# DerrickXuNu/CoBEVT

Measured on AMD Instinct MI355X. Metric: bev_frames_per_sec, higher is better.
Workload: dtype bf16

## Files before the change

### cobevt_amd/build.py

```python
import os
import subprocess
import sys

CSRC = os.path.join(os.path.dirname(os.path.abspath(__file__)), "csrc")
LIB = os.path.join(CSRC, "libcobevt_hip.so")
LIB_F32S = os.path.join(CSRC, "libcobevt_hip_f32s.so")
LIB_F32H = os.path.join(CSRC, "libcobevt_hip_f32h.so")
SOURCES = ["igemm.hip", "conv3x3.hip", "basicblock.hip", "bottleneck.hip", "bottleneck_f32.hip", "gemm_rows.hip", "gemm_rows3.hip", "gemm_rows3_f32.hip", "bev_query.hip", "row_chain.hip", "row_chain_f32.hip", "row_chain64.hip", "ln_linear64.hip", "proj_chain128.hip", "proj_chain_k.hip", "swap_stage.hip", "stem7x7.hip", "attention.hip", "attention_resident.hip", "attention_bwd.hip", "train_rows.hip", "train_glue.hip", "train_prep.hip", "wgrad3.hip", "train_nusc.hip", "train_fax.hip", "elementwise.hip", "pairwise_fusion.hip", "postprocess.hip", "depthwise.hip", "peer_gather.hip", "calibrate.hip"]
HEADERS = ["common.hpp", "attn_common.hpp", "warp_common.hpp", "row_chain.hpp", "bev_query.hpp"]
FLAGS = ["--offload-arch=gfx950", "-O3", "-std=c++17", "-fPIC", "-Wno-pass-failed"]
EXTRA_FLAGS = {}


def _hipcc():
    for cand in (os.environ.get("HIPCC"), "/opt/rocm/bin/hipcc", "hipcc"):
        if cand and (os.path.sep not in cand or os.path.exists(cand)):
            return cand
    raise RuntimeError("hipcc not found")


def _stale(target, deps):
    if not os.path.exists(target):
        return True
    t = os.path.getmtime(target)
    return any(os.path.getmtime(d) > t for d in deps)


def _build_one(lib, objdir, extra, force, verbose):
    hipcc = _hipcc()
    hdrs = [os.path.join(CSRC, h) for h in HEADERS]
    os.makedirs(objdir, exist_ok=True)
    objs = []
    procs = []
    for src in SOURCES:
        s = os.path.join(CSRC, src)
        o = os.path.join(objdir, src.replace(".hip", ".o"))
        objs.append(o)
        if force or _stale(o, [s] + hdrs):
            cmd = [hipcc] + FLAGS + extra + EXTRA_FLAGS.get(src, []) + ["-c", s, "-o", o]
            if verbose:
                print(" ".join(cmd), flush=True)
            procs.append((src, subprocess.Popen(cmd, stdout=subprocess.PIPE, stderr=subprocess.STDOUT)))
    for src, p in procs:
        out, _ = p.communicate()
        if p.returncode != 0:
            raise RuntimeError("hipcc failed for %s:\n%s" % (src, out.decode(errors="replace")))
    if force or _stale(lib, objs):
        cmd = [hipcc, "--offload-arch=gfx950", "-shared", "-fPIC", "-o", lib] + objs
        if verbose:
            print(" ".join(cmd), flush=True)
        subprocess.check_call(cmd)
    return lib


def build(force=False, verbose=True):
    _build_one(LIB_F32S, os.path.join(CSRC, "f32s"), ["-DCOBEVT_F32_SPLIT=1"], force, verbose)
    _build_one(LIB_F32H, os.path.join(CSRC, "f32h"), ["-DCOBEVT_F32_SPLIT=2"], force, verbose)
    return _build_one(LIB, CSRC, [], force, verbose)


if __name__ == "__main__":
    build(force="--force" in sys.argv)
    print(LIB)
```

### cobevt_amd/csrc/proj_chain128.hip

```cpp
#include "row_chain.hpp"

namespace cobevt {

namespace {

constexpr int kFp = 0, kFn = 32, kMaxNnt = 8;
constexpr int kTab = (kFn + kMaxNnt * 8) * 1024;
constexpr int kSc = 0, kSh = 128, kBp = 256, kBn = 384;
constexpr int kTabFloats = 640;
constexpr int kLdsBytes = kTab + kTabFloats * 4;

__device__ __forceinline__ float xhalf_sum(float v) {
    const auto r = __builtin_amdgcn_permlane32_swap(__float_as_uint(v), __float_as_uint(v), false, false);
    return __uint_as_float(r[0]) + __uint_as_float(r[1]);
}
__device__ __forceinline__ void half_swap(uint2& a, uint2& b) {
    auto r = __builtin_amdgcn_permlane32_swap(a.x, b.x, false, false);
    a.x = r[0]; b.x = r[1];
    r = __builtin_amdgcn_permlane32_swap(a.y, b.y, false, false);
    a.y = r[0]; b.y = r[1];
}
__device__ __forceinline__ uint4 pack8(const float* v) {
    return make_uint4(pack_bf2(v[0], v[1]), pack_bf2(v[2], v[3]), pack_bf2(v[4], v[5]), pack_bf2(v[6], v[7]));
}
__device__ __forceinline__ float rbf(float x) { return bf2f(f2bf(x)); }

template <int NNT, int NW>
__global__ __launch_bounds__(NW * 64, 1) void proj_chain128_kernel(RowChainParams p, int nblk) {
    extern __shared__ __attribute__((aligned(16))) unsigned char smem[];
    const uint4* wl = (const uint4*)smem;
    float* tab = (float*)(smem + kTab);
    const int tid = threadIdx.x, lane = tid & 63, wave = tid >> 6;
    const int h = lane >> 5, ql = lane & 31;

    {
        uint4* dst = (uint4*)smem;
        constexpr int TOTAL = (kFn + NNT * 8) * 64, PER = (TOTAL + NW * 64 - 1) / (NW * 64);
        uint4 tmp[PER];
#pragma unroll
        for (int u = 0; u < PER; ++u) {
            const int i = tid + u * NW * 64, ic = i < TOTAL ? i : TOTAL - 1;
            const int f = ic >> 6, ln = ic & 63, hh = ln >> 5, q = ln & 31;
            const uint4* base = f < kFn ? p.wp + (size_t)f * 64 : p.wn + (size_t)(f - kFn) * 64;
            const unsigned char* a0 = (const unsigned char*)(base + (f < kFn ? ln : q)) + (f < kFn ? 0 : 8 * hh);
            const unsigned char* a1 = f < kFn ? a0 + 8 : (const unsigned char*)(base + 32 + q) + 8 * hh;
            const uint2 lo = *(const uint2*)a0, hi = *(const uint2*)a1;
            tmp[u] = make_uint4(lo.x, lo.y, hi.x, hi.y);
        }
#pragma unroll
        for (int u = 0; u < PER; ++u) {
            const int i = tid + u * NW * 64;
            if (i < TOTAL) dst[i] = tmp[u];
        }
        for (int i = tid; i < kTabFloats; i += NW * 64) {
            float v;
            if (i < kSh) v = p.pre_scale ? p.pre_scale[i] : 1.f;
            else if (i < kBp) v = p.pre_shift ? p.pre_shift[i - kSh] : 0.f;
            else if (i < kBn) v = p.bp ? p.bp[i - kBp] : 0.f;
            else v = (p.bn && i - kBn < p.Nn) ? p.bn[i - kBn] : 0.f;
            tab[i] = v;
        }
    }
    __syncthreads();

    int opq = 0;
    const float relu_floor = (p.pre_scale && p.pre_relu) ? 0.f : -INFINITY;
    auto load_tile = [&](uint4 (&fr)[8], int first) {
#pragma unroll
        for (int g = 0; g < 8; ++g) fr[g] = wl[(first + g) * 64 + lane + opq];
    };
    const int nwaves = gridDim.x * NW;
    for (int blk = blockIdx.x * NW + wave; blk < nblk; blk += nwaves) {
        asm volatile("" : "+v"(opq));
        const int m0 = blk * 32;
        const bool live = m0 + ql < p.M;
        const size_t grow = live ? m0 + ql : p.M - 1;
        const bf16_t* arow = p.a + grow * 128;
        uint4 af[8], sk[8];
#pragma unroll
        for (int g = 0; g < 8; ++g) af[g] = *(const uint4*)(arow + 16 * g + 8 * h);
        if (p.skip) {
            const bf16_t* srow = p.skip + (size_t)(grow % p.skip_rows) * 128;
#pragma unroll
            for (int g = 0; g < 8; ++g) sk[g] = *(const uint4*)(srow + 16 * g + 8 * h);
        } else {
#pragma unroll
            for (int g = 0; g < 8; ++g) sk[g] = make_uint4(0, 0, 0, 0);
        }
#pragma unroll
        for (int g = 0; g < 8; ++g) {
            float v[8];
            chunk_to_f32<bf16_t>(af[g], v);
            const float* sc = tab + kSc + 16 * g + 8 * h + opq;
            const float4 s0 = *(const float4*)sc, s1 = *(const float4*)(sc + 4);
            const float4 t0 = *(const float4*)(sc + (kSh - kSc)), t1 = *(const float4*)(sc + (kSh - kSc) + 4);
            v[0] = fmaxf(fmaf(v[0], s0.x, t0.x), relu_floor); v[1] = fmaxf(fmaf(v[1], s0.y, t0.y), relu_floor);
            v[2] = fmaxf(fmaf(v[2], s0.z, t0.z), relu_floor); v[3] = fmaxf(fmaf(v[3], s0.w, t0.w), relu_floor);
            v[4] = fmaxf(fmaf(v[4], s1.x, t1.x), relu_floor); v[5] = fmaxf(fmaf(v[5], s1.y, t1.y), relu_floor);
            v[6] = fmaxf(fmaf(v[6], s1.z, t1.z), relu_floor); v[7] = fmaxf(fmaf(v[7], s1.w, t1.w), relu_floor);
            af[g] = f32_to_chunk<bf16_t>(v);
        }

        float y[4][16];
        uint4 fr[2][8];
        load_tile(fr[0], kFp);
#pragma unroll
        for (int t = 0; t < 4; ++t) {
            f32x16 acc;
#pragma unroll
            for (int r = 0; r < 16; ++r) acc[r] = 0.f;
            load_tile(fr[(t + 1) & 1], t < 3 ? kFp + (t + 1) * 8 : kFn);
            __builtin_amdgcn_sched_barrier(0);
#pragma unroll
            for (int g = 0; g < 8; ++g) mfma_kgroup<bf16_t>(fr[t & 1][g], af[g], acc);
#pragma unroll
            for (int m = 0; m < 2; ++m) {
                uint2 s0 = make_uint2(sk[2 * t + m].x, sk[2 * t + m].y), s1 = make_uint2(sk[2 * t + m].z, sk[2 * t + m].w);
                half_swap(s0, s1);
                const float4 b0 = *(const float4*)(tab + kBp + 32 * t + 16 * m + 4 * h + opq);
                const float4 b1 = *(const float4*)(tab + kBp + 32 * t + 16 * m + 8 + 4 * h + opq);
                float* d = &y[t][8 * m];
                d[0] = rbf(acc[8 * m + 0] + b0.x + bf2f(s0.x & 0xffff)); d[1] = rbf(acc[8 * m + 1] + b0.y + bf2f(s0.x >> 16));
                d[2] = rbf(acc[8 * m + 2] + b0.z + bf2f(s0.y & 0xffff)); d[3] = rbf(acc[8 * m + 3] + b0.w + bf2f(s0.y >> 16));
                d[4] = rbf(acc[8 * m + 4] + b1.x + bf2f(s1.x & 0xffff)); d[5] = rbf(acc[8 * m + 5] + b1.y + bf2f(s1.x >> 16));
                d[6] = rbf(acc[8 * m + 6] + b1.z + bf2f(s1.y & 0xffff)); d[7] = rbf(acc[8 * m + 7] + b1.w + bf2f(s1.y >> 16));
            }
        }
        if (p.out) {
            bf16_t* orow = p.out + grow * 128;
#pragma unroll
            for (int i = 0; i < 8; ++i) {
                const uint4 pk = pack8(&y[i >> 1][8 * (i & 1)]);
                uint2 r0 = make_uint2(pk.x, pk.y), r1 = make_uint2(pk.z, pk.w);
                half_swap(r0, r1);
                if (live) *(uint4*)(orow + 16 * i + 8 * h) = make_uint4(r0.x, r0.y, r1.x, r1.y);
            }
        }
        if (p.next_ln) {
            float s = 0.f;
#pragma unroll
            for (int t = 0; t < 4; ++t)
#pragma unroll
                for (int r = 0; r < 16; ++r) s += y[t][r];
            const float mean = xhalf_sum(s) * (1.0f / 128.0f);
            float q = 0.f;
#pragma unroll
            for (int t = 0; t < 4; ++t)
#pragma unroll
                for (int r = 0; r < 16; ++r) { const float d = y[t][r] - mean; q += d * d; }
            const float rstd = rsqrtf(xhalf_sum(q) * (1.0f / 128.0f) + p.eps_next);
#pragma unroll
            for (int t = 0; t < 4; ++t)
#pragma unroll
                for (int r = 0; r < 16; ++r) y[t][r] = (y[t][r] - mean) * rstd;
        }
        uint4 yh[8];
#pragma unroll
        for (int t = 0; t < 4; ++t)
#pragma unroll
            for (int u = 0; u < 2; ++u) yh[2 * t + u] = pack8(&y[t][8 * u]);

        bf16_t* nrow = p.out_next + grow * p.Nn;
#pragma unroll
        for (int n = 0; n < NNT; ++n) {
            f32x16 acc;
#pragma unroll
            for (int r = 0; r < 16; ++r) acc[r] = 0.f;
            if (n + 1 < NNT) load_tile(fr[(n + 1) & 1], kFn + (n + 1) * 8);
            __builtin_amdgcn_sched_barrier(0);
#pragma unroll
            for (int g = 0; g < 8; ++g) mfma_kgroup<bf16_t>(fr[n & 1][g], yh[g], acc);
            float nv[16];
#pragma unroll
            for (int k = 0; k < 4; ++k) {
                const float4 b = *(const float4*)(tab + kBn + 32 * n + 8 * k + 4 * h + opq);
                nv[4 * k] = acc[4 * k] + b.x; nv[4 * k + 1] = acc[4 * k + 1] + b.y;
                nv[4 * k + 2] = acc[4 * k + 2] + b.z; nv[4 * k + 3] = acc[4 * k + 3] + b.w;
            }
#pragma unroll
            for (int m = 0; m < 2; ++m) {
                const uint4 pk = pack8(&nv[8 * m]);
                uint2 r0 = make_uint2(pk.x, pk.y), r1 = make_uint2(pk.z, pk.w);
                half_swap(r0, r1);
                if (live) *(uint4*)(nrow + 32 * n + 16 * m + 8 * h) = make_uint4(r0.x, r0.y, r1.x, r1.y);
            }
        }
    }
}

template <int NNT> int launch128(const RowChainParams& p, hipStream_t stream) {
    constexpr int NW = 8;
    static cobevt::PerDeviceOnce attr_once;
    if (attr_once.first()) {
        (void)hipFuncSetAttribute((const void*)proj_chain128_kernel<NNT, NW>, hipFuncAttributeMaxDynamicSharedMemorySize, kLdsBytes);
    }
    const int nblk = (p.M + 31) / 32;
    int blocks = (nblk + NW - 1) / NW;
    if (blocks > 256) blocks = 256;
    hipLaunchKernelGGL((proj_chain128_kernel<NNT, NW>), dim3((unsigned)blocks), dim3(NW * 64), kLdsBytes, stream, p, nblk);
    return hipGetLastError() == hipSuccess ? COBEVT_OK : COBEVT_ERR_LAUNCH;
}

}

int launch_proj_chain128(const RowChainParams& p, hipStream_t stream) {
    if (p.C != 128 || !p.wn || !p.out_next || p.Nn % 32 != 0 || p.Nn > 32 * kMaxNnt || p.next_act != 0) return -1;
    if (p.M < 32768) return -1;
    switch (p.Nn / 32) {
        case 4: return launch128<4>(p, stream);
        case 8: return launch128<8>(p, stream);
        default: return -1;
    }
}

}
```

### cobevt_amd/csrc/proj_chain_k.hip

```cpp
#include "row_chain.hpp"

namespace cobevt {

namespace {

constexpr int kRow = 256 + 16;
constexpr int kNnMax = 768;

struct ProjChainKSide {
    const float* pre_scale;
    const float* pre_shift;
    const uint4* wp;
    const float* bp;
    const bf16_t* skip;
    const uint4* wn;
    const float* bn;
    bf16_t* out;
    bf16_t* out_next;
    int pre_relu, skip_rows;
};

struct ProjChainKParams {
    const bf16_t* a;
    ProjChainKSide side[2];
    int M, K, Nn, next_ln;
    float eps_next;
};

struct Lds {
    static constexpr int A = 0;
    static constexpr int Y = A + 32 * kRow;
    static constexpr int BIAS = Y + 32 * kRow;
    static constexpr int BYTES = BIAS + 4 * (128 + kNnMax);
};

__device__ __forceinline__ void normalise128(float (&v)[16], float eps) {
    float s = 0.f;
#pragma unroll
    for (int e = 0; e < 16; ++e) s += v[e];
    s += __shfl_xor(s, 1, 64); s += __shfl_xor(s, 2, 64); s += __shfl_xor(s, 4, 64);
    const float mean = s * (1.0f / 128.0f);
    float q = 0.f;
#pragma unroll
    for (int e = 0; e < 16; ++e) { const float d = v[e] - mean; q += d * d; }
    q += __shfl_xor(q, 1, 64); q += __shfl_xor(q, 2, 64); q += __shfl_xor(q, 4, 64);
    const float rstd = rsqrtf(q * (1.0f / 128.0f) + eps);
#pragma unroll
    for (int e = 0; e < 16; ++e) v[e] = (v[e] - mean) * rstd;
}

template <int NCH>
__global__ __launch_bounds__(256, 4) void proj_chain_k_kernel(ProjChainKParams p) {
    extern __shared__ __attribute__((aligned(16))) unsigned char smem[];
    unsigned char* As = smem + Lds::A;
    unsigned char* Ys = smem + Lds::Y;
    float* sb = (float*)(smem + Lds::BIAS);

    ProjChainKSide sd;
    {
        const bool s1 = blockIdx.y != 0;
        const ProjChainKSide &u = p.side[0], &w = p.side[1];
        sd.pre_scale = s1 ? w.pre_scale : u.pre_scale; sd.pre_shift = s1 ? w.pre_shift : u.pre_shift;
        sd.wp = s1 ? w.wp : u.wp; sd.bp = s1 ? w.bp : u.bp; sd.skip = s1 ? w.skip : u.skip;
        sd.wn = s1 ? w.wn : u.wn; sd.bn = s1 ? w.bn : u.bn; sd.out = s1 ? w.out : u.out; sd.out_next = s1 ? w.out_next : u.out_next;
        sd.pre_relu = s1 ? w.pre_relu : u.pre_relu; sd.skip_rows = s1 ? w.skip_rows : u.skip_rows;
    }
    const int tid = threadIdx.x, lane = tid & 63, wn = tid >> 6;
    const int h = lane >> 5, ql = lane & 31;
    const int m0 = blockIdx.x * 32;
    const int row = ql;
    const bool row_ok = m0 + row < p.M;
    const int sr = tid >> 3, sub = tid & 7;
    const bool srow_ok = m0 + sr < p.M;
    constexpr int NKG = NCH * 8;

    {
        constexpr int NIT = (128 + kNnMax + 255) / 256;
        float val[NIT];
#pragma unroll
        for (int it = 0; it < NIT; ++it) {
            const int i = tid + it * 256;
            const bool isp = i < 128;
            const float* src = isp ? sd.bp : sd.bn;
            const int j = isp ? i : i - 128;
            const bool keep = (src != nullptr) & (i < 128 + kNnMax) & (isp | (j < p.Nn));
            val[it] = keep ? src[j] : 0.f;
        }
#pragma unroll
        for (int it = 0; it < NIT; ++it) {
            const int i = tid + it * 256;
            if (i < 128 + kNnMax) sb[i] = val[it];
        }
    }

    auto load_frags = [&](uint4 (&b)[8], const uint4* w, int tile, int nkg, int kg0) {
        const uint4* src = w + ((size_t)tile * nkg + kg0) * 64 + lane;
#pragma unroll
        for (int g = 0; g < 8; ++g) b[g] = src[g * 64];
        __builtin_amdgcn_sched_barrier(0);
    };
    f32x16 acc;
    auto mma = [&](const uint4 (&b)[8], bool zero) {
        if (zero) {
#pragma unroll
            for (int r = 0; r < 16; ++r) acc[r] = 0.f;
        }
        const int abase = row * kRow + h * 16;
#pragma unroll
        for (int g = 0; g < 8; ++g) {
            const uint4 af = *(const uint4*)(As + abase + g * 32);
            mfma_kgroup<bf16_t>(b[g], af, acc);
        }
    };
    auto load_rows = [&](uint4 (&v)[2], int c) {
        const bf16_t* src = p.a + (size_t)(srow_ok ? m0 + sr : 0) * p.K + c * 128 + sub * 16;
        v[0] = *(const uint4*)src;
        v[1] = *(const uint4*)(src + 8);
    };
    auto stage_rows = [&](const uint4 (&v)[2], int c) {
#pragma unroll
        for (int j = 0; j < 2; ++j) {
            uint4 o = v[j];
            if (sd.pre_scale) {
                const int k = c * 128 + sub * 16 + j * 8;
                float f[8];
                chunk_to_f32<bf16_t>(v[j], f);
                const float4 s0 = *(const float4*)(sd.pre_scale + k), s1 = *(const float4*)(sd.pre_scale + k + 4);
                const float4 t0 = *(const float4*)(sd.pre_shift + k), t1 = *(const float4*)(sd.pre_shift + k + 4);
                const float sc[8] = {s0.x, s0.y, s0.z, s0.w, s1.x, s1.y, s1.z, s1.w}, sh[8] = {t0.x, t0.y, t0.z, t0.w, t1.x, t1.y, t1.z, t1.w};
#pragma unroll
                for (int e = 0; e < 8; ++e) {
                    f[e] = fmaf(f[e], sc[e], sh[e]);
                    if (sd.pre_relu) f[e] = fmaxf(f[e], 0.f);
                }
                o = f32_to_chunk<bf16_t>(f);
            }
            if (!srow_ok) o = make_uint4(0, 0, 0, 0);
            *(uint4*)(As + sr * kRow + sub * 32 + j * 16) = o;
        }
    };

    uint4 fa[8], fb[8];
    uint4 ra[2], rb[2];
    load_rows(ra, 0);
    load_frags(fa, sd.wp, wn, NKG, 0);
    const int cbase = wn * 32 + 4 * h;
    uint2 skp[4];
#pragma unroll
    for (int k = 0; k < 4; ++k) {
        skp[k] = make_uint2(0, 0);
        if (sd.skip && row_ok) skp[k] = *(const uint2*)(sd.skip + (size_t)((m0 + row) % sd.skip_rows) * 128 + cbase + 8 * k);
    }

#pragma unroll
    for (int c = 0; c < NCH; ++c) {
        if (c & 1) stage_rows(rb, c); else stage_rows(ra, c);
        if (c + 1 < NCH) {
            if (c & 1) { load_rows(ra, c + 1); load_frags(fa, sd.wp, wn, NKG, 8 * (c + 1)); }
            else { load_rows(rb, c + 1); load_frags(fb, sd.wp, wn, NKG, 8 * (c + 1)); }
        } else {
            if (c & 1) load_frags(fa, sd.wn, wn, 8, 0); else load_frags(fb, sd.wn, wn, 8, 0);
        }
        __syncthreads();
        if (c & 1) mma(fb, false); else mma(fa, c == 0);
        __syncthreads();
    }

    auto pack4 = [&](float x, float y, float z, float w) { return make_uint2(pack_bf2(x, y), pack_bf2(z, w)); };
#pragma unroll
    for (int k = 0; k < 4; ++k) {
        const int col0 = cbase + 8 * k;
        const float4 b = *(const float4*)(sb + col0);
        *(uint2*)(Ys + row * kRow + col0 * 2) = pack4(acc[4 * k] + b.x + bf2f(skp[k].x & 0xffff), acc[4 * k + 1] + b.y + bf2f(skp[k].x >> 16),
                                                      acc[4 * k + 2] + b.z + bf2f(skp[k].y & 0xffff), acc[4 * k + 3] + b.w + bf2f(skp[k].y >> 16));
    }
    __syncthreads();

    {
        const uint4 y0 = *(const uint4*)(Ys + sr * kRow + sub * 32), y1 = *(const uint4*)(Ys + sr * kRow + sub * 32 + 16);
        if (sd.out && srow_ok) {
            *(uint4*)(sd.out + (size_t)(m0 + sr) * 128 + sub * 16) = y0;
            *(uint4*)(sd.out + (size_t)(m0 + sr) * 128 + sub * 16 + 8) = y1;
        }
        uint4 o0 = y0, o1 = y1;
        if (p.next_ln) {
            float v[16];
            chunk_to_f32<bf16_t>(y0, v);
            chunk_to_f32<bf16_t>(y1, v + 8);
            normalise128(v, p.eps_next);
            o0 = f32_to_chunk<bf16_t>(v);
            o1 = f32_to_chunk<bf16_t>(v + 8);
        }
        *(uint4*)(As + sr * kRow + sub * 32) = o0;
        *(uint4*)(As + sr * kRow + sub * 32 + 16) = o1;
    }
    __syncthreads();

    const int npn = (p.Nn + 127) / 128;
    auto next_pass = [&](int pass, const uint4 (&cur)[8], uint4 (&nxt)[8]) {
        if (pass + 1 < npn) load_frags(nxt, sd.wn, (pass + 1) * 4 + wn, 8, 0);
        mma(cur, true);
#pragma unroll
        for (int k = 0; k < 4; ++k) {
            const int col0 = pass * 128 + cbase + 8 * k;
            const float4 b = *(const float4*)(sb + 128 + col0);
            *(uint2*)(Ys + row * kRow + (cbase + 8 * k) * 2) = pack4(acc[4 * k] + b.x, acc[4 * k + 1] + b.y, acc[4 * k + 2] + b.z, acc[4 * k + 3] + b.w);
        }
        __syncthreads();
        if (srow_ok) {
#pragma unroll
            for (int j = 0; j < 2; ++j) {
                const int c0 = pass * 128 + sub * 16 + j * 8;
                if (c0 < p.Nn) *(uint4*)(sd.out_next + (size_t)(m0 + sr) * p.Nn + c0) = *(const uint4*)(Ys + sr * kRow + sub * 32 + j * 16);
            }
        }
        if (pass + 1 < npn) __syncthreads();
    };
    for (int pass = 0; pass < npn; pass += 2) {
        if (NCH & 1) {
            next_pass(pass, fb, fa);
            if (pass + 1 < npn) next_pass(pass + 1, fa, fb);
        } else {
            next_pass(pass, fa, fb);
            if (pass + 1 < npn) next_pass(pass + 1, fb, fa);
        }
    }
}

template <int NCH>
void launch(const ProjChainKParams& p, int nsides, hipStream_t stream) {
    static cobevt::PerDeviceOnce attr_once;
    if (attr_once.first())
        (void)hipFuncSetAttribute((const void*)proj_chain_k_kernel<NCH>, hipFuncAttributeMaxDynamicSharedMemorySize, Lds::BYTES);
    hipLaunchKernelGGL((proj_chain_k_kernel<NCH>), dim3((unsigned)((p.M + 31) / 32), (unsigned)nsides), dim3(256), Lds::BYTES, stream, p);
}

}

}

using namespace cobevt;

extern "C" int cobevt_proj_chain_kv(const void* a, const void* const* ptrs, const int* dims, float eps_next, hipStream_t stream) {
    if (!a || !ptrs || !dims) return COBEVT_ERR_ARG;
    if (dims[0] != 0) return COBEVT_ERR_UNSUPPORTED;
    ProjChainKParams p;
    p.a = (const bf16_t*)a;
    p.M = dims[1]; p.K = dims[2]; p.Nn = dims[3]; p.next_ln = dims[4];
    const int nsides = dims[5];
    p.eps_next = eps_next;
    if (nsides < 1 || nsides > 2) return COBEVT_ERR_ARG;
    if (p.M < 1 || p.K < 256 || p.K > 512 || p.K % 128) return COBEVT_ERR_SHAPE;
    if (p.Nn < 8 || p.Nn % 8 || p.Nn > kNnMax) return COBEVT_ERR_SHAPE;
    for (int s = 0; s < 2; ++s) {
        const void* const* q = ptrs + 9 * (s < nsides ? s : 0);
        ProjChainKSide& sd = p.side[s];
        sd.pre_scale = (const float*)q[0]; sd.pre_shift = (const float*)q[1];
        sd.wp = (const uint4*)q[2]; sd.bp = (const float*)q[3]; sd.skip = (const bf16_t*)q[4];
        sd.wn = (const uint4*)q[5]; sd.bn = (const float*)q[6];
        sd.out = (bf16_t*)q[7]; sd.out_next = (bf16_t*)q[8];
        sd.pre_relu = dims[6 + 2 * (s < nsides ? s : 0)];
        sd.skip_rows = dims[7 + 2 * (s < nsides ? s : 0)] > 0 ? dims[7 + 2 * (s < nsides ? s : 0)] : p.M;
        if (!sd.wp || !sd.wn || !sd.out_next) return COBEVT_ERR_ARG;
        if ((sd.pre_scale == nullptr) != (sd.pre_shift == nullptr)) return COBEVT_ERR_ARG;
        if (sd.skip_rows > p.M || p.M % sd.skip_rows) return COBEVT_ERR_SHAPE;
    }
    switch (p.K / 128) {
        case 2: launch<2>(p, nsides, stream); break;
        case 3: launch<3>(p, nsides, stream); break;
        default: launch<4>(p, nsides, stream); break;
    }
    return hipGetLastError() == hipSuccess ? COBEVT_OK : COBEVT_ERR_LAUNCH;
}
```

### cobevt_amd/csrc/row_chain.hip

```cpp
#include "row_chain.hpp"

namespace cobevt {

constexpr int kRcRow = 256 + 16;
constexpr int kRcHRow = 512 + 16;
template <int ROWS> struct RcLds {
    static constexpr int A = 0;
    static constexpr int Y = A + ROWS * kRcRow;
    static constexpr int H = Y + ROWS * kRcRow;
    static constexpr int TOTAL = H + ROWS * kRcHRow;
    static constexpr int BIAS = TOTAL;
    static constexpr int BYTES = TOTAL + 4 * 1536;
};
constexpr int kRcBp = 0, kRcB1 = 128, kRcB2 = 384, kRcPg = 512, kRcPb = 640, kRcBn = 768, kRcBnMax = 768, kRcBiasFloats = 1536;

__device__ __forceinline__ void rc_normalise(float (&v)[16], int sub, int C, float eps) {
    float s = 0.f;
#pragma unroll
    for (int e = 0; e < 16; ++e) s += v[e];
    s += __shfl_xor(s, 1, 64); s += __shfl_xor(s, 2, 64); s += __shfl_xor(s, 4, 64);
    const float mean = s / (float)C;
    float q = 0.f;
#pragma unroll
    for (int e = 0; e < 16; ++e) { const float d = (sub * 16 + e) < C ? v[e] - mean : 0.f; q += d * d; }
    q += __shfl_xor(q, 1, 64); q += __shfl_xor(q, 2, 64); q += __shfl_xor(q, 4, 64);
    const float rstd = rsqrtf(q / (float)C + eps);
#pragma unroll
    for (int e = 0; e < 16; ++e) v[e] = (sub * 16 + e) < C ? (v[e] - mean) * rstd : 0.f;
}

template <int NPASS, int ROWS, bool FULL, bool MLP = true>
__global__ __launch_bounds__(ROWS * 8, 4) void row_chain_kernel(RowChainParams p) {
    extern __shared__ __attribute__((aligned(16))) unsigned char smem[];
    unsigned char* As = smem + RcLds<ROWS>::A;
    unsigned char* Ys = smem + RcLds<ROWS>::Y;
    unsigned char* Hs = smem + RcLds<ROWS>::H;

    const int tid = threadIdx.x, lane = tid & 63, wave = tid >> 6;
    const int h = lane >> 5, ql = lane & 31;
    const int wm = wave >> 2, wn = wave & 3;
    const int m0 = blockIdx.x * ROWS;
    const int ngc = FULL ? 8 : (p.C * 2 + 31) / 32;
    const int row = wm * 32 + ql;
    const bool row_ok = m0 + row < p.M;

    auto load_frags = [&](uint4 (&b)[8], const uint4* w, int tile, int nkg, int kg0, int n) {
        const uint4* src = w + ((size_t)tile * nkg + kg0) * 64 + lane;
#pragma unroll
        for (int g = 0; g < 8; ++g)
            if (g < n) b[g] = src[g * 64];
        __builtin_amdgcn_sched_barrier(0);
    };
    f32x16 acc;
    auto mma = [&](const unsigned char* A, int a_off, const uint4 (&b)[8], int n, bool zero) {
        if (zero) {
#pragma unroll
            for (int r = 0; r < 16; ++r) acc[r] = 0.f;
        }
#pragma unroll
        for (int g = 0; g < 8; ++g)
            if (g < n) {
                const uint4 af = *(const uint4*)(A + a_off + g * 32);
                mfma_kgroup<bf16_t>(b[g], af, acc);
            }
    };
    const int cbase = wn * 32 + 4 * h;
    const float* sb = (const float*)(smem + RcLds<ROWS>::BIAS);
    {
        float* w = (float*)(smem + RcLds<ROWS>::BIAS);
        constexpr int NT = ROWS * 8, NIT = kRcBiasFloats / NT;
        static_assert(kRcBiasFloats % NT == 0, "bias table fill");
        float val[NIT];
        bool keep[NIT];
#pragma unroll
        for (int it = 0; it < NIT; ++it) {
            const int i = tid + it * NT;
            const float* src = i < kRcB1 ? p.bp : i < kRcB2 ? p.b1 : i < kRcPg ? p.b2 : i < kRcPb ? p.post_g : i < kRcBn ? p.post_b : p.bn;
            const int j = i < kRcB1 ? i : i < kRcB2 ? i - kRcB1 : i < kRcPg ? i - kRcB2 : i < kRcPb ? i - kRcPg : i < kRcBn ? i - kRcPb : i - kRcBn;
            const int n = i < kRcB1 ? p.C : i < kRcB2 ? p.Hd : i < kRcBn ? p.C : p.Nn;
            keep[it] = (src != nullptr) & (j < n);
            val[it] = (src ? src : p.b1)[keep[it] ? j : 0];
        }
#pragma unroll
        for (int it = 0; it < NIT; ++it) w[tid + it * NT] = keep[it] ? val[it] : 0.f;
    }
    auto bias4 = [&](int table, int col0) { return *(const float4*)(sb + table + col0); };
    auto pack4 = [&](float x, float y, float z, float w) { return make_uint2(pack_bf2(x, y), pack_bf2(z, w)); };

    uint4 fa[8], fb[8];
    const int abase = row * kRcRow + h * 16;

    load_frags(fa, p.wp, wn, 8, 0, ngc);
    {
        const int r = tid >> 3, sub = tid & 7;
        const bool ok = m0 + r < p.M;
#pragma unroll
        for (int j = 0; j < 2; ++j) {
            const int k = (sub * 2 + j) * 8;
            uint4 v = make_uint4(0, 0, 0, 0);
            if (ok && k < p.C) v = *(const uint4*)(p.a + (size_t)(m0 + r) * p.C + k);
            if (!MLP && p.pre_scale) {
                float f[8];
                chunk_to_f32<bf16_t>(v, f);
                const float4 s0 = *(const float4*)(p.pre_scale + k), s1 = *(const float4*)(p.pre_scale + k + 4);
                const float4 t0 = *(const float4*)(p.pre_shift + k), t1 = *(const float4*)(p.pre_shift + k + 4);
                const float sc[8] = {s0.x, s0.y, s0.z, s0.w, s1.x, s1.y, s1.z, s1.w}, sh[8] = {t0.x, t0.y, t0.z, t0.w, t1.x, t1.y, t1.z, t1.w};
#pragma unroll
                for (int e = 0; e < 8; ++e) {
                    f[e] = fmaf(f[e], sc[e], sh[e]);
                    if (p.pre_relu) f[e] = fmaxf(f[e], 0.f);
                }
                v = ok ? f32_to_chunk<bf16_t>(f) : make_uint4(0, 0, 0, 0);
            }
            *(uint4*)(As + r * kRcRow + (sub * 2 + j) * 16) = v;
        }
    }
    uint2 skp[4];
#pragma unroll
    for (int k = 0; k < 4; ++k) {
        const int col0 = cbase + 8 * k;
        skp[k] = make_uint2(0, 0);
        if (p.skip && row_ok && col0 < p.C) skp[k] = *(const uint2*)(p.skip + (size_t)((m0 + row) % p.skip_rows) * p.C + col0);
    }
    __syncthreads();

    mma(As, abase, fa, ngc, true);
    if (MLP) load_frags(fb, p.w1, wn, 8, 0, ngc);
    else load_frags(fb, p.wn, wn, 8, 0, ngc);
#pragma unroll
    for (int k = 0; k < 4; ++k) {
        const int col0 = cbase + 8 * k;
        const float4 b = bias4(kRcBp, col0);
        float v0 = acc[4 * k] + b.x + bf2f(skp[k].x & 0xffff), v1 = acc[4 * k + 1] + b.y + bf2f(skp[k].x >> 16);
        float v2 = acc[4 * k + 2] + b.z + bf2f(skp[k].y & 0xffff), v3 = acc[4 * k + 3] + b.w + bf2f(skp[k].y >> 16);
        if (col0 >= p.C) v0 = v1 = v2 = v3 = 0.f;
        *(uint2*)(Ys + row * kRcRow + col0 * 2) = pack4(v0, v1, v2, v3);
    }
    __syncthreads();
    float* stage = (float*)Hs;
    constexpr int SROW = kRcHRow / 4;
    if constexpr (MLP) {

    if (NPASS == 2) load_frags(fa, p.w1, 4 + wn, 8, 0, ngc);
    else load_frags(fa, p.w2, wn, p.Hdp / 16, 0, 8);
    {
        const int r = tid >> 3, sub = tid & 7;
        float v[16];
        chunk_to_f32<bf16_t>(*(const uint4*)(Ys + r * kRcRow + sub * 32), v);
        chunk_to_f32<bf16_t>(*(const uint4*)(Ys + r * kRcRow + sub * 32 + 16), v + 8);
        rc_normalise(v, sub, p.C, p.eps1);
        *(uint4*)(As + r * kRcRow + sub * 32) = f32_to_chunk<bf16_t>(v);
        *(uint4*)(As + r * kRcRow + sub * 32 + 16) = f32_to_chunk<bf16_t>(v + 8);
    }
    __syncthreads();

    auto hidden_epilogue = [&](int pass) {
#pragma unroll
        for (int k = 0; k < 4; ++k) {
            const int col0 = pass * 128 + cbase + 8 * k;
            const float4 b = bias4(kRcB1, col0);
            uint2 o = make_uint2(0, 0);
            if (col0 < p.Hd) o = pack4(gelu_bf16(acc[4 * k] + b.x), gelu_bf16(acc[4 * k + 1] + b.y),
                                       gelu_bf16(acc[4 * k + 2] + b.z), gelu_bf16(acc[4 * k + 3] + b.w));
            *(uint2*)(Hs + row * kRcHRow + col0 * 2) = o;
        }
    };
    const int hbase = row * kRcHRow + h * 16;
    if (NPASS == 2) {
        mma(As, abase, fb, ngc, true);
        load_frags(fb, p.w2, wn, p.Hdp / 16, 0, 8);
        hidden_epilogue(0);
        mma(As, abase, fa, ngc, true);
        load_frags(fa, p.w2, wn, p.Hdp / 16, 8, 8);
        hidden_epilogue(1);
        __syncthreads();
        mma(Hs, hbase, fb, 8, true);
        load_frags(fb, p.wn ? p.wn : p.w1, wn, 8, 0, ngc);
        mma(Hs, hbase + 256, fa, 8, false);
    } else {
        mma(As, abase, fb, ngc, true);
        load_frags(fb, p.wn ? p.wn : p.w1, wn, 8, 0, ngc);
        hidden_epilogue(0);
        __syncthreads();
        mma(Hs, hbase, fa, (p.Hd * 2 + 31) / 32, true);
    }
    __syncthreads();
#pragma unroll
    for (int k = 0; k < 4; ++k) {
        const int col0 = cbase + 8 * k;
        const float4 b = bias4(kRcB2, col0);
        const uint2 y = *(const uint2*)(Ys + row * kRcRow + col0 * 2);
        float4 z = make_float4(0.f, 0.f, 0.f, 0.f);
        if (col0 < p.C)
            z = make_float4(acc[4 * k] + b.x + bf2f(y.x & 0xffff), acc[4 * k + 1] + b.y + bf2f(y.x >> 16),
                            acc[4 * k + 2] + b.z + bf2f(y.y & 0xffff), acc[4 * k + 3] + b.w + bf2f(y.y >> 16));
        *(float4*)(stage + row * SROW + col0) = z;
    }
    } else {
#pragma unroll
        for (int k = 0; k < 4; ++k) {
            const int col0 = cbase + 8 * k;
            const uint2 y = *(const uint2*)(Ys + row * kRcRow + col0 * 2);
            *(float4*)(stage + row * SROW + col0) = make_float4(bf2f(y.x & 0xffff), bf2f(y.x >> 16), bf2f(y.y & 0xffff), bf2f(y.y >> 16));
        }
    }
    const int npn = p.wn ? (p.Nn + 127) / 128 : 0;
    __syncthreads();

    {
        const int r = tid >> 3, sub = tid & 7;
        const bool live = m0 + r < p.M;
        float v[16];
#pragma unroll
        for (int e = 0; e < 16; e += 4) {
            const float4 t = *(const float4*)(stage + r * SROW + sub * 16 + e);
            v[e] = t.x; v[e + 1] = t.y; v[e + 2] = t.z; v[e + 3] = t.w;
        }
        if (p.post_g) {
            rc_normalise(v, sub, p.C, p.eps_post);
#pragma unroll
            for (int e = 0; e < 16; e += 4) {
                const float4 g = *(const float4*)(sb + kRcPg + sub * 16 + e), b = *(const float4*)(sb + kRcPb + sub * 16 + e);
                v[e] = v[e] * g.x + b.x; v[e + 1] = v[e + 1] * g.y + b.y;
                v[e + 2] = v[e + 2] * g.z + b.z; v[e + 3] = v[e + 3] * g.w + b.w;
            }
        }
        uint4 o[2];
        o[0] = f32_to_chunk<bf16_t>(v);
        o[1] = f32_to_chunk<bf16_t>(v + 8);
        if (live && (MLP || p.out)) {
#pragma unroll
            for (int j = 0; j < 2; ++j) {
                const int c0 = sub * 16 + j * 8;
                if (c0 < p.C) *(uint4*)(p.out + (size_t)(m0 + r) * p.C + c0) = o[j];
            }
        }
        if (!npn) return;

        if (p.next_ln) {
            chunk_to_f32<bf16_t>(o[0], v);
            chunk_to_f32<bf16_t>(o[1], v + 8);
            rc_normalise(v, sub, p.C, p.eps_next);
            o[0] = f32_to_chunk<bf16_t>(v);
            o[1] = f32_to_chunk<bf16_t>(v + 8);
        }
        *(uint4*)(As + r * kRcRow + sub * 32) = o[0];
        *(uint4*)(As + r * kRcRow + sub * 32 + 16) = o[1];
    }
    __syncthreads();
    auto next_pass = [&](int pass, const uint4 (&cur)[8], uint4 (&nxt)[8]) {
        if (pass + 1 < npn) load_frags(nxt, p.wn, (pass + 1) * 4 + wn, 8, 0, ngc);
        mma(As, abase, cur, ngc, true);
#pragma unroll
        for (int k = 0; k < 4; ++k) {
            const int col0 = pass * 128 + cbase + 8 * k;
            const float4 b = bias4(kRcBn, col0);
            float v0 = acc[4 * k] + b.x, v1 = acc[4 * k + 1] + b.y, v2 = acc[4 * k + 2] + b.z, v3 = acc[4 * k + 3] + b.w;
            if (p.next_act == 1) { v0 = fmaxf(v0, 0.f); v1 = fmaxf(v1, 0.f); v2 = fmaxf(v2, 0.f); v3 = fmaxf(v3, 0.f); }
            else if (p.next_act == 2) { v0 = gelu_bf16(v0); v1 = gelu_bf16(v1); v2 = gelu_bf16(v2); v3 = gelu_bf16(v3); }
            *(uint2*)(Ys + row * kRcRow + (cbase + 8 * k) * 2) = pack4(v0, v1, v2, v3);
        }
        __syncthreads();
        {
            const int r = tid >> 3, sub = tid & 7;
            if (m0 + r < p.M) {
#pragma unroll
                for (int j = 0; j < 2; ++j) {
                    const int c0 = pass * 128 + sub * 16 + j * 8;
                    if (c0 < p.Nn) *(uint4*)(p.out_next + (size_t)(m0 + r) * p.Nn + c0) = *(const uint4*)(Ys + r * kRcRow + sub * 32 + j * 16);
                }
            }
        }
        if (pass + 1 < npn) __syncthreads();
    };
    for (int pass = 0; pass < npn; pass += 2) {
        next_pass(pass, fb, fa);
        if (pass + 1 < npn) next_pass(pass + 1, fa, fb);
    }
}

template <int NPASS, int ROWS, bool FULL, bool MLP = true>
static void launch_chain(const RowChainParams& p, hipStream_t stream) {
    static cobevt::PerDeviceOnce attr_once;
    if (attr_once.first()) {
        (void)hipFuncSetAttribute((const void*)row_chain_kernel<NPASS, ROWS, FULL, MLP>, hipFuncAttributeMaxDynamicSharedMemorySize, RcLds<ROWS>::BYTES);
    }
    const unsigned blocks = (unsigned)((p.M + ROWS - 1) / ROWS);
    hipLaunchKernelGGL((row_chain_kernel<NPASS, ROWS, FULL, MLP>), dim3(blocks), dim3(ROWS * 8), RcLds<ROWS>::BYTES, stream, p);
}

}

using namespace cobevt;

extern "C" int cobevt_attn_mlp_chain(const void* a, const void* skip, void* out, const void* wp, const float* bp,
                                     const void* w1, const float* b1, const void* w2, const float* b2,
                                     const float* post_gamma, const float* post_beta, const void* wnext, const float* bnext,
                                     void* out_next, const int* dims, float eps1, float eps_post, float eps_next,
                                     hipStream_t stream) {
    if (!a || !out || !wp || !w1 || !b1 || !w2 || !b2 || !dims) return COBEVT_ERR_ARG;
    if (dims[0] != 0 && dims[0] != 1) return COBEVT_ERR_ARG;
    if (dims[0] == 1) {
        if ((post_gamma == nullptr) != (post_beta == nullptr) || (wnext == nullptr) != (out_next == nullptr)) return COBEVT_ERR_ARG;
        const int M = dims[1], sr = dims[9] > 0 ? dims[9] : dims[1];
        if (M < 1 || sr > M || M % sr || (wnext && (dims[7] < 0 || dims[7] > 2))) return COBEVT_ERR_SHAPE;
        const int rc = launch_row_chain_f32(a, skip, out, wp, bp, w1, b1, w2, b2, post_gamma, post_beta, wnext, bnext, out_next, M, dims[2], dims[3],
                                            dims[4], dims[5], dims[6], dims[7], sr, eps1, eps_post, eps_next, stream);
        return rc < 0 ? COBEVT_ERR_UNSUPPORTED : rc;
    }
    RowChainParams p;
    p.a = (const bf16_t*)a; p.skip = (const bf16_t*)skip; p.out = (bf16_t*)out;
    p.wp = (const uint4*)wp; p.bp = bp; p.w1 = (const uint4*)w1; p.b1 = b1; p.w2 = (const uint4*)w2; p.b2 = b2;
    p.post_g = post_gamma; p.post_b = post_beta;
    p.wn = (const uint4*)wnext; p.bn = bnext; p.out_next = (bf16_t*)out_next;
    p.M = dims[1]; p.C = dims[2]; p.Hd = dims[3]; p.Hdp = dims[4];
    p.Nn = dims[5]; p.next_ln = dims[6]; p.next_act = dims[7];
    p.skip_rows = dims[9] > 0 ? dims[9] : p.M;
    p.eps1 = eps1; p.eps_post = eps_post; p.eps_next = eps_next;
    p.pre_scale = p.pre_shift = nullptr; p.pre_relu = 0;
    if (p.M < 1 || p.C < 8 || p.C > 128 || p.C % 8 || p.Hd < 8 || p.Hd > 256 || p.Hd % 8) return COBEVT_ERR_SHAPE;
    if (p.Hdp % 128 || p.Hdp < p.Hd || p.Hdp > 256) return COBEVT_ERR_SHAPE;
    if (p.skip_rows > p.M || p.M % p.skip_rows) return COBEVT_ERR_SHAPE;
    if ((post_gamma == nullptr) != (post_beta == nullptr)) return COBEVT_ERR_ARG;
    if ((wnext == nullptr) != (out_next == nullptr)) return COBEVT_ERR_ARG;
    if (wnext && (p.Nn < 8 || p.Nn % 8 || p.Nn > kRcBnMax || p.next_act < 0 || p.next_act > 2)) return COBEVT_ERR_SHAPE;
    if (dims[8] == 0) {
        const int rc = launch_row_chain64(p, stream);
        if (rc >= 0) return rc;
    }
    const int rows = dims[8] == 64 ? 64 : 32;
    const bool two = p.Hd > 128, full = p.C == 128;
    if (rows == 64) {
        if (two) { if (full) launch_chain<2, 64, true>(p, stream); else launch_chain<2, 64, false>(p, stream); }
        else { if (full) launch_chain<1, 64, true>(p, stream); else launch_chain<1, 64, false>(p, stream); }
    } else {
        if (two) { if (full) launch_chain<2, 32, true>(p, stream); else launch_chain<2, 32, false>(p, stream); }
        else { if (full) launch_chain<1, 32, true>(p, stream); else launch_chain<1, 32, false>(p, stream); }
    }
    return hipGetLastError() == hipSuccess ? COBEVT_OK : COBEVT_ERR_LAUNCH;
}

extern "C" int cobevt_proj_chain(const void* a, const float* pre_scale, const float* pre_shift, const void* skip, const void* wp,
                                 const float* bp, void* out, const void* wnext, const float* bnext, void* out_next, const int* dims,
                                 float eps_next, hipStream_t stream) {
    if (!a || !wp || !wnext || !bnext || !out_next || !dims) return COBEVT_ERR_ARG;
    if ((pre_scale == nullptr) != (pre_shift == nullptr)) return COBEVT_ERR_ARG;
    if (dims[0] != 0) return COBEVT_ERR_UNSUPPORTED;
    RowChainParams p;
    p.a = (const bf16_t*)a; p.skip = (const bf16_t*)skip; p.out = (bf16_t*)out;
    p.wp = (const uint4*)wp; p.bp = bp;
    p.w1 = (const uint4*)wnext; p.b1 = bnext; p.w2 = (const uint4*)wnext; p.b2 = bnext;
    p.post_g = p.post_b = nullptr;
    p.wn = (const uint4*)wnext; p.bn = bnext; p.out_next = (bf16_t*)out_next;
    p.M = dims[1]; p.C = dims[2]; p.Hd = 8; p.Hdp = 128;
    p.Nn = dims[3]; p.next_ln = dims[4]; p.next_act = dims[5];
    p.skip_rows = dims[6] > 0 ? dims[6] : p.M;
    p.pre_scale = pre_scale; p.pre_shift = pre_shift; p.pre_relu = dims[7];
    p.eps1 = 0.f; p.eps_post = 0.f; p.eps_next = eps_next;
    if (p.M < 1 || p.C != 128) return COBEVT_ERR_SHAPE;
    if (p.Nn < 8 || p.Nn % 8 || p.Nn > kRcBnMax || p.next_act < 0 || p.next_act > 2) return COBEVT_ERR_SHAPE;
    if (p.skip_rows > p.M || p.M % p.skip_rows) return COBEVT_ERR_SHAPE;
    if (dims[8] == 0) {
        const int rc = launch_proj_chain128(p, stream);
        if (rc >= 0) return rc;
    }
    launch_chain<1, 32, true, false>(p, stream);
    return hipGetLastError() == hipSuccess ? COBEVT_OK : COBEVT_ERR_LAUNCH;
}
```

### cobevt_amd/csrc/row_chain.hpp

```cpp
#pragma once
#include "common.hpp"

namespace cobevt {

struct RowChainParams {
    const bf16_t* a;
    const bf16_t* skip;
    bf16_t* out;
    const uint4* wp;
    const float* bp;
    const uint4* w1;
    const float* b1;
    const uint4* w2;
    const float* b2;
    const float* post_g;
    const float* post_b;
    const uint4* wn;
    const float* bn;
    bf16_t* out_next;
    int M, C, Hd, Hdp;
    int Nn, next_ln, next_act, skip_rows;
    float eps1, eps_post, eps_next;
    const float* pre_scale;
    const float* pre_shift;
    int pre_relu;
};

int launch_row_chain64(const RowChainParams& p, hipStream_t stream);
int launch_proj_chain128(const RowChainParams& p, hipStream_t stream);

int launch_row_chain_f32(const void* a, const void* skip, void* out, const void* wp, const float* bp, const void* w1, const float* b1,
                         const void* w2, const float* b2, const float* post_g, const float* post_b, const void* wnext, const float* bnext,
                         void* out_next, int M, int C, int Hd, int Hdp, int Nn, int next_ln, int next_act, int skip_rows, float eps1,
                         float eps_post, float eps_next, hipStream_t stream);

}
```

### cobevt_amd/host/fax_modules.py

```python
import torch
import torch.nn as nn

from .. import ops
from ..lib import CobevtHipError
from . import runtime as rt
from . import training
from .runtime import HipModule


def generate_grid(height, width):
    xs = torch.linspace(0, 1, width)
    ys = torch.linspace(0, 1, height)
    gx = xs[None, :].expand(height, width)
    gy = ys[:, None].expand(height, width)
    return torch.stack([gx, gy, torch.ones(height, width)], 0)[None].contiguous()


def get_view_matrix(h=200, w=200, h_meters=100.0, w_meters=100.0, offset=0.0):
    sh = h / h_meters
    sw = w / w_meters
    return [[0., -sw, w / 2.], [-sh, 0., h * offset + h / 2.], [0., 0., 1.]]


class Bottleneck(HipModule):
    expansion = 4

    def __init__(self, inplanes, planes):
        super().__init__()
        width = planes
        self.conv1 = nn.Conv2d(inplanes, width, 1, bias=False)
        self.bn1 = nn.BatchNorm2d(width)
        self.conv2 = nn.Conv2d(width, width, 3, 1, 1, bias=False)
        self.bn2 = nn.BatchNorm2d(width)
        self.conv3 = nn.Conv2d(width, planes * self.expansion, 1, bias=False)
        self.bn3 = nn.BatchNorm2d(planes * self.expansion)
        self.relu = nn.ReLU(inplace=True)
        self.downsample = None

    def entry_plan(self):
        return rt.conv_plan(self, "c1", self.conv1, self.bn1, act=1)

    def fused_plan(self):
        if self.conv1.weight.shape[:2] != (32, 128) or self.downsample is not None:
            return None
        return self._plan("fused", rt.module_tensors(self.conv1, self.bn1, self.conv2, self.bn2, self.conv3, self.bn3),
                          lambda dt, dev: ops.BottleneckPlan(self.conv1, self.bn1, self.conv2, self.bn2, self.conv3, self.bn3, dev))

    def fusable(self, x):
        return ops.bottleneck_fusable(x) and self.conv1.weight.shape[:2] == (32, 128)

    def forward_nhwc(self, x, y1=None):
        if y1 is None and self.fusable(x):
            return ops.bottleneck(x, self.fused_plan())
        p1, p2, p3 = self.entry_plan(), rt.conv_plan(self, "c2", self.conv2, self.bn2, act=1), rt.conv_plan(self, "c3", self.conv3, self.bn3, act=1)
        if ops.bottleneck_f32_fusable(x, p1, p2, p3, y1):
            return ops.bottleneck_f32(x, p1, p2, p3, y1)
        y = ops.conv2d(x, p1) if y1 is None else y1
        y = ops.conv2d(y, p2)
        return ops.conv2d(y, p3, residual=x)

    def forward(self, x):
        if self.training:
            return training.bottleneck(self, x)
        self._require_inference(x)
        return rt.like_input(rt.nchw_view(self.forward_nhwc(rt.to_nhwc(x))), x)


ResNetBottleNeck = lambda c: Bottleneck(c, c // 4)


class BEVEmbedding(nn.Module):

    def __init__(self, dim, sigma, bev_height, bev_width, h_meters, w_meters, offset, upsample_scales):
        super().__init__()
        V_inv = torch.FloatTensor(get_view_matrix(bev_height, bev_width, h_meters, w_meters, offset)).inverse()
        for i, scale in enumerate(upsample_scales):
            h, w = bev_height // scale, bev_width // scale
            grid = generate_grid(h, w).squeeze(0)
            grid[0] = bev_width * grid[0]
            grid[1] = bev_height * grid[1]
            grid = (V_inv @ grid.reshape(3, h * w)).reshape(3, h, w)
            self.register_buffer("grid%d" % i, grid, persistent=False)
        self.learned_features = nn.Parameter(
            sigma * torch.randn(dim, bev_height // upsample_scales[0], bev_width // upsample_scales[0]))

    def get_prior(self):
        return self.learned_features


class Attention(HipModule):

    def __init__(self, dim, dim_head=32, dropout=0., window_size=25):
        super().__init__()
        assert (dim % dim_head) == 0, "dimension should be divisible by dimension per head"
        if dim_head != 32:
            raise CobevtHipError("the HIP attention kernel is built for dim_head = 32")
        self.heads = dim // dim_head
        self.scale = dim_head ** -0.5
        self.window_size = window_size
        self.to_qkv = nn.Linear(dim, dim * 3, bias=False)
        self.attend = nn.Sequential(nn.Softmax(dim=-1), nn.Dropout(dropout))
        self.to_out = nn.Sequential(nn.Linear(dim, dim, bias=False), nn.Dropout(dropout))
        self.rel_pos_bias = nn.Embedding((2 * window_size - 1) ** 2, self.heads)
        pos = torch.arange(window_size)
        gi, gj = torch.meshgrid(pos, pos, indexing="ij")
        grid = torch.stack([gi.reshape(-1), gj.reshape(-1)], -1)
        rel_pos = grid[:, None, :] - grid[None, :, :] + window_size - 1
        rel_pos_indices = (rel_pos * torch.tensor([2 * window_size - 1, 1])).sum(dim=-1)
        self.register_buffer("rel_pos_indices", rel_pos_indices, persistent=False)

    def forward_nhwc(self, x, out=None):
        b, h, w, d = x.shape
        if h != self.window_size or w != self.window_size:
            raise CobevtHipError("FAX global attention expects a %dx%d map" % (self.window_size, self.window_size))
        qkv = ops.linear(x, rt.linear_plan(self, "qkv", self.to_qkv))
        a = torch.empty((b, h, w, d), device=x.device, dtype=x.dtype)
        m = ops.tokmap(0, 1, h, w, h, w)
        table = rt.f32_param(self, "bias", self.rel_pos_bias.weight)
        ops.window_attention(qkv, qkv, qkv, a, m, m, m, b, self.heads, self.scale, 3 * d, 3 * d, 3 * d, d, koff=d,
                             voff=2 * d, bias_table=table, bias_L=1)
        return ops.linear(a, rt.linear_plan(self, "out", self.to_out[0]), out=out)

    def forward(self, x):
        if self.training:
            return training.global_attention(self, x)
        self._require_inference(x)
        return rt.like_input(rt.nchw_view(self.forward_nhwc(rt.to_nhwc(x))), x)


class CrossWinAttention(HipModule):

    def __init__(self, dim, heads, dim_head, qkv_bias, rel_pos_emb=False, norm=nn.LayerNorm):
        super().__init__()
        if dim_head != 32:
            raise CobevtHipError("the HIP attention kernel is built for dim_head = 32")
        self.scale = dim_head ** -0.5
        self.heads = heads
        self.dim_head = dim_head
        self.rel_pos_emb = rel_pos_emb
        self.to_q = nn.Sequential(norm(dim), nn.Linear(dim, heads * dim_head, bias=qkv_bias))
        self.to_k = nn.Sequential(norm(dim), nn.Linear(dim, heads * dim_head, bias=qkv_bias))
        self.to_v = nn.Sequential(norm(dim), nn.Linear(dim, heads * dim_head, bias=qkv_bias))
        self.proj = nn.Linear(heads * dim_head, dim)

    def add_rel_pos_emb(self, x):
        return x

    def _project(self, name, seq, x, out=None):
        return ops.linear(x, rt.linear_plan(self, name, seq[1], ln=seq[0]), out=out)

    def project_kv(self, k_src, v_src, out_k=None, out_v=None):
        return self._project("k", self.to_k, k_src, out_k), self._project("v", self.to_v, v_src, out_v)

    def q_plan(self):
        return rt.linear_plan(self, "q", self.to_q[1], ln=self.to_q[0])

    def attend_projected(self, q_src, kt, vt, qmap, kmap, omap, batch, out_shape, qt=None, ldkv=None, kvoff=0):
        inner = self.heads * self.dim_head
        if qt is None:
            qt = self._project("q", self.to_q, q_src)
        ld = inner if ldkv is None else ldkv
        a = torch.empty(tuple(out_shape) + (inner,), device=qt.device, dtype=qt.dtype)
        ops.window_attention(qt, kt, vt, a, qmap, kmap, omap, batch, self.heads, self.scale, inner, ld, ld, inner,
                             koff=kvoff, voff=kvoff, mean_q=qmap[1] > 1)
        return a

    def attend_core(self, q_src, k_src, v_src, qmap, kmap, omap, batch, out_shape):
        kt, vt = self.project_kv(k_src, v_src)
        return self.attend_projected(q_src, kt, vt, qmap, kmap, omap, batch, out_shape)

    def attend(self, q_src, k_src, v_src, qmap, kmap, omap, batch, skip, out_shape):
        a = self.attend_core(q_src, k_src, v_src, qmap, kmap, omap, batch, out_shape)
        return ops.linear(a, rt.linear_plan(self, "proj", self.proj), residual=skip)

    def forward(self, q, k, v, skip=None):
        if self.training:
            return training.cross_win_attention(self, q, k, v, skip)
        self._require_inference(q, k, v, skip)
        assert k.shape == v.shape
        b, n, X, Y, W1, W2, _ = q.shape
        _, nk, kx, ky, w1, w2, _ = k.shape
        assert X * Y == kx * ky
        qmap = (2, n, X * W1, Y * W2, W1, W2, X, Y)
        kmap = (2, nk, kx * w1, ky * w2, w1, w2, kx, ky)
        omap = (2, 1, X * W1, Y * W2, W1, W2, X, Y)
        sk = rt.as_compute(skip) if skip is not None else None
        z = self.attend(rt.as_compute(q), rt.as_compute(k), rt.as_compute(v), qmap, kmap, omap, b, sk,
                        (b, X, Y, W1, W2))
        return rt.like_input(z, q)


class CrossViewSwapAttention(HipModule):

    def __init__(self, feat_height, feat_width, feat_dim, dim, index, image_height, image_width, qkv_bias, q_win_size,
                 feat_win_size, heads, dim_head, bev_embedding_flag, rel_pos_emb=False, no_image_features=False,
                 skip=True, norm=nn.LayerNorm):
        super().__init__()
        image_plane = generate_grid(feat_height, feat_width)[None]
        image_plane[:, :, 0] *= image_width
        image_plane[:, :, 1] *= image_height
        self.register_buffer("image_plane", image_plane, persistent=False)
        self.feature_linear = nn.Sequential(nn.BatchNorm2d(feat_dim), nn.ReLU(), nn.Conv2d(feat_dim, dim, 1, bias=False))
        if no_image_features:
            self.feature_proj = None
        else:
            self.feature_proj = nn.Sequential(nn.BatchNorm2d(feat_dim), nn.ReLU(), nn.Conv2d(feat_dim, dim, 1, bias=False))
        self.bev_embed_flag = bev_embedding_flag[index]
        if self.bev_embed_flag:
            self.bev_embed = nn.Conv2d(2, dim, 1)
        self.img_embed = nn.Conv2d(4, dim, 1, bias=False)
        self.cam_embed = nn.Conv2d(4, dim, 1, bias=False)
        self.q_win_size = q_win_size[index]
        self.feat_win_size = feat_win_size[index]
        self.rel_pos_emb = rel_pos_emb
        self.cross_win_attend_1 = CrossWinAttention(dim, heads[index], dim_head[index], qkv_bias)
        self.cross_win_attend_2 = CrossWinAttention(dim, heads[index], dim_head[index], qkv_bias)
        self.skip = skip
        self.prenorm_1 = norm(dim)
        self.prenorm_2 = norm(dim)
        self.mlp_1 = nn.Sequential(nn.Linear(dim, 2 * dim), nn.GELU(), nn.Linear(2 * dim, dim))
        self.mlp_2 = nn.Sequential(nn.Linear(dim, 2 * dim), nn.GELU(), nn.Linear(2 * dim, dim))
        self.postnorm = norm(dim)
        self.dim = dim

    def _padded_hw(self, h, w):
        wh, ww = self.feat_win_size
        hp = ((h + wh) // wh) * wh if h % wh != 0 else h
        wp = ((w + ww) // ww) * ww if w % ww != 0 else w
        return hp, wp

    def _proj_mlp(self, name, attn, a, skip, prenorm, mlp, postnorm=None, next_plan=None):
        post = None
        if postnorm is not None:
            post = (rt.f32_param(self, name + ".post.w", postnorm.weight), rt.f32_param(self, name + ".post.b", postnorm.bias),
                    postnorm.eps)
        return ops.attn_mlp_chain(a, skip, rt.linear_plan(attn, "proj", attn.proj),
                                  rt.linear_plan(self, name + ".0", mlp[0], act=2, ln=prenorm),
                                  rt.linear_plan(self, name + ".2", mlp[2]), post, next_plan=next_plan)

    def prepare_kv(self, feature, I_inv, E_inv, batch, out=None):
        bn, h, w, _ = feature.shape
        d, dt = self.dim, feature.dtype
        n = bn // batch
        w1, w2 = self.feat_win_size
        hp, wp = self._padded_hw(h, w)
        padded = (hp, wp) != (h, w)
        plane = rt.f32_param(self, "plane", self.image_plane, (3, h * w))
        w_img = rt.f32_param(self, "w_img", self.img_embed.weight, (d, 4))
        w_cam = rt.f32_param(self, "w_cam", self.cam_embed.weight, (d, 4))
        img = ops.ray_embed(I_inv, E_inv, plane, w_img, w_cam, h * w, d, dt).reshape(bn, h, w, d)

        def kv_buffer(tag):
            if not padded:
                return None
            return self._plan("kvpad.%s.%dx%dx%d" % (tag, bn, hp, wp), [self.img_embed.weight],
                              lambda dt_, dev: torch.zeros((bn, hp, wp, d), device=feature.device, dtype=dt))

        o = out if out is not None else {}
        pk, pv = self._pair_plan("k"), self._pair_plan("v")
        plan_key = rt.conv_plan(self, "fproj", self.feature_proj[2], pre_bn=self.feature_proj[0]) if self.feature_proj is not None else None
        plan_val = rt.conv_plan(self, "flin", self.feature_linear[2], pre_bn=self.feature_linear[0])
        if (not padded and plan_key is not None and ops.proj_chain_fusable(feature, plan_key, pk, img)
                and ops.proj_chain_fusable(feature, plan_val, pv, None)):
            kk = ops.proj_chain(feature, plan_key, pk, residual=img, out_next=o.get("kk"))
            vv = ops.proj_chain(feature, plan_val, pv, out_next=o.get("vv"))
            return {"n": n, "hp": hp, "wp": wp, "kk": kk, "vv": vv}
        if not padded and plan_key is not None and ops.proj_chain_kv_fusable(feature, plan_key, plan_val, pk, pv, img):
            kk, vv = ops.proj_chain_kv(feature, plan_key, plan_val, pk, pv, residual=img, out_k=o.get("kk"), out_v=o.get("vv"))
            return {"n": n, "hp": hp, "wp": wp, "kk": kk, "vv": vv}
        if self.feature_proj is not None:
            key = ops.conv2d(feature, plan_key, residual=img, out=kv_buffer("key"))
        elif padded:
            key = ops.copy_into_interior(img, kv_buffer("key"))
        else:
            key = img
        val = ops.conv2d(feature, plan_val, out=kv_buffer("val"))
        kk = ops.linear(key, pk, out=o.get("kk"))
        vv = ops.linear(val, pv, out=o.get("vv"))
        return {"n": n, "hp": hp, "wp": wp, "kk": kk, "vv": vv}

    def _pair_plan(self, which):
        a1, a2 = getattr(self.cross_win_attend_1, "to_" + which), getattr(self.cross_win_attend_2, "to_" + which)
        if a1[0].eps != a2[0].eps:
            raise CobevtHipError("the two cross attentions normalise their keys / values with different eps")

        def build(dt, dev):
            ws, bs = [], []
            for ln, lin in ((a1[0], a1[1]), (a2[0], a2[1])):
                w = lin.weight.detach().double().cpu()
                b = lin.bias.detach().double().cpu() if lin.bias is not None else torch.zeros(w.shape[0], dtype=torch.float64)
                g, be = ln.weight.detach().double().cpu(), ln.bias.detach().double().cpu()
                bs.append(b + w @ be)
                ws.append(w * g[None, :])
            return ops.ConvPlan(torch.cat(ws), torch.cat(bs), dtype=dt, device=dev, ln_folded_eps=a1[0].eps)
        return self._plan("pair_" + which, rt.module_tensors(a1[0], a1[1], a2[0], a2[1]), build)

    def forward_query(self, index, x, bev, E_inv, kv, next_plan=None):
        b, H, W, d = x.shape
        n, hp, wp = kv["n"], kv["hp"], kv["wp"]
        W1, W2 = self.q_win_size
        w1, w2 = self.feat_win_size
        if self.bev_embed_flag:
            grid = getattr(bev, "grid%d" % index)
            world = rt.f32_param(self, "world%d" % index, grid[:2], (2, H * W))
            w_bev = rt.f32_param(self, "w_bev", self.bev_embed.weight, (d, 2))
            b_bev = rt.f32_param(self, "b_bev", self.bev_embed.bias)
            w_cam = rt.f32_param(self, "w_cam", self.cam_embed.weight, (d, 4))
            q1 = ops.bev_embed_linear(E_inv, world, w_bev, b_bev, w_cam, x.reshape(b, H * W, d), n,
                                      self.cross_win_attend_1.q_plan())
            query, nq = None, n
        else:
            x = x.contiguous()
            query, nq, q1 = x, 1, None
        qmap_n = ops.tokmap(0, nq, H, W, W1, W2)
        qmap_1 = ops.tokmap(0, 1, H, W, W1, W2)
        kwin = ops.tokmap(0, n, hp, wp, w1, w2)
        kgrid = ops.tokmap(1, n, hp, wp, w1, w2)
        if qmap_1[6] * qmap_1[7] != kwin[6] * kwin[7]:
            raise CobevtHipError("query windows %dx%d != key windows %dx%d" % (qmap_1[6], qmap_1[7], kwin[6], kwin[7]))
        inner = self.cross_win_attend_1.heads * self.cross_win_attend_1.dim_head
        a = self.cross_win_attend_1.attend_projected(query, kv["kk"], kv["vv"], qmap_n, kwin, qmap_1, b, (b, H, W), qt=q1,
                                                     ldkv=2 * inner, kvoff=0)
        y, q2 = self._proj_mlp("mlp1", self.cross_win_attend_1, a, x if self.skip else None, self.prenorm_1, self.mlp_1,
                               next_plan=self.cross_win_attend_2.q_plan())
        a = self.cross_win_attend_2.attend_projected(y, kv["kk"], kv["vv"], qmap_1, kgrid, qmap_1, b, (b, H, W), qt=q2,
                                                     ldkv=2 * inner, kvoff=inner)
        return self._proj_mlp("mlp2", self.cross_win_attend_2, a, y if self.skip else None, self.prenorm_2, self.mlp_2,
                              self.postnorm, next_plan=next_plan)

    def forward_nhwc(self, index, x, bev, feature, I_inv, E_inv):
        return self.forward_query(index, x, bev, E_inv, self.prepare_kv(feature, I_inv, E_inv, x.shape[0]))

    def forward(self, index, x, bev, feature, I_inv, E_inv):
        if self.training:
            return training.cross_view_swap_attention(self, index, x, bev, feature, I_inv, E_inv)
        self._require_inference(x, feature, I_inv, E_inv)
        b, n = feature.shape[:2]
        f = rt.to_nhwc(feature.reshape(b * n, *feature.shape[2:]))
        Ii = I_inv.reshape(b * n, 3, 3).to(torch.float32).contiguous()
        Ei = E_inv.reshape(b * n, 4, 4).to(torch.float32).contiguous()
        y = self.forward_nhwc(index, rt.to_nhwc(x), bev, f, Ii, Ei)
        return rt.like_input(rt.nchw_view(y), x)


class _Downsample(HipModule):

    def __init__(self, dim_in, dim_mid, dim_out):
        super().__init__()
        mods = [nn.Conv2d(dim_in, dim_mid, kernel_size=3, stride=1, padding=1, bias=False), nn.PixelUnshuffle(2),
                nn.Conv2d(dim_out, dim_out, 3, padding=1, bias=False), nn.BatchNorm2d(dim_out), nn.ReLU(inplace=True),
                nn.Conv2d(dim_out, dim_out, 1, padding=0, bias=False), nn.BatchNorm2d(dim_out)]
        for i, m in enumerate(mods):
            self.add_module(str(i), m)

    def __getitem__(self, i):
        return getattr(self, str(i))

    def forward_nhwc(self, x, out=None):
        y = ops.conv2d(x, rt.conv_plan(self, "c0", self[0], store_mode=1))
        y = ops.conv2d(y, rt.conv_plan(self, "c2", self[2], self[3], act=1))
        return ops.conv2d(y, rt.conv_plan(self, "c5", self[5], self[6]), out=out)


class FAXModule(HipModule):

    _downsample_div = 4

    def __init__(self, config):
        super().__init__()
        middle = config["middle"]
        dim = config["dim"]
        self.backbone_output_shape = config["backbone_output_shape"]
        assert len(middle) == len(self.backbone_output_shape)
        cross_view = config["cross_view"]
        cross_view_swap = config["cross_view_swap"]
        cross_views, layers, downsample_layers = [], [], []
        for i, (feat_shape, num_layers) in enumerate(zip(self.backbone_output_shape, middle)):
            _, _, _, feat_dim, feat_height, feat_width = tuple(feat_shape)
            cross_views.append(CrossViewSwapAttention(feat_height, feat_width, feat_dim, dim[i], i, **cross_view,
                                                      **cross_view_swap))
            layers.append(nn.Sequential(*[ResNetBottleNeck(dim[i]) for _ in range(num_layers)]))
            if i < len(middle) - 1:
                downsample_layers.append(nn.Sequential(_Downsample(dim[i], dim[i] // self._downsample_div, dim[i + 1])))
        self.bev_embedding = BEVEmbedding(dim[0], **config["bev_embedding"])
        self.cross_views = nn.ModuleList(cross_views)
        self.layers = nn.ModuleList(layers)
        self.downsample_layers = nn.ModuleList(downsample_layers)
        self.self_attn = Attention(dim[-1], **config["self_attn"])

    taps = None

    def forward_features(self, features, I_inv, E_inv, batch, kv=None, levels=None, x=None, out=None):
        nlev = len(self.cross_views)
        first, last = (0, nlev) if levels is None else levels
        if first == 0:
            dt = rt.get_compute_dtype()
            prior = self._plan("prior", [self.bev_embedding.learned_features],
                               lambda d_, dev: self.bev_embedding.learned_features.detach().permute(1, 2, 0).to(dt).contiguous())
            x = prior[None].expand(batch, *prior.shape)
        for i, (cross_view, feature, layer) in enumerate(zip(self.cross_views, features, self.layers)):
            if i < first or i >= last:
                continue
            kvi = kv[i]() if kv is not None else cross_view.prepare_kv(feature, I_inv, E_inv, batch)
            blocks = list(layer)
            y1 = None
            if blocks and not (x.dtype == torch.bfloat16 and ops.USE_BOTTLENECK and x.shape[-1] == 128
                               and blocks[0].conv1.weight.shape[:2] == (32, 128)):
                x, y1 = cross_view.forward_query(i, x, self.bev_embedding, E_inv, kvi, next_plan=blocks[0].entry_plan())
            else:
                x = cross_view.forward_query(i, x, self.bev_embedding, E_inv, kvi)
            for j, blk in enumerate(blocks):
                x = blk.forward_nhwc(x, y1=y1 if j == 0 else None)
            if self.taps is not None:
                self.taps["level%d" % i] = x
            if i < len(self.cross_views) - 1:
                final = out is not None and i == last - 1 and not (self.self_attn is not None and last == nlev)
                x = self.downsample_layers[i][0].forward_nhwc(x, out=out if final else None)
        if self.self_attn is not None and last == nlev:
            x = self.self_attn.forward_nhwc(x, out=out)
        if out is not None and x.data_ptr() != out.data_ptr():
            out.copy_(x)
            x = out
        return x

    def forward(self, batch):
        if self.training:
            return training.fax_module(self, batch)
        b, l, n = batch["inputs"].shape[:3]
        intrinsic, extrinsic = batch["intrinsic"], batch["extrinsic"]
        self._require_inference(intrinsic, extrinsic, *batch["features"])
        I_inv = ops.invert_small(intrinsic.reshape(b * l * n, 3, 3))
        E_inv = self._extrinsic(extrinsic.reshape(b * l * n, 4, 4).to(torch.float32)).contiguous()
        feats = [rt.to_nhwc(f.reshape(b * l * n, *f.shape[3:])) for f in batch["features"]]
        x = self.forward_features(feats, I_inv, E_inv, b * l)
        x = rt.nchw_view(x)
        return x.reshape(b, l, *x.shape[1:])

    @staticmethod
    def _extrinsic(e):
        return e
```

### cobevt_amd/lib.py

```python
import ctypes
import os

import torch

_HERE = os.path.dirname(os.path.abspath(__file__))
LIB_PATH = os.path.join(_HERE, "csrc", "libcobevt_hip.so")
LIB_PATH = os.environ.get("COBEVT_HIP_LIB") or LIB_PATH

_c_int_p = ctypes.POINTER(ctypes.c_int)
_c_long_p = ctypes.POINTER(ctypes.c_long)
_vp = ctypes.c_void_p

SIGNATURES = {
    "cobevt_abi_version": (ctypes.c_int, []),
    "cobevt_strerror": (ctypes.c_char_p, [ctypes.c_int]),
    "cobevt_conv2d_nhwc": (ctypes.c_int, [_vp, _vp, _vp, _vp, _vp, _vp, _vp, _vp, _c_int_p, _vp]),
    "cobevt_conv3x3_nhwc": (ctypes.c_int, [_vp, _vp, _vp, _vp, _vp, _c_int_p, _vp]),
    "cobevt_basicblock_nhwc": (ctypes.c_int, [_vp, _vp, _vp, _vp, _vp, _vp, _c_int_p, _vp]),
    "cobevt_dsblock_nhwc": (ctypes.c_int, [_vp, _vp, _vp, _vp, _vp, _vp, _vp, _vp, _c_int_p, _vp]),
    "cobevt_conv3x3_wfrag_nhwc": (ctypes.c_int, [_vp, _vp, _vp, _vp, _vp, _c_int_p, _vp]),
    "cobevt_conv3x3_ds_wfrag_nhwc": (ctypes.c_int, [_vp, _vp, _vp, _vp, _vp, _vp, _c_int_p, _vp]),
    "cobevt_stem_conv7x7s2_pool": (ctypes.c_int, [_vp, _vp, _vp, _vp, _c_int_p, _vp]),
    "cobevt_stem_conv7x7s2": (ctypes.c_int, [_vp, _vp, _vp, _vp, _c_int_p, _vp]),
    "cobevt_stem_conv7x7s2_pool_u8": (ctypes.c_int, [_vp, _vp, _vp, _vp, _vp, _c_int_p, _vp]),
    "cobevt_bev_embed_linear_rows": (ctypes.c_int, [_vp] * 9 + [_c_long_p, ctypes.c_float, _vp]),
    "cobevt_linear_rows_wfrag": (ctypes.c_int, [_vp, _vp, _vp, _vp, _vp, _vp, _vp, _c_long_p, ctypes.c_float, _vp]),
    "cobevt_linear_rows": (ctypes.c_int, [_vp, _vp, _vp, _vp, _vp, _vp, _vp, _vp, _vp, _c_long_p, ctypes.c_float, _vp]),
    "cobevt_attn_mlp_chain": (ctypes.c_int, [_vp] * 14 + [_c_int_p, ctypes.c_float, ctypes.c_float, ctypes.c_float, _vp]),
    "cobevt_pairwise_warp": (ctypes.c_int, [_vp] * 5 + [ctypes.c_int] * 6 + [ctypes.c_float, ctypes.c_float, _vp]),
    "cobevt_pairwise_warp_bwd": (ctypes.c_int, [_vp] * 4 + [ctypes.c_int] * 6 + [ctypes.c_float, ctypes.c_float, _vp]),
    "cobevt_agent_message_reduce": (ctypes.c_int, [_vp] * 5 + [ctypes.c_int] * 6 + [_vp]),
    "cobevt_gru_zero_state": (ctypes.c_int, [_vp, _vp, ctypes.c_int, ctypes.c_long, ctypes.c_int, _vp]),
    "cobevt_agent_softmax_sum": (ctypes.c_int, [_vp, ctypes.c_int, _vp, _vp, _vp, _vp] + [ctypes.c_int] * 6 + [_vp]),
    "cobevt_window_attention": (ctypes.c_int, [_vp, _vp, _vp, _vp, _vp, _vp, _c_int_p, ctypes.c_float, _vp]),
    "cobevt_window_attention_ksplit": (ctypes.c_int, [_vp] * 8 + [_c_int_p, ctypes.c_float, ctypes.c_int, ctypes.c_long, _vp]),
    "cobevt_window_attention_lse": (ctypes.c_int, [_vp, _vp, _vp, _vp, _vp, _vp, _vp, _c_int_p, ctypes.c_float, ctypes.c_float,
                                                   ctypes.c_uint, _vp, _vp]),
    "cobevt_conv3x3_head_nchw": (ctypes.c_int, [_vp, _vp, _vp, _vp] + [ctypes.c_int] * 6 + [_vp]),
    "cobevt_weighted_cross_entropy_bwd": (ctypes.c_int, [_vp] * 6 + [ctypes.c_int] * 3 + [_vp]),
    "cobevt_attention_dropout_mask": (ctypes.c_int, [ctypes.c_int] * 5 + [ctypes.c_float, ctypes.c_uint, _vp, _vp]),
    "cobevt_layernorm_bwd": (ctypes.c_int, [_vp] * 6 + [ctypes.c_int, ctypes.c_int, ctypes.c_float, _vp]),
    "cobevt_conv_wgrad": (ctypes.c_int, [_vp, _vp, _vp, _c_int_p, _vp]),
    "cobevt_conv_wgrad_blocked": (ctypes.c_int, [_vp, _vp, _vp, _c_int_p, _vp]),
    "cobevt_gelu": (ctypes.c_int, [_vp, _vp, _vp, ctypes.c_long, _vp]),
    "cobevt_layernorm_fwd_t": (ctypes.c_int, [_vp, _vp, _vp, _vp, ctypes.c_int, ctypes.c_int, ctypes.c_float, _c_int_p, _vp]),
    "cobevt_layernorm_bwd_t": (ctypes.c_int, [_vp] * 6 + [ctypes.c_int, ctypes.c_int, ctypes.c_float, _c_int_p, _vp]),
    "cobevt_gelu_bf16": (ctypes.c_int, [_vp, _vp, _vp, ctypes.c_long, _vp]),
    "cobevt_window_attention_bwd": (ctypes.c_int, [_vp] * 13 + [_c_int_p, ctypes.c_float, ctypes.c_float, ctypes.c_uint, _vp, _vp]),
    "cobevt_layernorm": (ctypes.c_int, [_vp, _vp, _vp, _vp, ctypes.c_int, ctypes.c_int, ctypes.c_int, ctypes.c_float,
                                        ctypes.c_int, ctypes.c_long, ctypes.c_long, ctypes.c_int, _vp]),
    "cobevt_fax_ray_embed": (ctypes.c_int, [_vp, _vp, _vp, _vp, _vp, _vp, ctypes.c_int, ctypes.c_int, ctypes.c_int,
                                            ctypes.c_int, _vp]),
    "cobevt_fax_bev_embed": (ctypes.c_int, [_vp, _vp, _vp, _vp, _vp, _vp, _vp, ctypes.c_int, ctypes.c_int, ctypes.c_int,
                                            ctypes.c_int, ctypes.c_int, ctypes.c_int, _vp]),
    "cobevt_maxpool3x3s2": (ctypes.c_int, [_vp, _vp, ctypes.c_int, ctypes.c_int, ctypes.c_int, ctypes.c_int, ctypes.c_int,
                                           _vp]),
    "cobevt_to_nhwc": (ctypes.c_int, [_vp, ctypes.c_int, _vp, ctypes.c_int, ctypes.c_int, ctypes.c_int, ctypes.c_int,
                                      ctypes.c_int, _c_long_p, _vp]),
    "cobevt_from_nhwc": (ctypes.c_int, [_vp, ctypes.c_int, _vp, ctypes.c_int, ctypes.c_int, ctypes.c_int, ctypes.c_int,
                                        ctypes.c_int, _c_long_p, _vp]),
    "cobevt_regroup": (ctypes.c_int, [_vp, _vp, _vp, _vp, ctypes.c_int, ctypes.c_int, ctypes.c_int, ctypes.c_long, _vp]),
    "cobevt_invert_small": (ctypes.c_int, [_vp, _vp, ctypes.c_int, ctypes.c_int, _vp]),
    "cobevt_resize_nhwc": (ctypes.c_int, [_vp, _vp] + [ctypes.c_int] * 8 + [_vp]),
    "cobevt_channel_affine": (ctypes.c_int, [_vp, _vp, _vp, _vp, ctypes.c_long, ctypes.c_int, ctypes.c_long, _vp]),
    "cobevt_sttf_warp": (ctypes.c_int, [_vp, _vp, _vp, _vp, _vp, _vp, _vp, ctypes.c_int, ctypes.c_int, ctypes.c_int, ctypes.c_int,
                                        ctypes.c_int, ctypes.c_int, ctypes.c_float, ctypes.c_float, _vp]),
    "cobevt_softmax_argmax": (ctypes.c_int, [_vp, _vp, _vp, ctypes.c_int, ctypes.c_int, ctypes.c_int, ctypes.c_int, _vp]),
    "cobevt_seg_class_counts": (ctypes.c_int, [_vp, _vp, _vp, ctypes.c_int, ctypes.c_int, ctypes.c_int, _vp]),
    "cobevt_weighted_cross_entropy": (ctypes.c_int, [_vp, _vp, _vp, _vp, _vp, ctypes.c_int, ctypes.c_int, ctypes.c_int, ctypes.c_int, _vp]),
    "cobevt_linear_rows_small_k": (ctypes.c_int, [_vp, _vp, _vp, _vp, _vp, _vp, _vp, _c_long_p, ctypes.c_float, _vp]),
    "cobevt_bev_embed_linear_rows_small_k": (ctypes.c_int, [_vp] * 9 + [_c_long_p, ctypes.c_float, _vp]),
    "cobevt_sigmoid_focal_loss": (ctypes.c_int, [_vp, _vp, _vp, _vp, _vp, _vp, ctypes.c_int, ctypes.c_int, ctypes.c_int, ctypes.c_int,
                                                 ctypes.c_int, ctypes.c_float, ctypes.c_float, ctypes.c_int, _vp]),
    "cobevt_iou_counts": (ctypes.c_int, [_vp, _vp, _vp, _vp, _vp, _vp, ctypes.c_int, ctypes.c_int, ctypes.c_int, ctypes.c_int,
                                         ctypes.c_int, ctypes.c_int, _vp]),
    "cobevt_agent_max": (ctypes.c_int, [_vp, _vp, ctypes.c_int, ctypes.c_int, ctypes.c_int, ctypes.c_long, _vp]),
    "cobevt_bottleneck_nhwc": (ctypes.c_int, [_vp] * 8 + [_c_int_p, _vp]),
    "cobevt_bottleneck_f32_nhwc": (ctypes.c_int, [_vp] * 9 + [_c_int_p, _vp]),
    "cobevt_attention_index_map": (ctypes.c_int, [_c_int_p, ctypes.c_int, _vp, _vp]),
    "cobevt_attention_bias_index": (ctypes.c_int, [_c_int_p, _c_int_p, ctypes.c_int, _vp, _vp]),
    "cobevt_depthwise_conv_nhwc": (ctypes.c_int, [_vp, _vp, _vp, _vp, _c_int_p, _vp]),
    "cobevt_spatial_mean_nhwc": (ctypes.c_int, [_vp, _vp, ctypes.c_int, ctypes.c_int, ctypes.c_int, ctypes.c_int, _vp]),
    "cobevt_se_gate": (ctypes.c_int, [_vp, _vp, _vp, _vp, _vp, _vp, ctypes.c_int, ctypes.c_int, ctypes.c_int, _vp]),
    "cobevt_mean_linear_rows_small_k": (ctypes.c_int, [_vp, _vp, _vp, _vp, _c_long_p, ctypes.c_float, _vp]),
    "cobevt_proj_chain": (ctypes.c_int, [_vp] * 10 + [_c_int_p, ctypes.c_float, _vp]),
    "cobevt_proj_chain_kv": (ctypes.c_int, [_vp, ctypes.POINTER(ctypes.c_void_p), _c_int_p, ctypes.c_float, _vp]),
    "cobevt_swap_fusion_stage": (ctypes.c_int, [_vp, _vp, _vp, _vp, _c_int_p, _vp, _vp, _vp, _vp, _vp, _vp, _vp, _vp, _vp, _vp, _c_int_p,
                                                ctypes.c_float, ctypes.c_float, ctypes.c_float, _vp]),
    "cobevt_channel_sums": (ctypes.c_int, [_vp, _vp, _vp, _vp, _vp, _vp, ctypes.c_int, ctypes.c_int, ctypes.c_long, ctypes.c_int, _vp]),
    "cobevt_f64_to_f32": (ctypes.c_int, [_vp, _vp, ctypes.c_int, _vp]),
    "cobevt_bn_batch_stats": (ctypes.c_int, [_vp] * 10 + [ctypes.c_int, ctypes.c_int, ctypes.c_long, ctypes.c_int, ctypes.c_float, ctypes.c_float, _vp, _vp]),
    "cobevt_bn_finalize": (ctypes.c_int, [_vp] * 10 + [ctypes.c_int, ctypes.c_long, ctypes.c_float, ctypes.c_float, ctypes.c_int, ctypes.c_int, _vp, _vp]),
    "cobevt_bn_apply": (ctypes.c_int, [_vp, _vp, _vp, _vp, _vp, ctypes.c_int, ctypes.c_long, ctypes.c_int, ctypes.c_int, _vp]),
    "cobevt_bn_backward": (ctypes.c_int, [_vp] * 9 + [ctypes.c_int, _vp, _vp, ctypes.c_int, ctypes.c_long, ctypes.c_int, ctypes.c_int,
                                          ctypes.c_int, _vp]),
    "cobevt_maxpool3x3s2_bwd": (ctypes.c_int, [_vp, _vp, _vp] + [ctypes.c_int] * 5 + [_vp]),
    "cobevt_maxpool3x3s2_bwd_t": (ctypes.c_int, [_vp, _vp, _vp] + [ctypes.c_int] * 5 + [_vp]),
    "cobevt_fax_bev_query_train": (ctypes.c_int, [_vp] * 6 + [_c_int_p, _vp]),
    "cobevt_fax_bev_query_train_bwd": (ctypes.c_int, [_vp] * 9 + [_c_int_p, _vp]),
    "cobevt_group_mean": (ctypes.c_int, [_vp, _vp, ctypes.c_int, ctypes.c_long, ctypes.c_int, ctypes.c_long, ctypes.c_int, _vp]),
    "cobevt_pixel_unshuffle2_nhwc": (ctypes.c_int, [_vp, _vp] + [ctypes.c_int] * 6 + [_vp]),
    "cobevt_upsample_nearest2_nhwc": (ctypes.c_int, [_vp, _vp] + [ctypes.c_int] * 6 + [_vp]),
    "cobevt_sttf_warp_bwd": (ctypes.c_int, [_vp, _vp, _vp, _vp] + [ctypes.c_int] * 5 + [ctypes.c_float, ctypes.c_float, _vp]),
    "cobevt_conv_weight_rows": (ctypes.c_int, [_vp, _vp, _vp, _c_int_p, _vp]),
    "cobevt_conv3_weight_operands": (ctypes.c_int, [_vp, _vp, _vp, _c_int_p, _vp]),
    "cobevt_conv3_weight_operands2": (ctypes.c_int, [_vp, ctypes.POINTER(ctypes.c_void_p), _c_int_p, _vp]),
    "cobevt_linear_weight_frags": (ctypes.c_int, [_vp, _vp, _vp, _c_int_p, _vp]),
    "cobevt_conv_wgrad3_chunks": (ctypes.c_int, [_c_int_p]),
    "cobevt_conv_wgrad3": (ctypes.c_int, [_vp, _vp, _vp, _vp, _c_int_p, _vp]),
    "cobevt_linear_wgrad_chunks": (ctypes.c_int, [_c_long_p]),
    "cobevt_linear_wgrad": (ctypes.c_int, [_vp, _vp, _vp, _vp, _c_long_p, _vp]),
    "cobevt_wgrad_block_operand": (ctypes.c_int, [_vp, _vp, _c_int_p, _vp]),
    "cobevt_swish": (ctypes.c_int, [_vp, _vp, _vp, ctypes.c_int, ctypes.c_long, _vp]),
    "cobevt_depthwise_wgrad": (ctypes.c_int, [_vp, _vp, _vp, _c_int_p, _vp]),
    "cobevt_resize_bilinear_bwd": (ctypes.c_int, [_vp, _vp] + [ctypes.c_int] * 7 + [_vp]),
    "cobevt_sigmoid_focal_loss_bwd": (ctypes.c_int, [_vp] * 7 + [ctypes.c_int] * 5 + [ctypes.c_float, ctypes.c_float, ctypes.c_int, _vp]),
    "cobevt_peer_window_alloc": (ctypes.c_int, [ctypes.c_long, ctypes.POINTER(_vp), _vp]),
    "cobevt_peer_window_open": (ctypes.c_int, [_vp, ctypes.POINTER(_vp)]),
    "cobevt_peer_window_close": (ctypes.c_int, [_vp]),
    "cobevt_peer_window_free": (ctypes.c_int, [_vp]),
    "cobevt_peer_window_status": (ctypes.c_int, [_vp, ctypes.c_long, _c_int_p, _c_int_p, _vp]),
    "cobevt_peer_window_status_async": (ctypes.c_int, [_vp, ctypes.c_long, _vp, _vp]),
    "cobevt_calibrate_mfma": (ctypes.c_int, [_vp, _vp, ctypes.c_int, ctypes.c_int, _vp]),
    "cobevt_calibrate_copy": (ctypes.c_int, [_vp, _vp, ctypes.c_long, _vp]),
    "cobevt_calibrate_clock_khz": (ctypes.c_int, [_c_int_p, _c_int_p]),
    "cobevt_peer_exchange": (ctypes.c_int, [_vp, ctypes.POINTER(_vp), ctypes.c_int, ctypes.c_int, ctypes.c_int, ctypes.c_long,
                                            _c_int_p, _c_int_p, ctypes.c_long, ctypes.c_long, _vp]),
    "cobevt_host_fetch": (ctypes.c_int, [_vp, _vp, ctypes.c_long, ctypes.c_int, _vp]),
    "cobevt_channel_gate_nhwc": (ctypes.c_int, [_vp, _vp, _vp, ctypes.c_int, ctypes.c_int, ctypes.c_int, ctypes.c_int, _vp]),
}

_libs = {}
_variant = ""
_encoder_variant = None
VARIANTS = ("", "f32s", "f32h")
LIB_PATH_F32S = os.environ.get("COBEVT_HIP_LIB_F32S") or os.path.join(_HERE, "csrc", "libcobevt_hip_f32s.so")
LIB_PATH_F32H = os.environ.get("COBEVT_HIP_LIB_F32H") or os.path.join(_HERE, "csrc", "libcobevt_hip_f32h.so")


class CobevtHipError(RuntimeError):
    pass


def set_variant(variant):
    global _variant
    if variant not in VARIANTS:
        raise CobevtHipError("unknown library variant %r" % (variant,))
    _variant = variant


def get_variant():
    return _variant


def set_encoder_variant(variant):
    global _encoder_variant
    if variant is not None and variant not in VARIANTS:
        raise CobevtHipError("unknown library variant %r" % (variant,))
    _encoder_variant = variant


def get_encoder_variant():
    return _encoder_variant


class encoder_scope(object):

    def __enter__(self):
        global _variant
        self.prev = _variant
        if _encoder_variant is not None:
            _variant = _encoder_variant
        return self

    def __exit__(self, *exc):
        global _variant
        _variant = self.prev
        return False


def load(variant=None):
    v = _variant if variant is None else variant
    lib = _libs.get(v)
    if lib is not None:
        return lib
    path = {"f32s": LIB_PATH_F32S, "f32h": LIB_PATH_F32H}.get(v, LIB_PATH)
    if not os.path.exists(path):
        raise CobevtHipError(
            "%s not found at %s — build it with `python -m cobevt_amd.build` "
            "(there is no CPU / eager fallback for the hot path)" % (os.path.basename(path), path))
    lib = ctypes.CDLL(path)
    for name, (res, args) in SIGNATURES.items():
        fn = getattr(lib, name)
        fn.restype = res
        fn.argtypes = args
    if lib.cobevt_abi_version() != 1:
        raise CobevtHipError("%s ABI version mismatch" % os.path.basename(path))
    _libs[v] = lib
    return lib


def check(rc, what):
    if rc != 0:
        msg = load().cobevt_strerror(rc).decode()
        raise CobevtHipError("%s failed: %s (code %d)" % (what, msg, rc))
```

### cobevt_amd/ops.py

```python
import ctypes
import os
import math

import torch

from . import lib as _L
from .lib import CobevtHipError

BF16, FP32 = 0, 1
USE_CONV3X3 = True
USE_CONV3_S2 = True
USE_CONV3_SMALL_TILES = True
USE_CONV3_DS = True
USE_CONV3_WFRAG = True
CONV3_VARIANT = 0
USE_GEMM_ROWS = True
USE_GEMM_ROWS2 = False
USE_GEMM_ROWS3 = True
GEMM_ROWS3_MIN_M = 0
GEMM_ROWS3_MAX_K = 512
GEMM_ROWS3_STRIDED = 1
GEMM_ROWS3_ROWS64_MIN_M = 0
USE_STEM_POOL = True
USE_STEM = True
ROW_CHAIN_ROWS = 0
USE_ROW_CHAIN = True
USE_BOTTLENECK_F32 = True
USE_GEMM_ROWS3_F32 = True
USE_ROW_CHAIN_F32 = True
BASICBLOCK_TILE_ROWS = 0
USE_BASICBLOCK = True
BASICBLOCK_MAX_C = 128
USE_DSBLOCK = True
USE_EMBED_GEMM = False
USE_EMBED_GEMM3 = True
USE_CHAIN_NEXT = True
USE_HEAD_CONV = True
USE_PROJ_CHAIN = True
USE_PROJ_CHAIN_KV = True
USE_PROJ_CHAIN_WAVE = True
USE_SWAP_STAGE = True
USE_BOTTLENECK = True
ATTN_VARIANT = 0
USE_ATTN_BIG_RESIDENT = False
ATTN_KSPLIT = 2
ATTN_QSPLIT = 0


def dcode(dtype):
    if dtype == torch.bfloat16:
        return BF16
    if dtype == torch.float32:
        return FP32
    raise CobevtHipError("compute dtype must be torch.bfloat16 or torch.float32, got %s" % dtype)


def _apply_env_flags():
    for item in os.environ.get("COBEVT_FLAGS", "").split(","):
        if "=" in item:
            k, v = item.split("=", 1)
            k = k.strip()
            if k not in globals() or not (k.startswith("USE_") or k in ("CONV3_VARIANT", "BASICBLOCK_TILE_ROWS", "ROW_CHAIN_ROWS", "GEMM_ROWS3_MIN_M", "GEMM_ROWS3_MAX_K", "GEMM_ROWS3_STRIDED", "GEMM_ROWS3_ROWS64_MIN_M", "BASICBLOCK_MAX_C", "ATTN_VARIANT", "ATTN_QSPLIT", "ATTN_KSPLIT")):
                raise CobevtHipError("COBEVT_FLAGS: unknown switch %r" % k)
            globals()[k] = int(v) if not k.startswith("USE_") else bool(int(v))


_apply_env_flags()


def _p(t):
    return None if t is None else ctypes.c_void_p(t.data_ptr())


def _stream():
    return ctypes.c_void_p(torch.cuda.current_stream().cuda_stream)


def _need_cuda(*ts):
    for t in ts:
        if t is not None and not t.is_cuda:
            raise CobevtHipError("cobevt_amd kernels need tensors on a ROCm device (got a CPU tensor); "
                                 "there is no CPU fallback")


def _ints(vals):
    return (ctypes.c_int * len(vals))(*[int(v) for v in vals])


_PROFILE = None


class LaunchProfile(object):

    def __init__(self):
        self.records = []

    def __enter__(self):
        global _PROFILE
        _PROFILE = self
        return self

    def __exit__(self, *exc):
        global _PROFILE
        _PROFILE = None

    def summary(self, by_shape=False):
        torch.cuda.synchronize()
        out = {}
        for fam, flops, nbytes, e0, e1 in self.records:
            if not by_shape:
                fam = fam.split("|")[0]
            d = out.setdefault(fam, {"calls": 0, "ms": 0.0, "flops": 0.0, "bytes": 0.0})
            d["calls"] += 1
            d["ms"] += e0.elapsed_time(e1)
            d["flops"] += flops
            d["bytes"] += nbytes
        return out


class _Timed(object):
    __slots__ = ("fam", "flops", "nbytes", "e0")

    def __init__(self, fam, flops, nbytes):
        self.fam, self.flops, self.nbytes = fam, flops, nbytes

    def __enter__(self):
        self.e0 = torch.cuda.Event(enable_timing=True)
        self.e0.record()

    def __exit__(self, *exc):
        e1 = torch.cuda.Event(enable_timing=True)
        e1.record()
        _PROFILE.records.append((self.fam, self.flops, self.nbytes, self.e0, e1))


class _NoTime(object):
    def __enter__(self):
        pass

    def __exit__(self, *exc):
        pass


_NOTIME = _NoTime()


def _timed(fam, flops_fn):
    if _PROFILE is None:
        return _NOTIME
    f, b = flops_fn()
    return _Timed(fam, f, b)


def bn_affine(bn):
    g = bn.weight.detach().double() if bn.weight is not None else torch.ones_like(bn.running_var).double()
    b = bn.bias.detach().double() if bn.bias is not None else torch.zeros_like(bn.running_var).double()
    s = g / torch.sqrt(bn.running_var.detach().double() + bn.eps)
    return s, b - bn.running_mean.detach().double() * s


class ConvPlan(object):

    def __init__(self, weight, bias=None, bn=None, pre_bn=None, pre_relu=False, stride=1, pad=0, act=0,
                 upsample=False, store_mode=0, dtype=torch.bfloat16, device="cuda", smallc=False, ln=None,
                 ln_folded_eps=None, pad_br=None):
        w = weight.detach().double().cpu()
        if w.dim() == 2:
            w = w[:, :, None, None]
        cout, cin, kh, kw = w.shape
        asym = pad_br is not None and int(pad_br) != int(pad)
        self.pad_br = int(pad if pad_br is None else pad_br)
        b = bias.detach().double().cpu() if bias is not None else torch.zeros(cout, dtype=torch.float64)
        has_bias = bias is not None or bn is not None
        self.has_ln, self.ln_eps = False, 0.0
        if ln_folded_eps is not None:
            if ln is not None or kh != 1 or kw != 1 or bn is not None or pre_bn is not None:
                raise CobevtHipError("ln_folded_eps applies to plain Linear / 1x1 layers without another ln")
            self.has_ln, self.ln_eps = True, float(ln_folded_eps)
        if ln is not None:
            if kh != 1 or kw != 1 or bn is not None or pre_bn is not None:
                raise CobevtHipError("LayerNorm folding applies to plain Linear / 1x1 layers")
            g, be = ln.weight.detach().double().cpu(), ln.bias.detach().double().cpu()
            b = b + (w[:, :, 0, 0] @ be)
            w = w * g[None, :, None, None]
            has_bias = True
            self.has_ln, self.ln_eps = True, float(ln.eps)
        if bn is not None:
            s, sh = bn_affine(bn)
            s, sh = s.cpu(), sh.cpu()
            w = w * s[:, None, None, None]
            b = b * s + sh
        self.dtype = dtype
        self.code = dcode(dtype)
        bke = 32 if self.code == BF16 else 16
        ch = 8 if self.code == BF16 else 4
        K = kh * kw * cin
        kpad = (K + bke - 1) // bke * bke
        wk = torch.zeros(cout, kpad, dtype=torch.float64)
        wk[:, :K] = w.permute(0, 2, 3, 1).reshape(cout, K)
        self.wgt = wk.to(torch.float32).to(dtype).to(device).contiguous()
        self.bias = b.to(torch.float32).to(device).contiguous() if has_bias else None
        self.pre_scale = self.pre_shift = None
        if pre_bn is not None:
            s, sh = bn_affine(pre_bn)
            self.pre_scale = s.to(torch.float32).to(device).contiguous()
            self.pre_shift = sh.to(torch.float32).to(device).contiguous()
        self.pre_relu = int(bool(pre_relu))
        self.klut = None
        self.smallc = int(bool(smallc))
        if not smallc and cin % ch != 0:
            raise CobevtHipError("Cin=%d must be a multiple of %d for the %s kernel (use smallc=True for image "
                                 "inputs)" % (cin, ch, dtype))
        if smallc:
            k = torch.arange(kpad)
            tap, c = k // cin, k % cin
            code = ((tap // kw) << 20) | ((tap % kw) << 10) | c
            code[k >= K] = -1
            self.klut = code.to(torch.int32).to(device).contiguous()
        self.wgt3, self.cc3 = None, 0
        if kh == 3 and kw == 3 and int(stride) in (1, 2) and int(pad) == 1 and not asym and int(act) <= 2 and not smallc and pre_bn is None \
                and int(store_mode) in (0, 1) and not (int(stride) == 2 and (upsample or int(store_mode) != 0)):
            cands = (64, 32) if self.code == BF16 else (32, 16)
            for cc in cands:
                if cin % cc == 0:
                    w3 = w.permute(0, 2, 3, 1).reshape(cout, 9, cin // cc, cc).permute(0, 2, 1, 3)
                    if int(stride) == 1:
                        self.wgt3 = w3.to(torch.float32).to(dtype).to(device).contiguous()
                    self.cc3 = cc
                    break
        self.wfrag, self.coutp3 = None, 0
        if self.cc3 and self.cc3 == (64 if self.code == BF16 else 32):
            cc, coutp = self.cc3, (cout + 127) // 128 * 128
            wp = torch.zeros(coutp, cin // cc, 9, cc, dtype=torch.float64)
            wp[:cout] = w.permute(0, 2, 3, 1).reshape(cout, 9, cin // cc, cc).permute(0, 2, 1, 3)
            wf = wp.reshape(coutp // 32, 32, cin // cc, 9, 4, 2, ch).permute(0, 2, 3, 4, 5, 1, 6)
            self.wfrag = wf.to(torch.float32).to(dtype).to(device).contiguous()
            self.coutp3 = coutp
        self.wgt_stem = None
        if smallc and kh == 7 and kw == 7 and int(stride) == 2 and int(pad) == 3 and not asym and int(act) <= 2 and cin == 3 and pre_bn is None \
                and int(store_mode) == 0 and not upsample and cout % (8 if self.code == BF16 else 4) == 0:
            ws = torch.zeros(cout, 4, 4, 16, dtype=torch.float64)
            for a in range(4):
                for bb in range(4):
                    for dy in range(2):
                        for dx in range(2):
                            ih, iw = 2 * a + dy - 1, 2 * bb + dx - 1
                            if 0 <= ih < 7 and 0 <= iw < 7:
                                ws[:, a, bb, dy * 6 + dx * 3:dy * 6 + dx * 3 + 3] = w[:, :, ih, iw]
            self.wgt_stem = ws.reshape(cout, 256).to(torch.float32).to(dtype).to(device).contiguous()
        self.wgt_rows, self.kp_rows, self.wfrag_rows = None, 0, None
        if kh == 1 and kw == 1 and int(stride) in (1, 2) and int(pad) == 0 and not asym and not smallc and int(store_mode) == 0 \
                and not upsample:
            tk = 128 if self.code == BF16 else 64
            kp = (K + tk - 1) // tk * tk
            wr = torch.zeros(cout, kp, dtype=torch.float64)
            wr[:, :K] = w.reshape(cout, K)
            self.wgt_rows = wr.to(torch.float32).to(dtype).to(device).contiguous()
            self.kp_rows = kp
            eg = 8 if self.code == BF16 else 4
            npad = (cout + 127) // 128 * 128
            wp_ = torch.zeros(npad, kp, dtype=torch.float64)
            wp_[:cout] = wr
            wf = wp_.reshape(npad // 32, 32, kp // (2 * eg), 2, eg).permute(0, 2, 3, 1, 4)
            self.wfrag_rows = wf.to(torch.float32).to(dtype).to(device).contiguous()
        self.wgt_head = None
        if kh == 3 and kw == 3 and int(stride) == 1 and int(pad) == 1 and not asym and not smallc and int(store_mode) == 2 and int(act) == 0 \
                and not upsample and pre_bn is None and cout <= 4 and cin * (2 if self.code == BF16 else 4) <= 256 and cin % ch == 0:
            self.wgt_head = w.permute(0, 2, 3, 1).reshape(cout, 9 * cin).to(torch.float32).to(device).contiguous()
        self.cin, self.cout, self.kh, self.kw = cin, cout, kh, kw
        self.K, self.kpad = K, kpad
        self.stride, self.pad, self.act = int(stride), int(pad), int(act)
        self.upsample = int(bool(upsample))
        self.store_mode = int(store_mode)

    def out_hw(self, h, w):
        hv, wv = (2 * h, 2 * w) if self.upsample else (h, w)
        return ((hv + self.pad + self.pad_br - self.kh) // self.stride + 1,
                (wv + self.pad + self.pad_br - self.kw) // self.stride + 1)


def ln_fusable(plan):
    return USE_GEMM_ROWS and plan.wgt_rows is not None and plan.K <= (128 if plan.code == BF16 else 64)


def conv3_tiling(n, ho, wo, cin, cout, cc, cus=256, stride=1, bf16=True, packed=0):
    if stride == 1:
        if cout <= 32 and bf16 and cc == 64:
            nstrips = n * (-(-ho // 2)) * (-(-wo // 16))
            best = None
            for mt in ((1, 2, 3, 4, 5) if USE_CONV3_SMALL_TILES else (3, 4, 5)):
                blocks = -(-nstrips // mt) * -(-cout // 32)
                cost = -(-blocks // (2 * cus)) * (6000 + 9 * (cin // cc) * mt * 80)
                if best is None or cost < best[0]:
                    best = (cost, 100 + 10 * mt + 3)
            return best[1]
        if cout < 64:
            return 0
        th, bn = (16, 64) if cout <= 64 else (8, 128)
        blocks_old = n * (-(-ho // th)) * (-(-wo // 16)) * (-(-cout // bn))
        if blocks_old >= 2 * cus and not (packed and cout >= 128):
            return 0
    nstrips = n * (-(-ho // 2)) * (-(-wo // 16))
    nsteps = 9 * (cin // cc)
    best = None
    for bn64 in ((1,) if cout <= 64 else (0, 1)):
        tile_n = 64 if bn64 else 128
        for mt in (3, 4, 5, 6):
            blocks = -(-nstrips // mt) * -(-cout // tile_n)
            per_step = int(40 * (float(packed) if packed else 1.0)) if (packed and not bn64) else 40
            cost = -(-blocks // cus) * (12000 + nsteps * mt * (tile_n // 32) * per_step
                                       + (1500 * mt * (cin // cc) if stride == 2 else 0))
            if best is None or cost < best[0]:
                best = (cost, 100 + 10 * mt + bn64, blocks)
    if USE_CONV3_SMALL_TILES and stride == 1 and bf16 and cc == 64 and not packed and best[2] < cus:
        for mt in (1, 2, 3, 4, 5):
            blocks = -(-nstrips // mt) * -(-cout // 32)
            cost = -(-blocks // (2 * cus)) * (6000 + nsteps * mt * 80)
            if cost < best[0]:
                best = (cost, 100 + 10 * mt + 3, blocks)
    return best[1]


def conv2d(x, plan, residual=None, out=None):
    _need_cuda(x, residual, out)
    ln = plan.has_ln
    if ln and not ln_fusable(plan):
        x = layernorm(x, None, None, plan.ln_eps)
        ln = False
    n, h, w, cin = x.shape
    if cin != plan.cin or not x.is_contiguous():
        raise CobevtHipError("conv2d: bad input %s (contiguous=%s) for Cin=%d" % (tuple(x.shape), x.is_contiguous(), plan.cin))
    if x.dtype != (torch.float32 if plan.smallc else plan.dtype):
        raise CobevtHipError("conv2d: input dtype %s does not match plan (%s, smallc=%d)" % (x.dtype, plan.dtype, plan.smallc))
    ho, wo = plan.out_hw(h, w)
    sm = plan.store_mode
    out_h, out_w = ho, wo
    if out is None:
        if sm == 0:
            out = torch.empty((n, ho, wo, plan.cout), device=x.device, dtype=plan.dtype)
        elif sm == 1:
            out = torch.empty((n, ho // 2, wo // 2, plan.cout * 4), device=x.device, dtype=plan.dtype)
        elif sm == 2:
# ... 417 lines not shown
def agent_max(x):
    _need_cuda(x)
    if not x.is_contiguous():
        raise CobevtHipError("agent_max: input must be contiguous")
    b, l = x.shape[:2]
    out = torch.empty((b,) + tuple(x.shape[2:]), device=x.device, dtype=x.dtype)
    per = out[0].numel()
    rc = _L.load().cobevt_agent_max(_p(x), _p(out), dcode(x.dtype), b, l, per, _stream())
    _L.check(rc, "cobevt_agent_max")
    return out


def ray_embed(i_inv, e_inv, image_plane, w_img, w_cam, hw, dim, dtype):
    _need_cuda(i_inv, e_inv, image_plane, w_img, w_cam)
    bn = i_inv.shape[0]
    out = torch.empty((bn, hw, dim), device=i_inv.device, dtype=dtype)
    rc = _L.load().cobevt_fax_ray_embed(_p(i_inv), _p(e_inv), _p(image_plane), _p(w_img), _p(w_cam), _p(out),
                                        dcode(dtype), bn, hw, dim, _stream())
    _L.check(rc, "cobevt_fax_ray_embed")
    return out


def batch_broadcast(x):
    return x.dim() >= 2 and x.shape[0] > 1 and x.stride(0) == 0 and x[0].is_contiguous()


def bev_embed(e_inv, world, w_bev, b_bev, w_cam, x, n):
    _need_cuda(e_inv, world, w_bev, b_bev, w_cam, x)
    b, hw, d = x.shape
    bcast = batch_broadcast(x)
    if not bcast:
        x = x.contiguous()
    out = torch.empty((b, n, hw, d), device=x.device, dtype=x.dtype)
    rc = _L.load().cobevt_fax_bev_embed(_p(e_inv), _p(world), _p(w_bev), _p(b_bev), _p(w_cam), _p(x), _p(out),
                                        dcode(x.dtype), b, n, hw, d, int(bcast), _stream())
    _L.check(rc, "cobevt_fax_bev_embed")
    return out


def bev_embed_linear(e_inv, world, w_bev, b_bev, w_cam, x, n, plan):
    b, hw, d = x.shape
    bcast = batch_broadcast(x)
    wave_level = d == 128 and plan.cout == 128 and b * n <= 32
    fused3 = ((USE_EMBED_GEMM3 == 2 or (USE_EMBED_GEMM3 and wave_level)) and USE_GEMM_ROWS3 and plan.code == BF16 and plan.has_ln
              and plan.K == d and d <= 128 and d % 8 == 0
              and plan.kp_rows == 128 and plan.wfrag_rows is not None and hw % 32 == 0 and plan.stride == 1
              and plan.pre_scale is None and plan.act == 0 and plan.cout % 8 == 0 and (bcast or x.is_contiguous()))
    if fused3:
        _need_cuda(e_inv, world, w_bev, b_bev, w_cam, x)
        out = torch.empty((b, n, hw, plan.cout), device=x.device, dtype=x.dtype)
        dims = (ctypes.c_long * 8)(plan.code, b, n, hw, d, plan.cout, 1, int(bcast))

        def cost3():
            m = b * n * hw
            return 2.0 * m * plan.cout * d, float((hw if bcast else x.numel() // d) * d * 2 + plan.cout * d * 2 + out.numel() * 2)

        with _timed("gemm_rows|embed %d->%d M=%d ln r32" % (d, plan.cout, b * n * hw), cost3):
            rc = _L.load().cobevt_bev_embed_linear_rows_small_k(_p(e_inv), _p(world), _p(w_bev), _p(b_bev), _p(w_cam), _p(x),
                                                                _p(plan.wfrag_rows), _p(plan.bias), _p(out), dims,
                                                                ctypes.c_float(plan.ln_eps), _stream())
        _L.check(rc, "cobevt_bev_embed_linear_rows_small_k")
        return out
    fused = (USE_EMBED_GEMM and USE_GEMM_ROWS and plan.has_ln and ln_fusable(plan) and plan.K == d and hw % 128 == 0
             and plan.stride == 1 and plan.pre_scale is None and plan.act == 0 and x.is_contiguous())
    if not fused:
        return linear(bev_embed(e_inv, world, w_bev, b_bev, w_cam, x, n), plan)
    _need_cuda(e_inv, world, w_bev, b_bev, w_cam, x)
    out = torch.empty((b, n, hw, plan.cout), device=x.device, dtype=x.dtype)
    dims = (ctypes.c_long * 8)(plan.code, b, n, hw, d, plan.cout, plan.kp_rows, 1)

    def cost():
        m = b * n * hw
        esz = 2 if plan.code == BF16 else 4
        return 2.0 * m * plan.cout * d, float(x.numel() * esz + plan.cout * d * esz + out.numel() * esz)

    with _timed("gemm_rows|embed %d->%d M=%d ln" % (d, plan.cout, b * n * hw), cost):
        rc = _L.load().cobevt_bev_embed_linear_rows(_p(e_inv), _p(world), _p(w_bev), _p(b_bev), _p(w_cam), _p(x),
                                                    _p(plan.wgt_rows), _p(plan.bias), _p(out), dims,
                                                    ctypes.c_float(plan.ln_eps), _stream())
    _L.check(rc, "cobevt_bev_embed_linear_rows")
    return out


def stem_pool(x, plan):
    _need_cuda(x)
    n, h, w, cin = x.shape
    fused = (USE_STEM_POOL and USE_STEM and plan.wgt_stem is not None and plan.cout == 64 and plan.act == 1
             and h % 4 == 0 and w % 4 == 0 and x.dtype == torch.float32 and x.is_contiguous())
    if not fused:
        return maxpool3x3s2(conv2d(x, plan))
    out = torch.empty((n, h // 4, w // 4, 64), device=x.device, dtype=plan.dtype)
    dims = _ints([plan.code, n, h, w])

    def cost():
        esz = 2 if plan.code == BF16 else 4
        return 2.0 * n * (h // 2) * (w // 2) * 64 * 147, float(x.numel() * 4 + out.numel() * esz)

    with _timed("stem7x7|pool %dx%dx%d" % (n, h, w), cost):
        rc = _L.load().cobevt_stem_conv7x7s2_pool(_p(x), _p(plan.wgt_stem), _p(plan.bias), _p(out), dims, _stream())
    _L.check(rc, "cobevt_stem_conv7x7s2_pool")
    return out


def stem_pool_u8(x, lut, plan):
    _need_cuda(x, lut)
    n, h, w, cin = x.shape
    if not (plan.wgt_stem is not None and plan.cout == 64 and plan.act == 1 and h % 4 == 0 and w % 4 == 0 and cin == 3
            and x.dtype == torch.uint8 and x.is_contiguous() and lut.dtype == torch.float32 and tuple(lut.shape) == (3, 256)
            and lut.is_contiguous()):
        raise CobevtHipError("stem_pool_u8: needs contiguous uint8 frames (N, H, W, 3) with H, W multiples of 4, a (3, 256) fp32 table "
                             "and the ResNet stem plan; got %s %s" % (tuple(x.shape), x.dtype))
    out = torch.empty((n, h // 4, w // 4, 64), device=x.device, dtype=plan.dtype)
    dims = _ints([plan.code, n, h, w])

    def cost():
        esz = 2 if plan.code == BF16 else 4
        return 2.0 * n * (h // 2) * (w // 2) * 64 * 147, float(x.numel() + out.numel() * esz)

    with _timed("stem7x7|pool u8 %dx%dx%d" % (n, h, w), cost):
        rc = _L.load().cobevt_stem_conv7x7s2_pool_u8(_p(x), _p(lut), _p(plan.wgt_stem), _p(plan.bias), _p(out), dims, _stream())
    _L.check(rc, "cobevt_stem_conv7x7s2_pool_u8")
    return out


def host_fetch(src_pinned, dst, blocks=0):
    _need_cuda(dst)
    if src_pinned.is_cuda or not src_pinned.is_pinned():
        raise CobevtHipError("host_fetch: the source must be a pinned host tensor (tensor.pin_memory())")
    nbytes = dst.numel() * dst.element_size()
    if (tuple(src_pinned.shape) != tuple(dst.shape) or src_pinned.dtype != dst.dtype or not src_pinned.is_contiguous() or not dst.is_contiguous()
            or nbytes % 16):
        raise CobevtHipError("host_fetch: contiguous tensors of one shape / dtype, a multiple of 16 bytes")
    rc = _L.load().cobevt_host_fetch(ctypes.c_void_p(src_pinned.data_ptr()), _p(dst), nbytes, int(blocks), _stream())
    _L.check(rc, "cobevt_host_fetch")
    return dst


def maxpool3x3s2(x):
    _need_cuda(x)
    n, h, w, c = x.shape
    ho, wo = (h + 2 - 3) // 2 + 1, (w + 2 - 3) // 2 + 1
    out = torch.empty((n, ho, wo, c), device=x.device, dtype=x.dtype)
    rc = _L.load().cobevt_maxpool3x3s2(_p(x), _p(out), dcode(x.dtype), n, h, w, c, _stream())
    _L.check(rc, "cobevt_maxpool3x3s2")
    return out


def to_nhwc(x, dtype):
    _need_cuda(x)
    n, c, h, w = x.shape
    v = x.permute(0, 2, 3, 1)
    if x.dtype == dtype and v.is_contiguous():
        return v
    out = torch.empty((n, h, w, c), device=x.device, dtype=dtype)
    strides = (ctypes.c_long * 4)(*x.stride())
    rc = _L.load().cobevt_to_nhwc(_p(x), dcode(x.dtype), _p(out), dcode(dtype), n, c, h, w, strides, _stream())
    _L.check(rc, "cobevt_to_nhwc")
    return out


def from_nhwc(x, dtype):
    _need_cuda(x)
    n, h, w, c = x.shape
    out = torch.empty((n, c, h, w), device=x.device, dtype=dtype)
    strides = (ctypes.c_long * 4)(*out.stride())
    rc = _L.load().cobevt_from_nhwc(_p(x), dcode(x.dtype), _p(out), dcode(dtype), n, c, h, w, strides, _stream())
    _L.check(rc, "cobevt_from_nhwc")
    return out


def copy_into_interior(x, dst):
    _need_cuda(x, dst)
    n, h, w, c = x.shape
    if dst.dtype != x.dtype or not x.is_contiguous() or not dst.is_contiguous() or dst.shape[0] != n or dst.shape[3] != c \
            or dst.shape[1] < h or dst.shape[2] < w:
        raise CobevtHipError("copy_into_interior: dst must be a contiguous (N, >= h, >= w, C) map of x's dtype")
    sN, sH, sW, sC = dst.stride()
    strides = (ctypes.c_long * 4)(sN, sC, sH, sW)
    rc = _L.load().cobevt_from_nhwc(_p(x), dcode(x.dtype), _p(dst), dcode(dst.dtype), n, c, h, w, strides, _stream())
    _L.check(rc, "cobevt_from_nhwc")
    return dst


def regroup(x, record_len, max_cav):
    _need_cuda(x, record_len)
    if record_len.dtype != torch.int32 or not x.is_contiguous():
        raise CobevtHipError("regroup: record_len must be int32 on the device and x contiguous")
    b = record_len.shape[0]
    per = x[0].numel()
    out = torch.empty((b, max_cav) + tuple(x.shape[1:]), device=x.device, dtype=x.dtype)
    mask = torch.empty((b, max_cav), device=x.device, dtype=torch.float32)
    rc = _L.load().cobevt_regroup(_p(x), _p(record_len), _p(out), _p(mask), dcode(x.dtype), b, max_cav, per, _stream())
    _L.check(rc, "cobevt_regroup")
    return out, mask


def sttf_warp(x, tmat, cav_mask, discrete_ratio, downsample_rate, want_mask=True, record_len=None, max_cav=None):
    _need_cuda(x, tmat, cav_mask, record_len)
    if tmat.dtype != torch.float32 or not tmat.is_contiguous() or not x.is_contiguous():
        raise CobevtHipError("sttf_warp: tmat must be contiguous fp32, x contiguous")
    if record_len is not None:
        if record_len.dtype != torch.int32 or x.dim() != 4:
            raise CobevtHipError("sttf_warp: record_len must be int32 on the device and x (N, H, W, C)")
        b, l = record_len.shape[0], int(max_cav)
        _, h, w, c = x.shape
        out = torch.empty((b, l, h, w, c), device=x.device, dtype=x.dtype)
        cav = torch.empty((b, l), device=x.device, dtype=torch.float32)
    else:
        b, l, h, w, c = x.shape
        out = torch.empty_like(x)
        cav = None
    if tuple(tmat.shape[:2]) != (b, l):
        raise CobevtHipError("sttf_warp: tmat must be (B, L, 4, 4)")
    com = torch.empty((b, h, w, 1, l), device=x.device, dtype=torch.float32) if want_mask else None
    rc = _L.load().cobevt_sttf_warp(_p(x), _p(tmat), _p(cav_mask), _p(out), _p(com), _p(record_len), _p(cav),
                                    dcode(x.dtype), b, l, h, w, c,
                                    ctypes.c_float(discrete_ratio), ctypes.c_float(downsample_rate), _stream())
    _L.check(rc, "cobevt_sttf_warp")
    return (out, com, cav) if record_len is not None else (out, com)


def pairwise_warp(x, pairwise, record_len, max_cav, discrete_ratio, downsample_rate):
    _need_cuda(x, pairwise, record_len)
    if record_len.dtype != torch.int32 or x.dim() != 4 or pairwise.dtype != torch.float32:
        raise CobevtHipError("pairwise_warp: record_len int32 on the device, x (N, H, W, C), pairwise fp32")
    b, l = record_len.shape[0], int(max_cav)
    _, h, w, c = x.shape
    if tuple(pairwise.shape) != (b, l, l, 4, 4):
        raise CobevtHipError("pairwise_warp: pairwise must be (B, max_cav, max_cav, 4, 4)")
    nb = torch.empty((b, l, l, h, w, c), device=x.device, dtype=x.dtype)
    roi = torch.empty((b, l, l, h, w), device=x.device, dtype=torch.float32)
    rc = _L.load().cobevt_pairwise_warp(_p(x), _p(pairwise.contiguous()), _p(record_len), _p(nb), _p(roi), dcode(x.dtype), b, l, h, w, c,
                                        ctypes.c_float(discrete_ratio), ctypes.c_float(downsample_rate), _stream())
    _L.check(rc, "cobevt_pairwise_warp")
    return nb, roi


def agent_message_reduce(msg, ego, roi, record_len, mode):
    _need_cuda(msg, ego, roi, record_len)
    b, l, _, h, w, c = msg.shape
    out = torch.zeros_like(ego)
    rc = _L.load().cobevt_agent_message_reduce(_p(msg), _p(ego), _p(roi), _p(record_len), _p(out), dcode(msg.dtype), b, l, h * w, c,
                                               {"avg": 0, "max": 1}[mode], _stream())
    _L.check(rc, "cobevt_agent_message_reduce")
    return out


def gru_zero_state(x):
    _need_cuda(x)
    c = x.shape[-1] // 2
    out = torch.empty(x.shape[:-1] + (c,), device=x.device, dtype=x.dtype)
    rc = _L.load().cobevt_gru_zero_state(_p(x), _p(out), dcode(x.dtype), x.numel() // (2 * c), c, _stream())
    _L.check(rc, "cobevt_gru_zero_state")
    return out


def agent_softmax_sum(score, nb, roi, record_len, n_agents, use_mask=True):
    _need_cuda(score, nb, roi, record_len)
    b, l, _, h, w, c = nb.shape
    out = torch.zeros((n_agents, h, w, c), device=nb.device, dtype=nb.dtype)
    rc = _L.load().cobevt_agent_softmax_sum(_p(score), score.shape[-1], _p(nb), _p(roi), _p(record_len), _p(out), dcode(nb.dtype),
                                            b, l, h * w, c, int(bool(use_mask)), _stream())
    _L.check(rc, "cobevt_agent_softmax_sum")
    return out


def invert_small(m):
    _need_cuda(m)
    d = m.shape[-1]
    x = m.to(torch.float32).contiguous()
    out = torch.empty_like(x)
    rc = _L.load().cobevt_invert_small(_p(x), _p(out), x.numel() // (d * d), d, _stream())
    _L.check(rc, "cobevt_invert_small")
    return out


def resize_nhwc(x, ho, wo, mode):
    _need_cuda(x)
    n, h, w, c = x.shape
    out = torch.empty((n, ho, wo, c), device=x.device, dtype=x.dtype)
    rc = _L.load().cobevt_resize_nhwc(_p(x), _p(out), dcode(x.dtype), n, h, w, c, ho, wo, 0 if mode == "nearest" else 1,
                                      _stream())
    _L.check(rc, "cobevt_resize_nhwc")
    return out


def channel_affine(x, scale, shift):
    _need_cuda(x, scale, shift)
    if x.dtype != torch.float32 or not x.is_contiguous():
        x = x.to(torch.float32).contiguous()
    out = torch.empty_like(x)
    n, c = x.shape[0], x.shape[1]
    rc = _L.load().cobevt_channel_affine(_p(x), _p(scale), _p(shift), _p(out), n, c, x.numel() // (n * c), _stream())
    _L.check(rc, "cobevt_channel_affine")
    return out


def chain_next_fusable(plan_n, c):
    return (plan_n is not None and plan_n.wfrag_rows is not None and plan_n.stride == 1 and plan_n.kp_rows == 128 and plan_n.K == c
            and plan_n.cout % 8 == 0 and plan_n.cout <= 768 and plan_n.pre_scale is None and not plan_n.pre_relu
            and plan_n.act <= 2)


def attn_mlp_chain(a, skip, plan_p, plan_1, plan_2, post_ln=None, next_plan=None):
    _need_cuda(a, skip)
    c, hd = plan_p.cout, plan_1.cout
    skip_rows = 0
    if skip is not None and batch_broadcast(skip) and skip.shape == a.shape:
        skip_rows = skip[0].numel() // c
    f32 = a.dtype == torch.float32
    fusable = (USE_ROW_CHAIN and (a.dtype == torch.bfloat16 or (f32 and USE_ROW_CHAIN_F32 and c == 128 and hd == 256 and plan_2.kp_rows == 256))
               and plan_p.wfrag_rows is not None and plan_1.wfrag_rows is not None
               and plan_2.wfrag_rows is not None and plan_2.kp_rows <= 256 and plan_1.has_ln and plan_1.act == 2 and plan_p.act == 0
               and plan_2.act == 0 and not plan_p.has_ln and not plan_2.has_ln and plan_p.K == c and plan_1.K == c
               and plan_2.K == hd and plan_2.cout == c and c <= 128 and c % 8 == 0 and hd <= 256 and hd % 8 == 0
               and plan_p.kp_rows == 128 and plan_1.kp_rows == 128 and a.shape[-1] == c and a.is_contiguous()
               and (skip is None or skip.dtype == a.dtype)
               and (skip is None or skip_rows or (skip.is_contiguous() and skip.shape == a.shape)))
    if not fusable:
        y = linear(a, plan_p, residual=skip.contiguous() if skip is not None else None)
        z = linear(linear(y, plan_1), plan_2, residual=y)
        z = layernorm(z, post_ln[0], post_ln[1], post_ln[2]) if post_ln is not None else z
        return (z, linear(z, next_plan)) if next_plan is not None else z
    m = a.numel() // c
    out = torch.empty_like(a)
    fuse_next = USE_CHAIN_NEXT and chain_next_fusable(next_plan, c)
    nn_ = next_plan.cout if fuse_next else 0
    out_next = torch.empty(a.shape[:-1] + (nn_,), device=a.device, dtype=a.dtype) if fuse_next else None
    dims = _ints([plan_p.code, m, c, hd, plan_2.kp_rows, nn_, int(next_plan.has_ln) if fuse_next else 0,
                  next_plan.act if fuse_next else 0, ROW_CHAIN_ROWS, skip_rows])
    pg, pb, pe = post_ln if post_ln is not None else (None, None, 0.0)

    def cost():
        flops = 2.0 * m * (c * c + 2 * c * hd + c * nn_)
        esz = a.element_size()
        return flops, float((2 * m + (0 if skip is None else skip_rows or m)) * c * esz + m * nn_ * esz + (c * c + 2 * c * hd + c * nn_) * esz)

    with _timed("row_chain|C%d H%d M=%d%s%s" % (c, hd, m, " post" if post_ln is not None else "",
                                                  " +next%d" % nn_ if fuse_next else ""), cost):
        rc = _L.load().cobevt_attn_mlp_chain(_p(a), _p(skip), _p(out), _p(plan_p.wfrag_rows), _p(plan_p.bias),
                                             _p(plan_1.wfrag_rows), _p(plan_1.bias), _p(plan_2.wfrag_rows), _p(plan_2.bias),
                                             _p(pg), _p(pb), _p(next_plan.wfrag_rows) if fuse_next else None,
                                             _p(next_plan.bias) if fuse_next else None, _p(out_next), dims,
                                             ctypes.c_float(plan_1.ln_eps), ctypes.c_float(pe),
                                             ctypes.c_float(next_plan.ln_eps if fuse_next else 0.0), _stream())
    _L.check(rc, "cobevt_attn_mlp_chain")
    if next_plan is None:
        return out
    return out, (out_next if fuse_next else linear(out, next_plan))


def proj_chain_fusable(x, plan_p, next_plan, residual):
    c = x.shape[-1]
    return (USE_PROJ_CHAIN and x.dtype == torch.bfloat16 and c == 128 and x.is_contiguous() and plan_p.wfrag_rows is not None
            and plan_p.kp_rows == 128 and plan_p.K == c and plan_p.cout == c and plan_p.act == 0 and not plan_p.has_ln
            and plan_p.stride == 1 and chain_next_fusable(next_plan, c)
            and (residual is None or (residual.is_contiguous() and residual.shape == x.shape and residual.dtype == x.dtype)))


def proj_chain(x, plan_p, next_plan, residual=None, out_next=None):
    _need_cuda(x, residual)
    c, nn_ = 128, next_plan.cout
    m = x.numel() // c
    if out_next is None:
        out_next = torch.empty(x.shape[:-1] + (nn_,), device=x.device, dtype=x.dtype)
    elif out_next.numel() != m * nn_ or not out_next.is_contiguous() or out_next.dtype != x.dtype:
        raise CobevtHipError("proj_chain: `out_next` must be a contiguous (.., %d) buffer of dtype %s" % (nn_, x.dtype))
    dims = _ints([0, m, c, nn_, int(next_plan.has_ln), next_plan.act, 0, plan_p.pre_relu, 0 if USE_PROJ_CHAIN_WAVE else 1])

    def cost():
        return 2.0 * m * (c * c + c * nn_), float(m * (c * (2 if residual is not None else 1) + nn_) * 2 + (c * c + c * nn_) * 2)

    with _timed("row_chain|proj C%d M=%d +next%d" % (c, m, nn_), cost):
        rc = _L.load().cobevt_proj_chain(_p(x), _p(plan_p.pre_scale), _p(plan_p.pre_shift), _p(residual), _p(plan_p.wfrag_rows),
                                         _p(plan_p.bias), None, _p(next_plan.wfrag_rows), _p(next_plan.bias), _p(out_next), dims,
                                         ctypes.c_float(next_plan.ln_eps), _stream())
    _L.check(rc, "cobevt_proj_chain")
    return out_next


def proj_chain_kv_fusable(x, plan_key, plan_val, next_key, next_val, residual):
    k = x.shape[-1]
    if not (USE_PROJ_CHAIN_KV and x.dtype == torch.bfloat16 and x.is_contiguous() and k in (256, 384, 512)):
        return False
    for pl in (plan_key, plan_val):
        if pl is None:
            continue
        if not (pl.wfrag_rows is not None and pl.kp_rows == k and pl.K == k and pl.cout == 128 and pl.act == 0 and not pl.has_ln
                and pl.stride == 1):
            return False
    for pn in (next_key, next_val):
        if not (chain_next_fusable(pn, 128) and pn.act == 0):
            return False
    return (plan_val is not None and next_key.cout == next_val.cout and next_key.has_ln == next_val.has_ln and next_key.ln_eps == next_val.ln_eps
            and (residual is None or (plan_key is not None and residual.is_contiguous() and residual.dtype == x.dtype
                                      and tuple(residual.shape) == tuple(x.shape[:-1]) + (128,))))


def proj_chain_kv(x, plan_key, plan_val, next_key, next_val, residual=None, out_k=None, out_v=None):
    _need_cuda(x, residual)
    k, nn_ = x.shape[-1], next_key.cout
    m = x.numel() // k
    outs = []
    for o in (out_k, out_v):
        if o is None:
            o = torch.empty(x.shape[:-1] + (nn_,), device=x.device, dtype=x.dtype)
        elif o.numel() != m * nn_ or not o.is_contiguous() or o.dtype != x.dtype:
            raise CobevtHipError("proj_chain_kv: result buffers must be contiguous (.., %d) of dtype %s" % (nn_, x.dtype))
        outs.append(o)
    ptrs = (ctypes.c_void_p * 18)()
    for s_, (pp, pn, res, o) in enumerate(((plan_key, next_key, residual, outs[0]), (plan_val, next_val, None, outs[1]))):
        vals = (pp.pre_scale, pp.pre_shift, pp.wfrag_rows, pp.bias, res, pn.wfrag_rows, pn.bias, None, o)
        for j, t in enumerate(vals):
            ptrs[9 * s_ + j] = None if t is None else t.data_ptr()
    dims = _ints([0, m, k, nn_, int(next_key.has_ln), 2, plan_key.pre_relu, 0, plan_val.pre_relu, 0])

    def cost():
        return 2.0 * 2 * m * (k * 128 + 128 * nn_), float(m * (k + (128 if residual is not None else 0) + 2 * nn_) * 2 + 2 * (k * 128 + 128 * nn_) * 2)

    with _timed("row_chain|proj kv K%d M=%d +next%d" % (k, m, nn_), cost):
        rc = _L.load().cobevt_proj_chain_kv(_p(x), ptrs, dims, ctypes.c_float(next_key.ln_eps), _stream())
    _L.check(rc, "cobevt_proj_chain_kv")
    return outs[0], outs[1]


def swap_stage_fusable(qkv, x, tmap, heads, plan_p, plan_1, plan_2, next_plan, mask):
    c = x.shape[-1]
    nk = tmap[1] * tmap[4] * tmap[5]
    return (USE_SWAP_STAGE and x.dtype == torch.bfloat16 and qkv.dtype == torch.bfloat16 and c == 128 and heads == 4
            and tmap[0] in (0, 1) and nk <= 384 and x.is_contiguous() and qkv.is_contiguous() and qkv.shape[-1] == 3 * c
            and plan_p.wfrag_rows is not None and plan_1.wfrag_rows is not None and plan_2.wfrag_rows is not None
            and plan_p.kp_rows == 128 and plan_1.kp_rows == 128 and plan_2.kp_rows in (128, 256) and plan_1.has_ln
            and plan_1.act == 2 and plan_p.act == 0 and plan_2.act == 0 and not plan_p.has_ln and not plan_2.has_ln
            and plan_p.K == c and plan_1.K == c and plan_2.K == plan_1.cout and plan_2.cout == c and plan_1.cout % 8 == 0
            and plan_1.cout <= 256 and plan_p.cout == c
            and (next_plan is None or (chain_next_fusable(next_plan, c) and next_plan.cout <= 384 and next_plan.has_ln
                                       and next_plan.act == 0))
            and (mask is None or (mask.dtype == torch.float32 and mask.is_contiguous())))


SWAP_STAGE_BIAS_FLOATS = 10240


def swap_stage(qkv, x, tmap, batch, heads, scale, bias_table, bias_L, mask, plan_p, plan_1, plan_2, next_plan=None):
    _need_cuda(qkv, x, bias_table, mask)
    c, hd = 128, plan_1.cout
    out = torch.empty_like(x)
    nn_ = next_plan.cout if next_plan is not None else 0
    qkv_next = torch.empty(x.shape[:-1] + (nn_,), device=x.device, dtype=x.dtype) if next_plan is not None else None
    bias_rows = (2 * bias_L - 1) * (2 * tmap[4] - 1) * (2 * tmap[5] - 1)
    if bias_table.numel() != SWAP_STAGE_BIAS_FLOATS or bias_table.dtype != torch.float32 or not bias_table.is_contiguous():
        raise CobevtHipError("swap_stage: bias table must be the flat fp32 image of stage_bias_table()")
    dims = _ints([0, batch, c, heads, hd, plan_2.kp_rows, nn_, bias_rows, bias_L])
    m = x.numel() // c
    nk = tmap[1] * tmap[4] * tmap[5]

    def cost():
        flops = 4.0 * m * nk * c + 2.0 * m * (c * c + 2 * c * hd + c * nn_)
        return flops, float(m * (3 * c + 2 * c + nn_) * 2 + (c * c + 2 * c * hd + c * nn_) * 2)

    with _timed("swap_stage|mode%d M=%d Nk%d H%d%s" % (tmap[0], m, nk, hd, " +next%d" % nn_ if nn_ else ""), cost):
        rc = _L.load().cobevt_swap_fusion_stage(
            _p(qkv), _p(x), _p(out), _p(qkv_next), _ints(tmap), _p(bias_table), _p(mask), _p(plan_p.wfrag_rows), _p(plan_p.bias),
            _p(plan_1.wfrag_rows), _p(plan_1.bias), _p(plan_2.wfrag_rows), _p(plan_2.bias),
            _p(next_plan.wfrag_rows) if next_plan is not None else None, _p(next_plan.bias) if next_plan is not None else None,
            dims, ctypes.c_float(scale), ctypes.c_float(plan_1.ln_eps), ctypes.c_float(next_plan.ln_eps if next_plan is not None else 0.0),
            _stream())
    _L.check(rc, "cobevt_swap_fusion_stage")
    return out, qkv_next


def softmax_argmax(seg_logits):
    _need_cuda(seg_logits)
    if seg_logits.dim() != 4:
        raise CobevtHipError("softmax_argmax expects (N, C, H, W) logits, got %s" % (tuple(seg_logits.shape),))
    x = seg_logits.contiguous()
    n, c, h, w = x.shape
    prob = torch.empty((n, c, h, w), device=x.device, dtype=torch.float32)
    seg_map = torch.empty((n, h, w), device=x.device, dtype=torch.int64)
    rc = _L.load().cobevt_softmax_argmax(_p(x), _p(prob), _p(seg_map), dcode(x.dtype), n, c, h * w, _stream())
    _L.check(rc, "cobevt_softmax_argmax")
    return prob, seg_map


def seg_class_counts(pred, gt, num_classes):
    _need_cuda(pred, gt)
    if pred.shape != gt.shape or pred.dim() != 3:
        raise CobevtHipError("seg_class_counts expects two (N, H, W) maps, got %s and %s" % (tuple(pred.shape), tuple(gt.shape)))
    p64, g64 = pred.to(torch.int64).contiguous(), gt.to(torch.int64).contiguous()
    n, h, w = p64.shape
    counts = torch.empty((n, num_classes + 1, 3), device=pred.device, dtype=torch.int64)
    rc = _L.load().cobevt_seg_class_counts(_p(p64), _p(g64), _p(counts), n, h * w, num_classes, _stream())
    _L.check(rc, "cobevt_seg_class_counts")
    host = counts.cpu()
    if int(host[:, num_classes, 0].sum()) or int(host[:, num_classes, 1].sum()):
        raise CobevtHipError("seg_class_counts: labels outside [0, %d)" % num_classes)
    return host[:, :num_classes]


class DepthwisePlan(object):

    def __init__(self, weight, bn=None, stride=1, pad=(0, 0), act=0, dtype=torch.bfloat16, device="cuda"):
        w = weight.detach().double().cpu()
        c, one, kh, kw = w.shape
        if one != 1 or kh != kw:
            raise CobevtHipError("DepthwisePlan expects a (C, 1, k, k) weight")
        b = torch.zeros(c, dtype=torch.float64)
        if bn is not None:
            s_, sh = bn_affine(bn)
            w = w * s_.cpu()[:, None, None, None]
            b = sh.cpu().double()
        if c % 8 != 0:
            raise CobevtHipError("depthwise conv needs a multiple of 8 channels, got %d" % c)
        self.c, self.k, self.stride, self.act = c, kh, int(stride), int(act)
        self.pad0, self.pad1 = int(pad[0]), int(pad[1])
        self.dtype, self.code = dtype, dcode(dtype)
        self.wgt = w[:, 0].permute(1, 2, 0).reshape(kh * kw, c).to(torch.float32).to(device).contiguous()
        self.bias = b.to(torch.float32).to(device).contiguous()

    def out_hw(self, h, w):
        return ((h + self.pad0 + self.pad1 - self.k) // self.stride + 1, (w + self.pad0 + self.pad1 - self.k) // self.stride + 1)


def depthwise_conv(x, plan):
    _need_cuda(x)
    n, h, w, c = x.shape
    if c != plan.c or x.dtype != plan.dtype or not x.is_contiguous():
        raise CobevtHipError("depthwise_conv: bad input %s %s for C=%d %s" % (tuple(x.shape), x.dtype, plan.c, plan.dtype))
    ho, wo = plan.out_hw(h, w)
    out = torch.empty((n, ho, wo, c), device=x.device, dtype=plan.dtype)
    dims = _ints([plan.code, n, h, w, c, plan.k, plan.stride, plan.pad0, plan.pad0, ho, wo, plan.act])

    def cost():
        esz = 2 if plan.code == BF16 else 4
        return 2.0 * n * ho * wo * c * plan.k * plan.k, float((x.numel() + out.numel()) * esz)

    with _timed("depthwise|%dx%d s%d C%d %dx%d" % (plan.k, plan.k, plan.stride, c, h, w), cost):
        rc = _L.load().cobevt_depthwise_conv_nhwc(_p(x), _p(plan.wgt), _p(plan.bias), _p(out), dims, _stream())
    _L.check(rc, "cobevt_depthwise_conv_nhwc")
    return out


def spatial_mean(x):
    _need_cuda(x)
    n, h, w, c = x.shape
    if not x.is_contiguous():
        raise CobevtHipError("spatial_mean: input must be contiguous channels-last")
    out = torch.empty((n, c), device=x.device, dtype=torch.float32)
    rc = _L.load().cobevt_spatial_mean_nhwc(_p(x), _p(out), dcode(x.dtype), n, h * w, c, _stream())
    _L.check(rc, "cobevt_spatial_mean_nhwc")
    return out


def se_gate(mean, w_reduce, b_reduce, w_expand, b_expand):
    _need_cuda(mean, w_reduce, b_reduce, w_expand, b_expand)
    n, c = mean.shape
    cs = w_reduce.shape[0]
    if tuple(w_reduce.shape) != (cs, c) or tuple(w_expand.shape) != (c, cs) or b_reduce.numel() != cs or b_expand.numel() != c:
        raise CobevtHipError("se_gate: inconsistent shapes")
    gate = torch.empty((n, c), device=mean.device, dtype=torch.float32)
    rc = _L.load().cobevt_se_gate(_p(mean), _p(w_reduce), _p(b_reduce), _p(w_expand), _p(b_expand), _p(gate), n, c, cs, _stream())
    _L.check(rc, "cobevt_se_gate")
    return gate


def channel_gate(x, gate):
    _need_cuda(x, gate)
    n, h, w, c = x.shape
    if tuple(gate.shape) != (n, c) or gate.dtype != torch.float32 or not x.is_contiguous() or not gate.is_contiguous():
        raise CobevtHipError("channel_gate: gate must be (N, C) fp32 for a contiguous (N, H, W, C) map")
    out = torch.empty_like(x)
    rc = _L.load().cobevt_channel_gate_nhwc(_p(x), _p(gate), _p(out), dcode(x.dtype), n, h * w, c, _stream())
    _L.check(rc, "cobevt_channel_gate_nhwc")
    return out


_DEFERRED_LABELS = []


_LABEL_RING = 32


def _label_word(c):
    global _LABEL_NEXT
    if len(_DEFERRED_LABELS) < _LABEL_RING:
        if torch.cuda.is_current_stream_capturing():
            if not _DEFERRED_LABELS:
                return None
        else:
            _DEFERRED_LABELS.append([torch.zeros(1, dtype=torch.float32).pin_memory(), c])
            return _DEFERRED_LABELS[-1][0]
    _LABEL_NEXT = (_LABEL_NEXT + 1) % len(_DEFERRED_LABELS)
    ent = _DEFERRED_LABELS[_LABEL_NEXT]
    ent[1] = c
    return ent[0]


_LABEL_NEXT = -1


def _check_deferred_labels():
    for word, c in _DEFERRED_LABELS:
        bad = int(word[0])
        if bad:
            word[0] = 0.0
            raise CobevtHipError("weighted_cross_entropy: %d target labels outside [0, %d) in an earlier call (only -100 is ignored)"
                                 % (bad, c))


def check_deferred_label_errors():
    torch.cuda.synchronize()
    _check_deferred_labels()


def weighted_cross_entropy(logits, target, weight, want_stats=False):
    _need_cuda(logits, target)
    if logits.dim() != 4 or tuple(target.shape) != (logits.shape[0],) + tuple(logits.shape[2:]):
        raise CobevtHipError("weighted_cross_entropy expects (N, C, H, W) logits and an (N, H, W) target")
    x, y = logits.contiguous(), target.to(torch.int64).contiguous()
    n, c, h, w = x.shape
    wt = weight.to(device=x.device, dtype=torch.float32).contiguous()
    if wt.numel() != c:
        raise CobevtHipError("weighted_cross_entropy: %d class weights for %d classes" % (wt.numel(), c))
    scratch = torch.empty(3 * n * ((h * w + 4095) // 4096), device=x.device, dtype=torch.float32)
    out = torch.empty(4, device=x.device, dtype=torch.float32)
    rc = _L.load().cobevt_weighted_cross_entropy(_p(x), _p(y), _p(wt), _p(scratch), _p(out), dcode(x.dtype), n, c, h * w, _stream())
    _L.check(rc, "cobevt_weighted_cross_entropy")
    _check_deferred_labels()
    host_word = _label_word(c)
    if host_word is not None:
        host_word.copy_(out[3:4], non_blocking=True)
    return (out[0], out, x, y, wt) if want_stats else out[0]


def iou_counts(pred, label, visibility, label_indices, thresholds, min_visibility):
    _need_cuda(pred)
    n, c, hw = pred.shape
    dev = pred.device
    label = label.to(device=dev, dtype=torch.float32).contiguous()
    nl = label.shape[1]
    if len(label_indices) != c or nl > 32 or tuple(label.shape) != (n, nl, hw):
        raise CobevtHipError("iou_counts: %d prediction channels need %d label groups over at most 32 label channels" % (c, c))
    masks = torch.tensor([sum(1 << int(l) for l in group) for group in label_indices], dtype=torch.int64).to(torch.int32).to(dev)
    thr = torch.as_tensor(thresholds, dtype=torch.float32).to(dev).contiguous()
    counts = torch.zeros((thr.numel(), 3), device=dev, dtype=torch.int64)
    vis = None
    mv = -1
    if min_visibility is not None:
        vis = visibility.to(device=dev, dtype=torch.uint8).contiguous()
        mv = int(min_visibility)
    rc = _L.load().cobevt_iou_counts(_p(pred.contiguous()), _p(label), _p(vis), _p(masks), _p(thr), _p(counts), n, c, nl, hw,
                                     thr.numel(), mv, _stream())
    _L.check(rc, "cobevt_iou_counts")
    return counts.cpu()


def sigmoid_focal_loss_mean(pred, label, visibility, label_indices, min_visibility, alpha, gamma):
    _need_cuda(pred)
    n, c, hw = pred.shape
    dev = pred.device
    label = label.to(device=dev, dtype=torch.float32).contiguous()
    nl = label.shape[1]
    soft = label_indices is None
    if (soft and nl != c) or (not soft and len(label_indices) != c) or nl > 32 or tuple(label.shape) != (n, nl, hw):
        raise CobevtHipError("sigmoid_focal_loss_mean: inconsistent prediction / label channels")
    masks = None
    if not soft:
        masks = torch.tensor([sum(1 << int(l) for l in g) for g in label_indices], dtype=torch.int64).to(torch.int32).to(dev)
    vis, mv = None, -1
    if min_visibility is not None:
        vis, mv = visibility.to(device=dev, dtype=torch.uint8).contiguous(), int(min_visibility)
    scratch = torch.empty(2 * n * ((hw + 2047) // 2048), device=dev, dtype=torch.float32)
    out = torch.empty(3, device=dev, dtype=torch.float32)
    rc = _L.load().cobevt_sigmoid_focal_loss(_p(pred.float().contiguous()), _p(label), _p(vis), _p(masks), _p(scratch), _p(out), n, c, nl,
                                             hw, mv, ctypes.c_float(alpha), ctypes.c_float(gamma), int(soft), _stream())
    _L.check(rc, "cobevt_sigmoid_focal_loss")
    return out[0]
```

### include/cobevt_hip.h

```cpp
#ifndef COBEVT_HIP_H
#define COBEVT_HIP_H

#include <hip/hip_runtime_api.h>

#ifdef __cplusplus
extern "C" {
#endif

#define COBEVT_OK 0
#define COBEVT_ERR_ARG 1
#define COBEVT_ERR_SHAPE 2
#define COBEVT_ERR_LAUNCH 3
#define COBEVT_ERR_UNSUPPORTED 4

int cobevt_abi_version(void);
const char* cobevt_strerror(int code);

int cobevt_conv2d_nhwc(const void* in, const void* wgt, const float* bias, const void* residual,
                       const float* pre_scale, const float* pre_shift, const int* klut, void* out,
                       const int* dims, hipStream_t stream);

int cobevt_conv3x3_nhwc(const void* in, const void* wgt, const float* bias, const void* residual, void* out,
                        const int* dims, hipStream_t stream);

int cobevt_conv3x3_wfrag_nhwc(const void* in, const void* wfrag, const float* bias, const void* residual, void* out,
                              const int* dims, hipStream_t stream);

int cobevt_conv3x3_ds_wfrag_nhwc(const void* in, const void* in2, const void* wfrag, const float* bias, const float* bias2, void* out,
                                 const int* dims, hipStream_t stream);

int cobevt_basicblock_nhwc(const void* in, const void* wfrag1, const float* bias1, const void* wfrag2, const float* bias2,
                           void* out, const int* dims, hipStream_t stream);

int cobevt_dsblock_nhwc(const void* in, const void* wfrag1, const float* bias1, const void* wfrag2, const float* bias2,
                        const void* wfrag_ds, const float* bias_ds, void* out, const int* dims, hipStream_t stream);

int cobevt_stem_conv7x7s2(const float* in, const void* wgt, const float* bias, void* out, const int* dims,
                          hipStream_t stream);

int cobevt_stem_conv7x7s2_pool(const float* in, const void* wgt, const float* bias, void* out, const int* dims,
                               hipStream_t stream);

int cobevt_stem_conv7x7s2_pool_u8(const unsigned char* in, const float* lut, const void* wgt, const float* bias, void* out,
                                  const int* dims, hipStream_t stream);

int cobevt_linear_rows(const void* in, const void* wgt, const float* bias, const void* residual, const float* ln_gamma,
                       const float* ln_beta, const float* pre_scale, const float* pre_shift, void* out, const long* dims,
                       float ln_eps, hipStream_t stream);

int cobevt_linear_rows_wfrag(const void* in, const void* wfrag, const float* bias, const void* residual,
                             const float* pre_scale, const float* pre_shift, void* out, const long* dims, float ln_eps,
                             hipStream_t stream);

int cobevt_attn_mlp_chain(const void* a, const void* skip, void* out, const void* wp, const float* bp, const void* w1,
                          const float* b1, const void* w2, const float* b2, const float* post_gamma,
                          const float* post_beta, const void* wnext, const float* bnext, void* out_next, const int* dims,
                          float eps1, float eps_post, float eps_next, hipStream_t stream);

int cobevt_window_attention(const void* q, const void* k, const void* v, void* out, const float* bias_table,
                            const float* mask, const int* dims, float scale, hipStream_t stream);

int cobevt_window_attention_lse(const void* q, const void* k, const void* v, void* out, float* lse, const float* bias_table,
                                const float* mask, const int* dims, float scale, float drop_p, unsigned drop_seed,
                                const unsigned* drop_seed_dev, hipStream_t stream);
int cobevt_window_attention_bwd(const void* q, const void* k, const void* v, const void* out, const float* lse,
                                const void* dout, const float* dlse, void* dq, void* dk, void* dv, float* dbias, const float* bias_table,
                                const float* mask, const int* dims, float scale, float drop_p, unsigned drop_seed,
                                const unsigned* drop_seed_dev, hipStream_t stream);
int cobevt_attention_dropout_mask(int B, int L, int heads, int Nq, int Nk, float drop_p, unsigned drop_seed, unsigned char* keep,
                                  hipStream_t stream);

int cobevt_layernorm_bwd(const float* x, const float* dy, const float* gamma, float* dx, float* dgamma, float* dbeta, int rows,
                         int C, float eps, hipStream_t stream);
int cobevt_gelu(const float* x, const float* dy, float* out, long n, hipStream_t stream);
int cobevt_layernorm_fwd_t(const void* x, const float* gamma, const float* beta, void* y, int rows, int C, float eps, const int* dtypes,
                           hipStream_t stream);
int cobevt_layernorm_bwd_t(const void* x, const void* dy, const float* gamma, void* dx, float* dgamma, float* dbeta, int rows, int C,
                           float eps, const int* dtypes, hipStream_t stream);
int cobevt_gelu_bf16(const void* x, const void* dy, void* out, long n, hipStream_t stream);
int cobevt_conv_wgrad(const void* x, const void* dy, float* dw, const int* dims, hipStream_t stream);
int cobevt_conv_wgrad_blocked(const void* xb, const void* db, float* dw, const int* dims, hipStream_t stream);

int cobevt_agent_max(const void* in, void* out, int dtype, int B, int L, long per, hipStream_t stream);

int cobevt_bottleneck_nhwc(const void* in, const void* w1, const void* w2, const void* w3, const float* b1, const float* b2,
                           const float* b3, void* out, const int* dims, hipStream_t stream);

int cobevt_bottleneck_f32_nhwc(const void* in, const void* y1, const void* w1frag, const float* b1, const void* w2frag, const float* b2,
                               const void* w3frag, const float* b3, void* out, const int* dims, hipStream_t stream);

int cobevt_attention_index_map(const int* map8, int B, int* rows, hipStream_t stream);
int cobevt_attention_bias_index(const int* qmap8, const int* kmap8, int bias_L, int* idx, hipStream_t stream);

int cobevt_layernorm(const void* in, const float* gamma, const float* beta, void* out, int dtype, int rows, int C,
                     float eps, int navg, long avg_stride, long in_batch_stride, int rows_per_batch,
                     hipStream_t stream);

int cobevt_fax_ray_embed(const float* I_inv, const float* E_inv, const float* image_plane, const float* w_img,
                         const float* w_cam, void* out, int dtype, int BN, int hw, int D, hipStream_t stream);

int cobevt_fax_bev_embed(const float* E_inv, const float* world, const float* w_bev, const float* b_bev,
                         const float* w_cam, const void* x, void* out, int dtype, int B, int n, int hw, int D,
                         int x_bcast, hipStream_t stream);

int cobevt_bev_embed_linear_rows(const float* E_inv, const float* world, const float* w_bev, const float* b_bev,
                                 const float* w_cam, const void* x, const void* wgt, const float* bias, void* out,
                                 const long* dims, float ln_eps, hipStream_t stream);

int cobevt_maxpool3x3s2(const void* in, void* out, int dtype, int N, int H, int W, int C, hipStream_t stream);

int cobevt_to_nhwc(const void* in, int in_dtype, void* out, int out_dtype, int N, int C, int H, int W,
                   const long* strides, hipStream_t stream);
int cobevt_from_nhwc(const void* in, int in_dtype, void* out, int out_dtype, int N, int C, int H, int W,
                     const long* strides, hipStream_t stream);

int cobevt_pairwise_warp(const void* x, const float* pairwise, const int* record_len, void* nb, float* roi, int dtype, int B, int L,
                         int H, int W, int C, float discrete_ratio, float downsample_rate, hipStream_t stream);
int cobevt_pairwise_warp_bwd(const void* dnb, const float* pairwise, const int* record_len, float* dx, int dtype, int B, int L, int H,
                             int W, int C, float discrete_ratio, float downsample_rate, hipStream_t stream);
int cobevt_agent_message_reduce(const void* msg, const void* ego, const float* roi, const int* record_len, void* out, int dtype,
                                int B, int L, int HW, int C, int mode, hipStream_t stream);
int cobevt_gru_zero_state(const void* in, void* out, int dtype, long rows, int C, hipStream_t stream);
int cobevt_agent_softmax_sum(const void* score, int lds, const void* nb, const float* roi, const int* record_len, void* out, int dtype,
                             int B, int L, int HW, int C, int use_mask, hipStream_t stream);

int cobevt_regroup(const void* in, const int* record_len, void* out, float* mask, int dtype, int B, int max_cav,
                   long elems_per_agent, hipStream_t stream);

int cobevt_sttf_warp(const void* x, const float* tmat, const float* cav_mask, void* out, float* com_mask,
                     const int* record_len, float* cav_out, int dtype, int B, int L, int H, int W, int C,
                     float discrete_ratio, float downsample_rate, hipStream_t stream);

int cobevt_invert_small(const float* in, float* out, int n, int dim, hipStream_t stream);

int cobevt_resize_nhwc(const void* in, void* out, int dtype, int N, int H, int W, int C, int Ho, int Wo, int mode,
                       hipStream_t stream);

int cobevt_channel_affine(const float* in, const float* scale, const float* shift, float* out, long N, int C, long HW,
                          hipStream_t stream);

int cobevt_host_fetch(const void* host_src, void* dst, long bytes, int blocks, hipStream_t stream);


int cobevt_softmax_argmax(const void* logits, float* prob, long long* map, int dtype, int N, int C, int hw,
                          hipStream_t stream);

int cobevt_seg_class_counts(const long long* pred, const long long* gt, unsigned long long* counts, int N, int hw, int K,
                            hipStream_t stream);

int cobevt_weighted_cross_entropy(const void* logits, const long long* target, const float* weight, float* scratch, float* out,
                                  int dtype, int N, int C, int hw, hipStream_t stream);
int cobevt_weighted_cross_entropy_bwd(const float* logits, const long long* target, const float* weight, const float* stats,
                                      const float* upstream, float* dlogits, int N, int C, int hw, hipStream_t stream);

int cobevt_conv3x3_head_nchw(const void* in, const float* wgt, const float* bias, float* out, int dtype, int N, int H, int W, int Cin,
                             int Cout, hipStream_t stream);

int cobevt_linear_rows_small_k(const void* in, const void* wfrag, const float* bias, const void* residual, const float* pre_scale,
                               const float* pre_shift, void* out, const long* dims, float ln_eps, hipStream_t stream);

int cobevt_bev_embed_linear_rows_small_k(const float* E_inv, const float* world, const float* w_bev, const float* b_bev,
                                         const float* w_cam, const void* x, const void* wfrag, const float* bias, void* out,
                                         const long* dims, float ln_eps, hipStream_t stream);

int cobevt_sigmoid_focal_loss(const float* pred, const float* label, const unsigned char* visibility, const unsigned int* label_mask,
                              float* scratch, float* out, int N, int C, int NL, int hw, int min_visibility, float alpha,
                              float gamma, int soft_label, hipStream_t stream);

int cobevt_iou_counts(const float* pred, const float* label, const unsigned char* visibility, const unsigned int* label_mask,
                      const float* thresholds, unsigned long long* counts, int N, int C, int NL, int hw, int T,
                      int min_visibility, hipStream_t stream);


int cobevt_depthwise_conv_nhwc(const void* in, const float* wgt, const float* bias, void* out, const int* dims,
                               hipStream_t stream);

int cobevt_spatial_mean_nhwc(const void* in, float* out, int dtype, int N, int hw, int C, hipStream_t stream);

int cobevt_se_gate(const float* mean, const float* w_reduce, const float* b_reduce, const float* w_expand,
                   const float* b_expand, float* gate, int N, int C, int Cs, hipStream_t stream);

int cobevt_channel_gate_nhwc(const void* in, const float* gate, void* out, int dtype, int N, int hw, int C,
                             hipStream_t stream);

int cobevt_mean_linear_rows_small_k(const void* in, const void* wfrag, const float* bias, void* out, const long* dims,
                                    float ln_eps, hipStream_t stream);

int cobevt_window_attention_ksplit(const void* q, const void* k, const void* v, void* out, const float* bias_table,
                                   const float* mask, void* part_out, float* part_lse, const int* dims, float scale,
                                   int ksplit, long out_rows, hipStream_t stream);

int cobevt_proj_chain(const void* a, const float* pre_scale, const float* pre_shift, const void* skip, const void* wp,
                      const float* bp, void* out, const void* wnext, const float* bnext, void* out_next, const int* dims,
                      float eps_next, hipStream_t stream);

int cobevt_proj_chain_kv(const void* a, const void* const* ptrs, const int* dims, float eps_next, hipStream_t stream);

int cobevt_swap_fusion_stage(const void* qkv, const void* x, void* out, void* qkv_next, const int* map,
                             const float* bias_table, const float* mask, const void* wp, const float* bp, const void* w1,
                             const float* b1, const void* w2, const float* b2, const void* wn, const float* bn,
                             const int* dims, float scale, float eps1, float eps_next, hipStream_t stream);


int cobevt_channel_sums(const void* x, const float* shift, double* sum, double* sumsq, float* out_f, double* scratch,
                        int scratch_blocks, int dtype, long rows, int C, hipStream_t stream);
int cobevt_f64_to_f32(const double* in, float* out, int n, hipStream_t stream);
int cobevt_bn_finalize(const double* sum, const double* sumsq, const float* gamma, const float* beta, float* running_mean,
                       float* running_var, float* scale, float* shift, float* mean, float* rstd, int C, long rows, float eps,
                       float momentum, int training, int shifted, long long* batches_tracked, hipStream_t stream);
int cobevt_bn_batch_stats(const void* x, const float* gamma, const float* beta, float* running_mean, float* running_var, float* scale,
                          float* shift, float* mean, float* rstd, double* scratch, int scratch_blocks, int dtype, long rows, int C,
                          float eps, float momentum, long long* batches_tracked, hipStream_t stream);
int cobevt_bn_apply(const void* x, const void* residual, const float* scale, const float* shift, void* y, int dtype, long rows,
                    int C, int act, hipStream_t stream);
int cobevt_bn_backward(const void* x, const void* y, const void* dy, const float* mean, const float* rstd, const float* gamma,
                       double* dgamma_dbeta, float* grads_f, double* scratch, int scratch_blocks, void* dx, void* dres, int dtype,
                       long rows, int C, int act, int training, hipStream_t stream);
int cobevt_maxpool3x3s2_bwd(const void* x, const void* dy, float* dx, int dtype, int N, int H, int W, int C, hipStream_t stream);
int cobevt_fax_bev_query_train(const float* grid, const float* w, const float* bias, const float* c, const float* x, float* out,
                               const int* dims, hipStream_t stream);
int cobevt_fax_bev_query_train_bwd(const float* grid, const float* w, const float* bias, const float* c, const float* dq, float* dx,
                                   float* dw, float* dbias, float* dc, const int* dims, hipStream_t stream);
int cobevt_group_mean(const void* in, void* out, int dtype, long B, int n, long inner, int backward, hipStream_t stream);
int cobevt_maxpool3x3s2_bwd_t(const void* x, const void* dy, void* dx, int dtype, int N, int H, int W, int C, hipStream_t stream);
int cobevt_pixel_unshuffle2_nhwc(const void* in, void* out, int dtype, int N, int Ho, int Wo, int C, int inverse,
                                 hipStream_t stream);
int cobevt_upsample_nearest2_nhwc(const void* in, void* out, int dtype, int N, int H, int W, int C, int backward,
                                  hipStream_t stream);
int cobevt_sttf_warp_bwd(const float* dout, const float* tmat, const int* record_len, float* dx, int B, int L, int H, int W, int C,
                         float discrete_ratio, float downsample_rate, hipStream_t stream);

int cobevt_conv_weight_rows(const float* w, void* rows_fwd, void* rows_dgrad, const int* dims, hipStream_t stream);
int cobevt_conv3_weight_operands(const float* w, void* frag, void* rows3, const int* dims, hipStream_t stream);
int cobevt_conv3_weight_operands2(const float* w, void* const* outs, const int* dims, hipStream_t stream);
int cobevt_linear_weight_frags(const float* w, void* frag, void* frag_t, const int* dims, hipStream_t stream);
int cobevt_conv_wgrad3_chunks(const int* dims);
int cobevt_conv_wgrad3(const void* x, const void* dy, float* dw, float* scratch, const int* dims, hipStream_t stream);
int cobevt_linear_wgrad_chunks(const long* dims);
int cobevt_linear_wgrad(const void* x, const void* dy, float* dw, float* scratch, const long* dims, hipStream_t stream);
int cobevt_wgrad_block_operand(const void* src, void* dst, const int* dims, hipStream_t stream);

int cobevt_swish(const void* x, const void* dy, void* out, int dtype, long n, hipStream_t stream);
int cobevt_depthwise_wgrad(const void* x, const void* dy, float* dw, const int* dims, hipStream_t stream);
int cobevt_resize_bilinear_bwd(const void* dy, float* dx, int dtype, int N, int H, int W, int C, int Ho, int Wo, hipStream_t stream);
int cobevt_sigmoid_focal_loss_bwd(const float* pred, const float* label, const unsigned char* visibility, const unsigned int* label_mask,
                                  const float* stats, const float* gscale, float* dpred, int N, int C, int NL, int hw, int min_visibility,
                                  float alpha, float gamma, int soft_label, hipStream_t stream);


int cobevt_peer_window_alloc(long bytes, void** dptr, void* handle64);
int cobevt_peer_window_open(const void* handle64, void** dptr);
int cobevt_peer_window_close(void* dptr);
int cobevt_peer_window_free(void* dptr);
int cobevt_peer_window_status(const void* window, long bytes, int* status, int* epoch, hipStream_t stream);
int cobevt_peer_window_status_async(const void* window, long bytes, unsigned int* host_words, hipStream_t stream);
int cobevt_peer_exchange(const void* local, void* const* windows, int world, int rank, int n_local, long block_bytes,
                         const int* dest_rank, const int* dest_block, long window_bytes, long spin_limit,
                         hipStream_t stream);

int cobevt_calibrate_mfma(float* out, long long* clk, int blocks, int iters, hipStream_t stream);
int cobevt_calibrate_copy(const void* src, void* dst, long bytes, hipStream_t stream);
int cobevt_calibrate_clock_khz(int* wall_khz, int* sclk_max_khz);

#ifdef __cplusplus
}
#endif
#endif
```

Before: 633.6.

## Fuse K/V 128-channel projection chains into one launch; add wave row-chain128 kernel

Adds a two-sided variant of the 128-channel projection-chain kernel so key and value chains run in a single launch, with blocks interleaved between the K and V sides. The host now prefers this fused KV path over two separate proj_chain calls. It also adds a new row_chain128 wave kernel for attention MLP chains, though it is gated off by default via USE_ROW_CHAIN_WAVE=False, which forces 32-row tiles for C=128. The KV merge aims to cut launch overhead and improve occupancy, at the cost of a fixed 256-block grid and extra parameter passing.

```diff
diff --git a/cobevt_amd/build.py b/cobevt_amd/build.py
--- a/cobevt_amd/build.py
+++ b/cobevt_amd/build.py
@@ -6,7 +6,7 @@
 LIB = os.path.join(CSRC, "libcobevt_hip.so")
 LIB_F32S = os.path.join(CSRC, "libcobevt_hip_f32s.so")
 LIB_F32H = os.path.join(CSRC, "libcobevt_hip_f32h.so")
-SOURCES = ["igemm.hip", "conv3x3.hip", "basicblock.hip", "bottleneck.hip", "bottleneck_f32.hip", "gemm_rows.hip", "gemm_rows3.hip", "gemm_rows3_f32.hip", "bev_query.hip", "row_chain.hip", "row_chain_f32.hip", "row_chain64.hip", "ln_linear64.hip", "proj_chain128.hip", "proj_chain_k.hip", "swap_stage.hip", "stem7x7.hip", "attention.hip", "attention_resident.hip", "attention_bwd.hip", "train_rows.hip", "train_glue.hip", "train_prep.hip", "wgrad3.hip", "train_nusc.hip", "train_fax.hip", "elementwise.hip", "pairwise_fusion.hip", "postprocess.hip", "depthwise.hip", "peer_gather.hip", "calibrate.hip"]
+SOURCES = ["igemm.hip", "conv3x3.hip", "basicblock.hip", "bottleneck.hip", "bottleneck_f32.hip", "gemm_rows.hip", "gemm_rows3.hip", "gemm_rows3_f32.hip", "bev_query.hip", "row_chain.hip", "row_chain_f32.hip", "row_chain64.hip", "row_chain128.hip", "ln_linear64.hip", "proj_chain128.hip", "proj_chain_k.hip", "swap_stage.hip", "stem7x7.hip", "attention.hip", "attention_resident.hip", "attention_bwd.hip", "train_rows.hip", "train_glue.hip", "train_prep.hip", "wgrad3.hip", "train_nusc.hip", "train_fax.hip", "elementwise.hip", "pairwise_fusion.hip", "postprocess.hip", "depthwise.hip", "peer_gather.hip", "calibrate.hip"]
 HEADERS = ["common.hpp", "attn_common.hpp", "warp_common.hpp", "row_chain.hpp", "bev_query.hpp"]
 FLAGS = ["--offload-arch=gfx950", "-O3", "-std=c++17", "-fPIC", "-Wno-pass-failed"]
 EXTRA_FLAGS = {}
diff --git a/cobevt_amd/csrc/proj_chain128.hip b/cobevt_amd/csrc/proj_chain128.hip
--- a/cobevt_amd/csrc/proj_chain128.hip
+++ b/cobevt_amd/csrc/proj_chain128.hip
@@ -25,13 +25,35 @@
 }
 __device__ __forceinline__ float rbf(float x) { return bf2f(f2bf(x)); }
 
-template <int NNT, int NW>
-__global__ __launch_bounds__(NW * 64, 1) void proj_chain128_kernel(RowChainParams p, int nblk) {
+struct Proj128Side {
+    const float* pre_scale;
+    const float* pre_shift;
+    const uint4* wp;
+    const float* bp;
+    const bf16_t* skip;
+    const uint4* wn;
+    const float* bn;
+    bf16_t* out;
+    bf16_t* out_next;
+    int pre_relu, skip_rows;
+};
+
+template <int NNT, int NW, bool TWO>
+__global__ __launch_bounds__(NW * 64, 1) void proj_chain128_kernel(RowChainParams p, Proj128Side sv, int nblk) {
     extern __shared__ __attribute__((aligned(16))) unsigned char smem[];
     const uint4* wl = (const uint4*)smem;
     float* tab = (float*)(smem + kTab);
     const int tid = threadIdx.x, lane = tid & 63, wave = tid >> 6;
     const int h = lane >> 5, ql = lane & 31;
+    int grp = blockIdx.x, ngrp = gridDim.x;
+    if (TWO) {
+        grp = (blockIdx.x >> 4) * 8 + (blockIdx.x & 7);
+        ngrp = gridDim.x >> 1;
+        if ((blockIdx.x >> 3) & 1) {
+            p.pre_scale = sv.pre_scale; p.pre_shift = sv.pre_shift; p.wp = sv.wp; p.bp = sv.bp; p.skip = sv.skip;
+            p.wn = sv.wn; p.bn = sv.bn; p.out = sv.out; p.out_next = sv.out_next; p.pre_relu = sv.pre_relu; p.skip_rows = sv.skip_rows;
+        }
+    }
 
     {
         uint4* dst = (uint4*)smem;
@@ -69,8 +91,8 @@
 #pragma unroll
         for (int g = 0; g < 8; ++g) fr[g] = wl[(first + g) * 64 + lane + opq];
     };
-    const int nwaves = gridDim.x * NW;
-    for (int blk = blockIdx.x * NW + wave; blk < nblk; blk += nwaves) {
+    const int nwaves = ngrp * NW;
+    for (int blk = wave * ngrp + grp; blk < nblk; blk += nwaves) {
         asm volatile("" : "+v"(opq));
         const int m0 = blk * 32;
         const bool live = m0 + ql < p.M;
@@ -188,16 +210,18 @@
     }
 }
 
-template <int NNT> int launch128(const RowChainParams& p, hipStream_t stream) {
-    constexpr int NW = 8;
+constexpr int kNW = 8;
+
+template <int NNT, bool TWO> int launch128(const RowChainParams& p, const Proj128Side& sv, hipStream_t stream) {
     static cobevt::PerDeviceOnce attr_once;
     if (attr_once.first()) {
-        (void)hipFuncSetAttribute((const void*)proj_chain128_kernel<NNT, NW>, hipFuncAttributeMaxDynamicSharedMemorySize, kLdsBytes);
+        (void)hipFuncSetAttribute((const void*)proj_chain128_kernel<NNT, kNW, TWO>, hipFuncAttributeMaxDynamicSharedMemorySize, kLdsBytes);
     }
     const int nblk = (p.M + 31) / 32;
-    int blocks = (nblk + NW - 1) / NW;
+    int blocks = (nblk + kNW - 1) / kNW;
     if (blocks > 256) blocks = 256;
-    hipLaunchKernelGGL((proj_chain128_kernel<NNT, NW>), dim3((unsigned)blocks), dim3(NW * 64), kLdsBytes, stream, p, nblk);
+    if (TWO) blocks = 256;
+    hipLaunchKernelGGL((proj_chain128_kernel<NNT, kNW, TWO>), dim3((unsigned)blocks), dim3(kNW * 64), kLdsBytes, stream, p, sv, nblk);
     return hipGetLastError() == hipSuccess ? COBEVT_OK : COBEVT_ERR_LAUNCH;
 }
 
@@ -206,11 +230,20 @@
 int launch_proj_chain128(const RowChainParams& p, hipStream_t stream) {
     if (p.C != 128 || !p.wn || !p.out_next || p.Nn % 32 != 0 || p.Nn > 32 * kMaxNnt || p.next_act != 0) return -1;
     if (p.M < 32768) return -1;
+    const Proj128Side none = {};
     switch (p.Nn / 32) {
-        case 4: return launch128<4>(p, stream);
-        case 8: return launch128<8>(p, stream);
+        case 4: return launch128<4, false>(p, none, stream);
+        case 8: return launch128<8, false>(p, none, stream);
         default: return -1;
     }
 }
 
-}
+bool proj_chain128_kv_fits(int M, int Nn) { return M >= 32768 && (Nn == 128 || Nn == 256); }
+
+int launch_proj_chain128_kv(const RowChainParams& pk, const RowChainParams& pv, hipStream_t stream) {
+    if (pk.C != 128 || !pk.wn || !pk.out_next || !pv.wn || !pv.out_next || pk.next_act != 0 || !proj_chain128_kv_fits(pk.M, pk.Nn)) return -1;
+    const Proj128Side sv = {pv.pre_scale, pv.pre_shift, pv.wp, pv.bp, pv.skip, pv.wn, pv.bn, pv.out, pv.out_next, pv.pre_relu, pv.skip_rows};
+    return pk.Nn == 128 ? launch128<4, true>(pk, sv, stream) : launch128<8, true>(pk, sv, stream);
+}
+
+}
diff --git a/cobevt_amd/csrc/proj_chain_k.hip b/cobevt_amd/csrc/proj_chain_k.hip
--- a/cobevt_amd/csrc/proj_chain_k.hip
+++ b/cobevt_amd/csrc/proj_chain_k.hip
@@ -250,6 +250,29 @@
     const int nsides = dims[5];
     p.eps_next = eps_next;
     if (nsides < 1 || nsides > 2) return COBEVT_ERR_ARG;
+    if (p.K == 128) {
+        if (nsides != 2 || p.M < 1) return COBEVT_ERR_SHAPE;
+        RowChainParams rp[2];
+        for (int s = 0; s < 2; ++s) {
+            const void* const* q = ptrs + 9 * s;
+            RowChainParams& r = rp[s];
+            r.a = p.a; r.skip = (const bf16_t*)q[4]; r.out = (bf16_t*)q[7];
+            r.wp = (const uint4*)q[2]; r.bp = (const float*)q[3];
+            r.w1 = r.w2 = (const uint4*)q[5]; r.b1 = r.b2 = (const float*)q[6];
+            r.post_g = r.post_b = nullptr;
+            r.wn = (const uint4*)q[5]; r.bn = (const float*)q[6]; r.out_next = (bf16_t*)q[8];
+            r.M = p.M; r.C = 128; r.Hd = 8; r.Hdp = 128;
+            r.Nn = p.Nn; r.next_ln = p.next_ln; r.next_act = 0;
+            r.skip_rows = dims[7 + 2 * s] > 0 ? dims[7 + 2 * s] : p.M;
+            r.eps1 = 0.f; r.eps_post = 0.f; r.eps_next = eps_next;
+            r.pre_scale = (const float*)q[0]; r.pre_shift = (const float*)q[1]; r.pre_relu = dims[6 + 2 * s];
+            if (!r.wp || !r.wn || !r.out_next) return COBEVT_ERR_ARG;
+            if ((r.pre_scale == nullptr) != (r.pre_shift == nullptr)) return COBEVT_ERR_ARG;
+            if (r.skip_rows > p.M || p.M % r.skip_rows) return COBEVT_ERR_SHAPE;
+        }
+        const int rc = launch_proj_chain128_kv(rp[0], rp[1], stream);
+        return rc < 0 ? COBEVT_ERR_SHAPE : rc;
+    }
     if (p.M < 1 || p.K < 256 || p.K > 512 || p.K % 128) return COBEVT_ERR_SHAPE;
     if (p.Nn < 8 || p.Nn % 8 || p.Nn > kNnMax) return COBEVT_ERR_SHAPE;
     for (int s = 0; s < 2; ++s) {
@@ -272,3 +295,11 @@
     }
     return hipGetLastError() == hipSuccess ? COBEVT_OK : COBEVT_ERR_LAUNCH;
 }
+
+extern "C" int cobevt_proj_chain_kv_route(const int* dims) {
+    if (!dims || dims[0] != 0 || dims[1] < 1 || dims[5] < 1 || dims[5] > 2) return 0;
+    const int M = dims[1], K = dims[2], Nn = dims[3];
+    if (K == 128) return dims[5] == 2 && proj_chain128_kv_fits(M, Nn) ? 2 : 0;
+    if (K < 256 || K > 512 || K % 128) return 0;
+    return (Nn < 8 || Nn % 8 || Nn > kNnMax) ? 0 : 1;
+}
diff --git a/cobevt_amd/csrc/row_chain.hip b/cobevt_amd/csrc/row_chain.hip
--- a/cobevt_amd/csrc/row_chain.hip
+++ b/cobevt_amd/csrc/row_chain.hip
@@ -325,7 +325,9 @@
     if ((wnext == nullptr) != (out_next == nullptr)) return COBEVT_ERR_ARG;
     if (wnext && (p.Nn < 8 || p.Nn % 8 || p.Nn > kRcBnMax || p.next_act < 0 || p.next_act > 2)) return COBEVT_ERR_SHAPE;
     if (dims[8] == 0) {
-        const int rc = launch_row_chain64(p, stream);
+        int rc = launch_row_chain64(p, stream);
+        if (rc >= 0) return rc;
+        rc = launch_row_chain128(p, stream);
         if (rc >= 0) return rc;
     }
     const int rows = dims[8] == 64 ? 64 : 32;
@@ -367,3 +369,8 @@
     launch_chain<1, 32, true, false>(p, stream);
     return hipGetLastError() == hipSuccess ? COBEVT_OK : COBEVT_ERR_LAUNCH;
 }
+
+extern "C" int cobevt_attn_mlp_chain_wave128(const int* dims) {
+    if (!dims || dims[0] != 0 || dims[8] != 0) return 0;
+    return row_chain128_route(dims[1], dims[2], dims[3], dims[4], dims[5], dims[5] ? dims[7] : 0) >= 0 ? 1 : 0;
+}
diff --git a/cobevt_amd/csrc/row_chain.hpp b/cobevt_amd/csrc/row_chain.hpp
--- a/cobevt_amd/csrc/row_chain.hpp
+++ b/cobevt_amd/csrc/row_chain.hpp
@@ -27,7 +27,11 @@
 };
 
 int launch_row_chain64(const RowChainParams& p, hipStream_t stream);
+int row_chain128_route(int M, int C, int Hd, int Hdp, int Nn, int next_act);
+int launch_row_chain128(const RowChainParams& p, hipStream_t stream);
 int launch_proj_chain128(const RowChainParams& p, hipStream_t stream);
+bool proj_chain128_kv_fits(int M, int Nn);
+int launch_proj_chain128_kv(const RowChainParams& pk, const RowChainParams& pv, hipStream_t stream);
 
 int launch_row_chain_f32(const void* a, const void* skip, void* out, const void* wp, const float* bp, const void* w1, const float* b1,
                          const void* w2, const float* b2, const float* post_g, const float* post_b, const void* wnext, const float* bnext,
diff --git a/cobevt_amd/csrc/row_chain128.hip b/cobevt_amd/csrc/row_chain128.hip
--- /dev/null
+++ b/cobevt_amd/csrc/row_chain128.hip
@@ -0,0 +1,298 @@
+#include "row_chain.hpp"
+
+namespace cobevt {
+
+namespace {
+
+constexpr int kF1 = 0, kF2 = 64;
+constexpr int kTab = 128 * 1024;
+constexpr int kB1 = 0, kBp = 256, kB2 = 384, kPg = 512, kPb = 640, kBn = 768;
+constexpr int kTabFloats = 896;
+constexpr int kLdsBytes = kTab + kTabFloats * 4;
+constexpr int kNW = 8;
+
+__device__ __forceinline__ float xhalf_sum(float v) {
+    const auto r = __builtin_amdgcn_permlane32_swap(__float_as_uint(v), __float_as_uint(v), false, false);
+    return __uint_as_float(r[0]) + __uint_as_float(r[1]);
+}
+__device__ __forceinline__ void half_swap(uint2& a, uint2& b) {
+    auto r = __builtin_amdgcn_permlane32_swap(a.x, b.x, false, false);
+    a.x = r[0]; b.x = r[1];
+    r = __builtin_amdgcn_permlane32_swap(a.y, b.y, false, false);
+    a.y = r[0]; b.y = r[1];
+}
+__device__ __forceinline__ uint4 pack8(const float* v) {
+    return make_uint4(pack_bf2(v[0], v[1]), pack_bf2(v[2], v[3]), pack_bf2(v[4], v[5]), pack_bf2(v[6], v[7]));
+}
+__device__ __forceinline__ void unpack8(const uint4& u, float* v) {
+    v[0] = bf2f(u.x & 0xffff); v[1] = bf2f(u.x >> 16); v[2] = bf2f(u.y & 0xffff); v[3] = bf2f(u.y >> 16);
+    v[4] = bf2f(u.z & 0xffff); v[5] = bf2f(u.z >> 16); v[6] = bf2f(u.w & 0xffff); v[7] = bf2f(u.w >> 16);
+}
+__device__ __forceinline__ float rbf(float x) { return bf2f(f2bf(x)); }
+
+__device__ __forceinline__ void normalise_row(float (&v)[64], float eps) {
+    float s = 0.f;
+#pragma unroll
+    for (int i = 0; i < 64; ++i) s += v[i];
+    const float mean = xhalf_sum(s) * (1.0f / 128.0f);
+    float q = 0.f;
+#pragma unroll
+    for (int i = 0; i < 64; ++i) { const float d = v[i] - mean; q += d * d; }
+    const float rstd = rsqrtf(xhalf_sum(q) * (1.0f / 128.0f) + eps);
+#pragma unroll
+    for (int i = 0; i < 64; ++i) v[i] = (v[i] - mean) * rstd;
+}
+
+template <int NNT>
+__global__ __launch_bounds__(kNW * 64, 1) void row_chain128_kernel(RowChainParams p, int nblk) {
+    extern __shared__ __attribute__((aligned(16))) unsigned char smem[];
+    const uint4* wl = (const uint4*)smem;
+    float* tab = (float*)(smem + kTab);
+    const int tid = threadIdx.x, lane = tid & 63, wave = tid >> 6;
+    const int h = lane >> 5, ql = lane & 31;
+
+    {
+        uint4* dst = (uint4*)smem;
+        constexpr int TOTAL = 128 * 64, PER = TOTAL / (kNW * 64);
+        uint4 tmp[PER];
+#pragma unroll
+        for (int u = 0; u < PER; ++u) {
+            const int i = tid + u * kNW * 64;
+            const int f = i >> 6, ln = i & 63, hh = ln >> 5, q = ln & 31;
+            const uint4* base = f < kF2 ? p.w1 + (size_t)f * 64 : p.w2 + (size_t)(f - kF2) * 64;
+            const unsigned char* a0 = (const unsigned char*)(base + q) + 8 * hh;
+            const unsigned char* a1 = (const unsigned char*)(base + 32 + q) + 8 * hh;
+            const uint2 lo = *(const uint2*)a0, hi = *(const uint2*)a1;
+            tmp[u] = make_uint4(lo.x, lo.y, hi.x, hi.y);
+        }
+#pragma unroll
+        for (int u = 0; u < PER; ++u) dst[tid + u * kNW * 64] = tmp[u];
+        for (int i = tid; i < kTabFloats; i += kNW * 64) {
+            float v;
+            if (i < kBp) v = p.b1[i];
+            else if (i < kB2) v = p.bp ? p.bp[i - kBp] : 0.f;
+            else if (i < kPg) v = p.b2[i - kB2];
+            else if (i < kPb) v = p.post_g ? p.post_g[i - kPg] : 1.f;
+            else if (i < kBn) v = p.post_b ? p.post_b[i - kPb] : 0.f;
+            else v = (NNT > 0 && p.bn && i - kBn < p.Nn) ? p.bn[i - kBn] : 0.f;
+            tab[i] = v;
+        }
+    }
+    __syncthreads();
+
+    int li = lane, t4 = 4 * h, li2 = kF2 * 64 + lane, tb = kTab + 16 * h;
+    auto load_wp = [&](uint4 (&fr)[8], int t) {
+        const uint4* src = p.wp + (size_t)t * 8 * 64 + li;
+#pragma unroll
+        for (int g = 0; g < 8; ++g) fr[g] = src[g * 64];
+    };
+    auto load_wn = [&](uint4 (&fr)[8], int n) {
+        const unsigned char* src = (const unsigned char*)(p.wn + (size_t)n * 8 * 64 + (li & 31)) + 2 * t4;
+#pragma unroll
+        for (int g = 0; g < 8; ++g) {
+            const uint2 lo = *(const uint2*)(src + g * 1024), hi = *(const uint2*)(src + g * 1024 + 512);
+            fr[g] = make_uint4(lo.x, lo.y, hi.x, hi.y);
+        }
+    };
+    const int nwaves = gridDim.x * kNW;
+    for (int blk = wave * gridDim.x + blockIdx.x; blk < nblk; blk += nwaves) {
+        asm volatile("" : "+v"(li), "+v"(t4), "+v"(li2), "+v"(tb));
+        const int m0 = blk * 32;
+        const bool live = m0 + ql < p.M;
+        const size_t grow = live ? m0 + ql : p.M - 1;
+        const bf16_t* arow = p.a + grow * 128;
+        uint4 ypk[8];
+        {
+            uint4 af[8], sk[8], fr[2][8];
+            load_wp(fr[0], 0);
+#pragma unroll
+            for (int g = 0; g < 8; ++g) af[g] = *(const uint4*)(arow + 16 * g + 8 * h);
+            if (p.skip) {
+                const bf16_t* srow = p.skip + (size_t)(grow % p.skip_rows) * 128;
+#pragma unroll
+                for (int g = 0; g < 8; ++g) sk[g] = *(const uint4*)(srow + 16 * g + 8 * h);
+            } else {
+#pragma unroll
+                for (int g = 0; g < 8; ++g) sk[g] = make_uint4(0, 0, 0, 0);
+            }
+#pragma unroll
+            for (int t = 0; t < 4; ++t) {
+                f32x16 acc;
+#pragma unroll
+                for (int r = 0; r < 16; ++r) acc[r] = 0.f;
+                if (t < 3) load_wp(fr[(t + 1) & 1], t + 1);
+                __builtin_amdgcn_sched_barrier(0);
+#pragma unroll
+                for (int g = 0; g < 8; ++g) mfma_kgroup<bf16_t>(fr[t & 1][g], af[g], acc);
+#pragma unroll
+                for (int m = 0; m < 2; ++m) {
+                    uint2 s0 = make_uint2(sk[2 * t + m].x, sk[2 * t + m].y), s1 = make_uint2(sk[2 * t + m].z, sk[2 * t + m].w);
+                    half_swap(s0, s1);
+                    const float4 b0 = *(const float4*)(smem + tb + 4 * (kBp + 32 * t + 16 * m));
+                    const float4 b1 = *(const float4*)(smem + tb + 4 * (kBp + 32 * t + 16 * m + 8));
+                    float d[8];
+                    d[0] = acc[8 * m + 0] + b0.x + bf2f(s0.x & 0xffff); d[1] = acc[8 * m + 1] + b0.y + bf2f(s0.x >> 16);
+                    d[2] = acc[8 * m + 2] + b0.z + bf2f(s0.y & 0xffff); d[3] = acc[8 * m + 3] + b0.w + bf2f(s0.y >> 16);
+                    d[4] = acc[8 * m + 4] + b1.x + bf2f(s1.x & 0xffff); d[5] = acc[8 * m + 5] + b1.y + bf2f(s1.x >> 16);
+                    d[6] = acc[8 * m + 6] + b1.z + bf2f(s1.y & 0xffff); d[7] = acc[8 * m + 7] + b1.w + bf2f(s1.y >> 16);
+                    ypk[2 * t + m] = pack8(d);
+                }
+            }
+        }
+        uint4 xh[8];
+        {
+            float v[64];
+#pragma unroll
+            for (int i = 0; i < 8; ++i) unpack8(ypk[i], &v[8 * i]);
+            normalise_row(v, p.eps1);
+#pragma unroll
+            for (int i = 0; i < 8; ++i) xh[i] = pack8(&v[8 * i]);
+        }
+        uint4 fr[8];
+#pragma unroll
+        for (int g = 0; g < 8; ++g) fr[g] = wl[(kF1 + g) * 64 + li];
+        f32x16 z[4];
+#pragma unroll
+        for (int t = 0; t < 4; ++t)
+#pragma unroll
+            for (int m = 0; m < 2; ++m) {
+                float yv[8];
+                unpack8(ypk[2 * t + m], yv);
+                const float4 b0 = *(const float4*)(smem + tb + 4 * (kB2 + 32 * t + 16 * m));
+                const float4 b1 = *(const float4*)(smem + tb + 4 * (kB2 + 32 * t + 16 * m + 8));
+                z[t][8 * m + 0] = yv[0] + b0.x; z[t][8 * m + 1] = yv[1] + b0.y; z[t][8 * m + 2] = yv[2] + b0.z; z[t][8 * m + 3] = yv[3] + b0.w;
+                z[t][8 * m + 4] = yv[4] + b1.x; z[t][8 * m + 5] = yv[5] + b1.y; z[t][8 * m + 6] = yv[6] + b1.z; z[t][8 * m + 7] = yv[7] + b1.w;
+            }
+#pragma unroll
+        for (int n = 0; n < 8; ++n) {
+            f32x16 acc;
+#pragma unroll
+            for (int r = 0; r < 16; ++r) acc[r] = 0.f;
+#pragma unroll
+            for (int hf = 0; hf < 2; ++hf) {
+#pragma unroll
+                for (int g = 0; g < 4; ++g) mfma_kgroup<bf16_t>(fr[4 * hf + g], xh[4 * hf + g], acc);
+                __builtin_amdgcn_sched_barrier(0);
+#pragma unroll
+                for (int j = 0; j < 4; ++j)
+                    fr[4 * hf + j] = wl[((2 * hf + (j >> 1)) * 16 + 2 * n + (j & 1)) * 64 + li2];
+                __builtin_amdgcn_sched_barrier(0);
+            }
+            float hv[16];
+#pragma unroll
+            for (int k = 0; k < 4; ++k) {
+                const float4 b = *(const float4*)(smem + tb + 4 * (kB1 + 32 * n + 8 * k));
+                hv[4 * k] = gelu_bf16(acc[4 * k] + b.x); hv[4 * k + 1] = gelu_bf16(acc[4 * k + 1] + b.y);
+                hv[4 * k + 2] = gelu_bf16(acc[4 * k + 2] + b.z); hv[4 * k + 3] = gelu_bf16(acc[4 * k + 3] + b.w);
+            }
+            const uint4 hb0 = pack8(&hv[0]), hb1 = pack8(&hv[8]);
+#pragma unroll
+            for (int hf = 0; hf < 2; ++hf) {
+#pragma unroll
+                for (int j = 0; j < 4; ++j) mfma_kgroup<bf16_t>(fr[4 * hf + j], (j & 1) ? hb1 : hb0, z[2 * hf + (j >> 1)]);
+                __builtin_amdgcn_sched_barrier(0);
+                if (n < 7) {
+#pragma unroll
+                    for (int g = 0; g < 4; ++g) fr[4 * hf + g] = wl[(kF1 + (n + 1) * 8 + 4 * hf + g) * 64 + li];
+                }
+                __builtin_amdgcn_sched_barrier(0);
+            }
+        }
+        uint4 fn[2][8];
+        if (NNT > 0) load_wn(fn[0], 0);
+        float v[64];
+#pragma unroll
+        for (int t = 0; t < 4; ++t)
+#pragma unroll
+            for (int r = 0; r < 16; ++r) v[16 * t + r] = z[t][r];
+        if (p.post_g) {
+            normalise_row(v, p.eps_post);
+#pragma unroll
+            for (int i = 0; i < 8; ++i) {
+                const float4 g0 = *(const float4*)(smem + tb + 4 * (kPg + 16 * i)), g1 = *(const float4*)(smem + tb + 4 * (kPg + 16 * i + 8));
+                const float4 c0 = *(const float4*)(smem + tb + 4 * (kPb + 16 * i)), c1 = *(const float4*)(smem + tb + 4 * (kPb + 16 * i + 8));
+                float* d = &v[8 * i];
+                d[0] = d[0] * g0.x + c0.x; d[1] = d[1] * g0.y + c0.y; d[2] = d[2] * g0.z + c0.z; d[3] = d[3] * g0.w + c0.w;
+                d[4] = d[4] * g1.x + c1.x; d[5] = d[5] * g1.y + c1.y; d[6] = d[6] * g1.z + c1.z; d[7] = d[7] * g1.w + c1.w;
+            }
+        }
+        uint4 opk[8];
+        {
+            bf16_t* orow = p.out + grow * 128;
+#pragma unroll
+            for (int i = 0; i < 8; ++i) {
+                opk[i] = pack8(&v[8 * i]);
+                uint2 r0 = make_uint2(opk[i].x, opk[i].y), r1 = make_uint2(opk[i].z, opk[i].w);
+                half_swap(r0, r1);
+                if (live) *(uint4*)(orow + 16 * i + 8 * h) = make_uint4(r0.x, r0.y, r1.x, r1.y);
+            }
+        }
+        if (NNT > 0) {
+            if (p.next_ln) {
+#pragma unroll
+                for (int i = 0; i < 8; ++i) unpack8(opk[i], &v[8 * i]);
+                normalise_row(v, p.eps_next);
+#pragma unroll
+                for (int i = 0; i < 8; ++i) opk[i] = pack8(&v[8 * i]);
+            }
+            bf16_t* nrow = p.out_next + grow * p.Nn;
+            const float act_floor = p.next_act == 1 ? 0.f : -INFINITY;
+#pragma unroll
+            for (int n = 0; n < NNT; ++n) {
+                f32x16 acc;
+#pragma unroll
+                for (int r = 0; r < 16; ++r) acc[r] = 0.f;
+                if (n + 1 < NNT) load_wn(fn[(n + 1) & 1], n + 1);
+                __builtin_amdgcn_sched_barrier(0);
+#pragma unroll
+                for (int g = 0; g < 8; ++g) mfma_kgroup<bf16_t>(fn[n & 1][g], opk[g], acc);
+                float nv[16];
+#pragma unroll
+                for (int k = 0; k < 4; ++k) {
+                    const float4 b = *(const float4*)(smem + tb + 4 * (kBn + 32 * n + 8 * k));
+                    nv[4 * k] = fmaxf(acc[4 * k] + b.x, act_floor); nv[4 * k + 1] = fmaxf(acc[4 * k + 1] + b.y, act_floor);
+                    nv[4 * k + 2] = fmaxf(acc[4 * k + 2] + b.z, act_floor); nv[4 * k + 3] = fmaxf(acc[4 * k + 3] + b.w, act_floor);
+                }
+#pragma unroll
+                for (int m = 0; m < 2; ++m) {
+                    const uint4 pk = pack8(&nv[8 * m]);
+                    uint2 r0 = make_uint2(pk.x, pk.y), r1 = make_uint2(pk.z, pk.w);
+                    half_swap(r0, r1);
+                    if (live) *(uint4*)(nrow + 32 * n + 16 * m + 8 * h) = make_uint4(r0.x, r0.y, r1.x, r1.y);
+                }
+            }
+        }
+    }
+}
+
+template <int NNT> int launch(const RowChainParams& p, hipStream_t stream) {
+    static cobevt::PerDeviceOnce attr_once;
+    if (attr_once.first()) {
+        (void)hipFuncSetAttribute((const void*)row_chain128_kernel<NNT>, hipFuncAttributeMaxDynamicSharedMemorySize, kLdsBytes);
+    }
+    const int nblk = (p.M + 31) / 32;
+    int blocks = (nblk + kNW - 1) / kNW;
+    if (blocks > 256) blocks = 256;
+    hipLaunchKernelGGL((row_chain128_kernel<NNT>), dim3((unsigned)blocks), dim3(kNW * 64), kLdsBytes, stream, p, nblk);
+    return hipGetLastError() == hipSuccess ? COBEVT_OK : COBEVT_ERR_LAUNCH;
+}
+
+}
+
+int row_chain128_route(int M, int C, int Hd, int Hdp, int Nn, int next_act) {
+    if (C != 128 || Hd != 256 || Hdp != 256 || M < 32768) return -1;
+    if (Nn == 0) return 0;
+    if (next_act != 0 && next_act != 1) return -1;
+    return Nn == 128 ? 4 : Nn == 32 ? 1 : -1;
+}
+
+int launch_row_chain128(const RowChainParams& p, hipStream_t stream) {
+    switch (row_chain128_route(p.M, p.C, p.Hd, p.Hdp, p.wn ? p.Nn : 0, p.wn ? p.next_act : 0)) {
+        case 0: return launch<0>(p, stream);
+        case 1: return launch<1>(p, stream);
+        case 4: return launch<4>(p, stream);
+        default: return -1;
+    }
+}
+
+}
diff --git a/cobevt_amd/host/fax_modules.py b/cobevt_amd/host/fax_modules.py
--- a/cobevt_amd/host/fax_modules.py
+++ b/cobevt_amd/host/fax_modules.py
@@ -260,13 +260,13 @@
         pk, pv = self._pair_plan("k"), self._pair_plan("v")
         plan_key = rt.conv_plan(self, "fproj", self.feature_proj[2], pre_bn=self.feature_proj[0]) if self.feature_proj is not None else None
         plan_val = rt.conv_plan(self, "flin", self.feature_linear[2], pre_bn=self.feature_linear[0])
+        if not padded and plan_key is not None and ops.proj_chain_kv_fusable(feature, plan_key, plan_val, pk, pv, img):
+            kk, vv = ops.proj_chain_kv(feature, plan_key, plan_val, pk, pv, residual=img, out_k=o.get("kk"), out_v=o.get("vv"))
+            return {"n": n, "hp": hp, "wp": wp, "kk": kk, "vv": vv}
         if (not padded and plan_key is not None and ops.proj_chain_fusable(feature, plan_key, pk, img)
                 and ops.proj_chain_fusable(feature, plan_val, pv, None)):
             kk = ops.proj_chain(feature, plan_key, pk, residual=img, out_next=o.get("kk"))
             vv = ops.proj_chain(feature, plan_val, pv, out_next=o.get("vv"))
-            return {"n": n, "hp": hp, "wp": wp, "kk": kk, "vv": vv}
-        if not padded and plan_key is not None and ops.proj_chain_kv_fusable(feature, plan_key, plan_val, pk, pv, img):
-            kk, vv = ops.proj_chain_kv(feature, plan_key, plan_val, pk, pv, residual=img, out_k=o.get("kk"), out_v=o.get("vv"))
             return {"n": n, "hp": hp, "wp": wp, "kk": kk, "vv": vv}
         if self.feature_proj is not None:
             key = ops.conv2d(feature, plan_key, residual=img, out=kv_buffer("key"))
diff --git a/cobevt_amd/lib.py b/cobevt_amd/lib.py
--- a/cobevt_amd/lib.py
+++ b/cobevt_amd/lib.py
@@ -27,6 +27,7 @@
     "cobevt_linear_rows_wfrag": (ctypes.c_int, [_vp, _vp, _vp, _vp, _vp, _vp, _vp, _c_long_p, ctypes.c_float, _vp]),
     "cobevt_linear_rows": (ctypes.c_int, [_vp, _vp, _vp, _vp, _vp, _vp, _vp, _vp, _vp, _c_long_p, ctypes.c_float, _vp]),
     "cobevt_attn_mlp_chain": (ctypes.c_int, [_vp] * 14 + [_c_int_p, ctypes.c_float, ctypes.c_float, ctypes.c_float, _vp]),
+    "cobevt_attn_mlp_chain_wave128": (ctypes.c_int, [_c_int_p]),
     "cobevt_pairwise_warp": (ctypes.c_int, [_vp] * 5 + [ctypes.c_int] * 6 + [ctypes.c_float, ctypes.c_float, _vp]),
     "cobevt_pairwise_warp_bwd": (ctypes.c_int, [_vp] * 4 + [ctypes.c_int] * 6 + [ctypes.c_float, ctypes.c_float, _vp]),
     "cobevt_agent_message_reduce": (ctypes.c_int, [_vp] * 5 + [ctypes.c_int] * 6 + [_vp]),
@@ -85,6 +86,7 @@
     "cobevt_mean_linear_rows_small_k": (ctypes.c_int, [_vp, _vp, _vp, _vp, _c_long_p, ctypes.c_float, _vp]),
     "cobevt_proj_chain": (ctypes.c_int, [_vp] * 10 + [_c_int_p, ctypes.c_float, _vp]),
     "cobevt_proj_chain_kv": (ctypes.c_int, [_vp, ctypes.POINTER(ctypes.c_void_p), _c_int_p, ctypes.c_float, _vp]),
+    "cobevt_proj_chain_kv_route": (ctypes.c_int, [_c_int_p]),
     "cobevt_swap_fusion_stage": (ctypes.c_int, [_vp, _vp, _vp, _vp, _c_int_p, _vp, _vp, _vp, _vp, _vp, _vp, _vp, _vp, _vp, _vp, _c_int_p,
                                                 ctypes.c_float, ctypes.c_float, ctypes.c_float, _vp]),
     "cobevt_channel_sums": (ctypes.c_int, [_vp, _vp, _vp, _vp, _vp, _vp, ctypes.c_int, ctypes.c_int, ctypes.c_long, ctypes.c_int, _vp]),
diff --git a/cobevt_amd/ops.py b/cobevt_amd/ops.py
--- a/cobevt_amd/ops.py
+++ b/cobevt_amd/ops.py
@@ -27,6 +27,7 @@
 USE_ROW_CHAIN = True
 USE_BOTTLENECK_F32 = True
 USE_GEMM_ROWS3_F32 = True
+USE_ROW_CHAIN_WAVE = False
 USE_ROW_CHAIN_F32 = True
 BASICBLOCK_TILE_ROWS = 0
 USE_BASICBLOCK = True
@@ -38,6 +39,7 @@
 USE_HEAD_CONV = True
 USE_PROJ_CHAIN = True
 USE_PROJ_CHAIN_KV = True
+USE_PROJ_CHAIN_KV128 = True
 USE_PROJ_CHAIN_WAVE = True
 USE_SWAP_STAGE = True
 USE_BOTTLENECK = True
@@ -1061,6 +1063,12 @@
             and plan_n.act <= 2)
 
 
+def row_chain_wave128(m, c, hd, hdp, nn_, next_act, rows=0):
+    if rows != 0 or c != 128 or hd != 256 or hdp != 256 or m < 32768:
+        return False
+    return nn_ == 0 or (nn_ in (32, 128) and next_act in (0, 1))
+
+
 def attn_mlp_chain(a, skip, plan_p, plan_1, plan_2, post_ln=None, next_plan=None):
     _need_cuda(a, skip)
     c, hd = plan_p.cout, plan_1.cout
@@ -1087,7 +1095,7 @@
     nn_ = next_plan.cout if fuse_next else 0
     out_next = torch.empty(a.shape[:-1] + (nn_,), device=a.device, dtype=a.dtype) if fuse_next else None
     dims = _ints([plan_p.code, m, c, hd, plan_2.kp_rows, nn_, int(next_plan.has_ln) if fuse_next else 0,
-                  next_plan.act if fuse_next else 0, ROW_CHAIN_ROWS, skip_rows])
+                  next_plan.act if fuse_next else 0, ROW_CHAIN_ROWS or (0 if USE_ROW_CHAIN_WAVE or c != 128 else 32), skip_rows])
     pg, pb, pe = post_ln if post_ln is not None else (None, None, 0.0)
 
     def cost():
@@ -1138,9 +1146,22 @@
     return out_next
 
 
+def proj_chain_kv_route(m, k, nn_, nsides=2):
+    if m < 1 or nsides not in (1, 2):
+        return 0
+    if k == 128:
+        return 2 if nsides == 2 and m >= 32768 and nn_ in (128, 256) else 0
+    if k not in (256, 384, 512):
+        return 0
+    return 1 if 8 <= nn_ <= 768 and nn_ % 8 == 0 else 0
+
+
 def proj_chain_kv_fusable(x, plan_key, plan_val, next_key, next_val, residual):
     k = x.shape[-1]
-    if not (USE_PROJ_CHAIN_KV and x.dtype == torch.bfloat16 and x.is_contiguous() and k in (256, 384, 512)):
+    if not (USE_PROJ_CHAIN_KV and x.dtype == torch.bfloat16 and x.is_contiguous()):
+        return False
+    route = proj_chain_kv_route(x.numel() // k, k, next_key.cout)
+    if route == 0 or (route == 2 and not (USE_PROJ_CHAIN and USE_PROJ_CHAIN_WAVE and USE_PROJ_CHAIN_KV128)):
         return False
     for pl in (plan_key, plan_val):
         if pl is None:
diff --git a/include/cobevt_hip.h b/include/cobevt_hip.h
--- a/include/cobevt_hip.h
+++ b/include/cobevt_hip.h
@@ -56,6 +56,7 @@
                           const float* b1, const void* w2, const float* b2, const float* post_gamma,
                           const float* post_beta, const void* wnext, const float* bnext, void* out_next, const int* dims,
                           float eps1, float eps_post, float eps_next, hipStream_t stream);
+int cobevt_attn_mlp_chain_wave128(const int* dims);
 
 int cobevt_window_attention(const void* q, const void* k, const void* v, void* out, const float* bias_table,
                             const float* mask, const int* dims, float scale, hipStream_t stream);
@@ -195,6 +196,7 @@
                       float eps_next, hipStream_t stream);
 
 int cobevt_proj_chain_kv(const void* a, const void* const* ptrs, const int* dims, float eps_next, hipStream_t stream);
+int cobevt_proj_chain_kv_route(const int* dims);
 
 int cobevt_swap_fusion_stage(const void* qkv, const void* x, void* out, void* qkv_next, const int* map,
                              const float* bias_table, const float* mask, const void* wp, const float* bp, const void* w1,
```

Measured after the change: 635.6 (median of 3 runs). Within noise of the previous version (+0.3%).
